# sea-with-sakura/ViT-of-Pytorch

Hardware: AMD Instinct MI355X
Metric: images/sec training step, ViT-B/16 224px bf16, 1/2/4/8 MI355X (higher is better)
Workload: dtype bf16; 1 GPU; ViT-B16 @224 train step (fwd+CE+bwd+SGD-momentum/OneCycleLR); model=ViT-B16, image_size=224, per_gpu_batch=256, global_batch=256, seq_len=197, num_classes=1000, parallelism=dp1, step_launch=eager

## Files before the change

### include/vit_hip.h

```cpp
#ifndef VIT_HIP_H_
#define VIT_HIP_H_

#include <stdint.h>

#ifdef __cplusplus
extern "C" {
#endif

typedef void* vit_stream_t;

enum vit_status {
  VIT_OK = 0,
  VIT_ERR_INVALID_ARG = 1,
  VIT_ERR_HIP = 2,
  VIT_ERR_UNSUPPORTED = 3,
};

const char* vit_last_error(void);
int vit_abi_version(void);
const char* vit_build_id(void);

enum vit_layout { VIT_K_CONTIG = 0, VIT_MN_CONTIG = 1 };

typedef struct vit_dropout {
  float p;
  uint32_t site;
  uint64_t seed;
  uint64_t offset;
  int64_t row_stride;
} vit_dropout;

int vit_dropout_mask(const vit_dropout* d, int64_t row0, int64_t rows, int64_t cols, float* mult,
                     int64_t ld, vit_stream_t stream);

enum vit_epilogue {
  VIT_EPI_F32 = 0,
  VIT_EPI_BF16 = 1,
  VIT_EPI_BIAS_BF16 = 2,
  VIT_EPI_BIAS_GELU = 3,
  VIT_EPI_BIAS_RESID_F32 = 4,
  VIT_EPI_GELU_BWD = 5,
  VIT_EPI_PATCH = 6,
  VIT_EPI_SPLITK = 7,
  VIT_EPI_BIAS_GELU_DGELU = 8,
  VIT_EPI_MUL_BF16 = 9,
};

typedef struct vit_gemm_args {
  int64_t M, N, K;
  const void* A;
  int64_t lda;
  int64_t a_batch_stride;
  int32_t a_layout;
  int32_t b_layout;
  const void* B;
  int64_t ldb;
  int64_t b_batch_stride;
  void* C;
  int64_t ldc;
  int64_t c_batch_stride;
  void* C2;
  int64_t ldc2;
  const float* bias;
  int64_t bias_batch_stride;
  const void* aux;
  int64_t ldaux;
  const float* aux2;
  int64_t batch;
  int64_t split_k;
  int64_t tokens;
  float* col_partial;
  int32_t epilogue;
  int32_t tile;
  const vit_dropout* dropout;
} vit_gemm_args;

int vit_gemm_bf16(const vit_gemm_args* args, vit_stream_t stream);
int64_t vit_gemm_tile_rows(const vit_gemm_args* args);
int64_t vit_gemm_partial_rows(const vit_gemm_args* args);
int64_t vit_gemm_split_rows(const vit_gemm_args* args);
int vit_gemm_bf16_part(const vit_gemm_args* args, int32_t part, vit_stream_t stream);
int vit_gemm_splitk_group(const vit_gemm_args* args, int32_t n, vit_stream_t stream);
#define VIT_GEMM_TABLE_MAX 128
int64_t vit_gemm_group_table_bytes(int32_t n);
int vit_gemm_group_prepare(const vit_gemm_args* args, const int32_t* direct, int32_t n, void* table,
                           int64_t table_bytes, int32_t* total, vit_stream_t stream);
int vit_gemm_group_launch(const void* table, int32_t n, int32_t total, vit_stream_t stream);

int vit_splitk_reduce(const float* ws, int64_t batch, int64_t split, int64_t M, int64_t N,
                      float* out, int64_t ldo, int64_t out_batch_stride, int32_t accumulate,
                      vit_stream_t stream);
#define VIT_SPLITK_GROUP_MAX 8
typedef struct vit_splitk_job {
  const float* ws;
  int64_t batch, split, M, N;
  float* out;
  int64_t ldo, out_batch_stride;
  int32_t accumulate;
  int32_t reserved;
} vit_splitk_job;
int vit_splitk_reduce_group(const vit_splitk_job* jobs, int32_t njobs, vit_stream_t stream);

int vit_layernorm_fwd(const float* x, int64_t ldx, const float* gamma, const float* beta,
                      void* y, int64_t ldy, int32_t y_f32, float* mean, float* rstd,
                      int64_t rows, int64_t D, float eps, vit_stream_t stream);
int64_t vit_layernorm_bwd_partial_rows(int64_t rows);
int64_t vit_layernorm_bwd_blocks(int64_t rows);
int vit_layernorm_bwd(const void* dy, int64_t lddy, int32_t dy_f32, const float* x, int64_t ldx,
                      const float* mean, const float* rstd, const float* gamma,
                      const float* dres, int64_t lddres, float* dx, int64_t lddx,
                      void* dx_bf16, int64_t lddxb, float* partial, float* dgamma_dbeta,
                      float* dx_colsum, int32_t accumulate_params, int64_t rows, int64_t D,
                      const vit_dropout* dx_dropout, vit_stream_t stream);

int vit_attention_fwd(const void* qkv, void* o, float* lse, int64_t B, int64_t N, int64_t H,
                      int64_t hd, float scale, vit_stream_t stream);
int vit_attention_bwd(const void* qkv, const void* o, const void* dout, const float* lse, void* dqkv,
                      float* bias_partial, int64_t B, int64_t N, int64_t H, int64_t hd, float scale,
                      vit_stream_t stream);
int vit_attention_fwd_rows(const void* qkv, void* o, float* lse, int64_t B, int64_t N, int64_t H, int64_t hd,
                           float scale, int64_t q_rows, vit_stream_t stream);
int vit_attention_bwd_rows(const void* qkv, const void* o, const void* dout, const float* lse, void* dqkv,
                           float* bias_partial, int64_t B, int64_t N, int64_t H, int64_t hd, float scale,
                           int64_t q_rows, vit_stream_t stream);
int64_t vit_attention_bias_rows(int64_t N, int64_t hd, int32_t path);
int64_t vit_attention_workspace_elems(int64_t B, int64_t N, int64_t H, int32_t path);
int vit_attention_fwd_ex(const void* qkv, void* o, float* lse, int64_t B, int64_t N, int64_t H, int64_t hd,
                         float scale, int64_t q_rows, int32_t path, vit_stream_t stream);
int vit_attention_bwd_ex(const void* qkv, const void* o, const void* dout, const float* lse, void* dqkv,
                         float* bias_partial, int64_t B, int64_t N, int64_t H, int64_t hd, float scale,
                         int64_t q_rows, int32_t path, float* workspace, vit_stream_t stream);

int vit_attention_fwd_varlen(const void* q, int64_t ldq, const void* k, int64_t ldk, const void* v, int64_t ldv,
                             void* o, int64_t ldo, const int32_t* cu_q, int64_t B, int64_t max_q, int64_t Nkv,
                             int64_t H, int64_t hd, float scale, vit_stream_t stream);

int vit_im2col(const float* x, void* out, int64_t B, int64_t img, int64_t P, int64_t Kpad,
               vit_stream_t stream);
int vit_im2col_hw(const float* x, void* out, int64_t B, int64_t H, int64_t W, int64_t Ph, int64_t Pw, int64_t Kpad,
                  vit_stream_t stream);

int vit_preprocess_u8(const uint8_t* images, int64_t B, int64_t H, int64_t W, int64_t image_stride,
                      const uint8_t* flips, int64_t out_h, int64_t out_w, const float* mean_std, float* out,
                      vit_stream_t stream);

enum vit_image_layout { VIT_IMAGES_HWC = 0, VIT_IMAGES_CHW = 1 };
int vit_preprocess_u8_gather(const uint8_t* images, int64_t n_images, int32_t layout, int64_t H, int64_t W,
                             int64_t image_stride, const int64_t* index, int64_t B, const uint8_t* flips,
                             int64_t out_h, int64_t out_w, const float* mean_std, float* out,
                             const int64_t* labels_in, int64_t* labels_out, vit_stream_t stream);

int vit_embed_grad(const float* dh0, int64_t B, int64_t N, int64_t D, float* dpos, float* dcls,
                   float* dconv_bias, const vit_dropout* dropout, vit_stream_t stream);

int64_t vit_colsum_partial_rows(int64_t rows);
int vit_colsum(const void* in, int32_t in_bf16, int64_t rows, int64_t cols, int64_t ld,
               float* partial, float* out, int32_t accumulate, vit_stream_t stream);
int vit_colsum3(const void* in, int32_t in_bf16, int64_t rows, int64_t seg, int64_t ld, float* partial,
                float* out0, float* out1, float* out2, int32_t accumulate, vit_stream_t stream);

#define VIT_COLSUM_BATCH_MAX 8
typedef struct vit_colsum_job {
  const float* in;
  int64_t rows, cols, ld, seg;
  float* out0;
  float* out1;
  float* out2;
  int32_t accumulate;
  int32_t reserved;
} vit_colsum_job;
int vit_colsum_batch(const vit_colsum_job* jobs, int32_t njobs, vit_stream_t stream);

int vit_gemm_f32(int64_t M, int64_t N, int64_t K, const float* A, int64_t lda, int32_t a_trans,
                 const float* B, int64_t ldb, int32_t b_trans, float* C, int64_t ldc,
                 const float* bias, int32_t accumulate, vit_stream_t stream);

int vit_cross_entropy(const float* logits, const int64_t* labels, int64_t B, int64_t C,
                      float* dlogits, float grad_scale, float* row_stats, vit_stream_t stream);

int vit_sgd_step(float* p, const float* g, float* buf, void* p_bf16, int64_t n, float lr,
                 float momentum, float weight_decay, int32_t first, vit_stream_t stream);
int vit_sgd_step_dev(float* p, const float* g, float* buf, void* p_bf16, int64_t n, const float* hyper,
                     float weight_decay, vit_stream_t stream);
int vit_cast_f32_bf16(const float* in, void* out, int64_t n, vit_stream_t stream);
int vit_cast_pad_rows(const float* in, int64_t rows, int64_t cols, void* out, int64_t ldo,
                      vit_stream_t stream);
#define VIT_CAST_BATCH_MAX 8
typedef struct vit_cast_job {
  const float* in;
  int64_t rows, cols, ldi;
  void* out;
  int64_t ldo, rows_pad, cols_pad;
} vit_cast_job;
int vit_cast_pad_batch(const vit_cast_job* jobs, int32_t njobs, vit_stream_t stream);
int vit_pack_cols(const float* in, int64_t zstride, int64_t ldi, int64_t rows, int64_t cols, int64_t Z,
                  void* out, int64_t ldo, int32_t out_bf16, vit_stream_t stream);
int vit_pack_cols_batched(const float* in, int64_t in_batch_stride, int64_t zstride, int64_t ldi, int64_t rows,
                          int64_t cols, int64_t Z, void* out, int64_t out_batch_stride, int64_t ldo,
                          int32_t out_bf16, int64_t batch, vit_stream_t stream);
int vit_transpose_f32_bf16(const float* in, int64_t rows, int64_t cols, int64_t ldi, void* out, int64_t ldo,
                           int64_t batch, int64_t in_batch_stride, int64_t out_batch_stride, vit_stream_t stream);
int vit_axpby(const float* x, float* y, int64_t n, float a, float b, vit_stream_t stream);

int vit_im2col_f32(const float* x, float* out, int64_t B, int64_t img, int64_t P, int64_t Kpad,
                   vit_stream_t stream);
int vit_im2col_hw_f32(const float* x, float* out, int64_t B, int64_t H, int64_t W, int64_t Ph, int64_t Pw,
                      int64_t Kpad, vit_stream_t stream);
int vit_embed_fwd_f32(float* h, int64_t B, int64_t N, int64_t D, const float* pos, const float* cls,
                      vit_stream_t stream);
int vit_gelu_f32(const float* in, float* out, int64_t n, vit_stream_t stream);
int vit_attention_fwd_f32(const float* qkv, float* o, int64_t B, int64_t N, int64_t H, int64_t hd,
                          float inv_sqrt_hd, vit_stream_t stream);

int vit_gelu_bwd_f32(const float* u, const float* dy, float* dx, int64_t n, vit_stream_t stream);
int vit_dropout_apply_f32(const vit_dropout* d, const float* in, float* out, int64_t rows, int64_t cols,
                          vit_stream_t stream);
int vit_add_bcast_f32(const float* x, const float* y, float* out, int64_t outer, int64_t inner, vit_stream_t stream);
int vit_segment_colsum(const void* in, int32_t in_bf16, int64_t ld, int64_t segs, int64_t seg_stride, int64_t row0,
                       int64_t seg_rows, int64_t cols, float scale, float* out, int64_t ldo, vit_stream_t stream);
int vit_segment_colsum_bcast(const void* in, int32_t in_bf16, int64_t ld, int64_t segs, int64_t seg_stride,
                             int64_t row0, int64_t seg_rows, int64_t cols, float scale, float* out, int64_t ldo,
                             void* bc, int64_t ldbc, int64_t bc_rows, vit_stream_t stream);
int64_t vit_router_dx_gate_partial_rows(int64_t rows_pad);
int vit_router_dx_gate(const float* dx, int64_t ldx, const float* g, int64_t ldg, float g_scale, const void* gp,
                       int64_t ldgp, int64_t T, int64_t N, int64_t reserve, int64_t cols, void* out, int64_t ldo,
                       int64_t rows_pad, int64_t cols_pad, float* col_partial, int64_t ldp, vit_stream_t stream);
int64_t vit_router_head_partials(int64_t T);
int vit_router_head_fwd(const float* logits, const float* noise, int32_t noise_mode, const float* yhard_in, int64_t T,
                        int64_t N, int32_t bs, int64_t reserve, int32_t training, float norm, float* soft, float* ysoft,
                        float* hard, float* indices, float* ent_part, float* entropy, vit_stream_t stream);
int vit_router_head_bwd(const float* soft, const float* ysoft, const float* dsoft, const float* dhard, const float* dind,
                        const float* dent, float norm, int64_t T, int64_t N, int32_t bs, int64_t reserve,
                        int32_t training, float* dlogits, vit_stream_t stream);
int vit_router_select(const float* indices, int64_t T, int32_t npos, const uint32_t* active_masks, int32_t nkeys,
                      void* active, void* sel, void* any, vit_stream_t stream);
int vit_cast_rows_masked(const float* in, int64_t ldi, int64_t rows, int64_t cols, const void* mask, void* out,
                         int64_t ldo, vit_stream_t stream);
int vit_cls_mse(const float* x, int64_t ldx, const float* t, int64_t ldt, int64_t B, int64_t D, float* e, float* part,
                float* loss, vit_stream_t stream);
int vit_cls_mse_bwd(float* dx, int64_t lddx, const float* e, int64_t B, int64_t D, const float* g,
// ... 24 lines not shown
```

### vit-of-pytorch_amd/csrc/capi.hip

```cpp
#include <stdarg.h>

#include "common.h"
#include "build_id.h"

namespace vit {
static thread_local char g_last_error[512] = "";

void set_error(const char* fmt, ...) {
  va_list ap;
  va_start(ap, fmt);
  vsnprintf(g_last_error, sizeof(g_last_error), fmt, ap);
  va_end(ap);
}

int check_hip(hipError_t e, const char* what) {
  if (e == hipSuccess) return VIT_OK;
  set_error("%s: %s", what, hipGetErrorString(e));
  return VIT_ERR_HIP;
}
}

extern "C" const char* vit_last_error(void) { return vit::g_last_error; }
extern "C" int vit_abi_version(void) { return 21; }
extern "C" const char* vit_build_id(void) { return VIT_BUILD_ID; }
```

### vit-of-pytorch_amd/csrc/elementwise.hip

```cpp
#include "common.h"

namespace {

template <typename OUT>
__global__ void im2col_kernel(const float* __restrict__ x, OUT* __restrict__ out, int B, int H, int W, int Ph, int Pw,
                              int Kpad) {
  const int gw = W / Pw;
  const int N = (H / Ph) * gw + 1;
  const long total = (long)B * N * Kpad;
  const int PP = Ph * Pw, K = 3 * PP;
  for (long i = (long)blockIdx.x * blockDim.x + threadIdx.x; i < total; i += (long)gridDim.x * blockDim.x) {
    const int col = (int)(i % Kpad);
    const long row = i / Kpad;
    const int t = (int)(row % N);
    const int b = (int)(row / N);
    float v = 0.f;
    if (t > 0 && col < K) {
      const int patch = t - 1, py = patch / gw, px = patch % gw;
      const int c = col / PP, rem = col % PP, ky = rem / Pw, kx = rem % Pw;
      v = x[(((long)b * 3 + c) * H + (py * Ph + ky)) * W + (px * Pw + kx)];
    }
    if constexpr (sizeof(OUT) == 2)
      out[i] = f2bf(v);
    else
      out[i] = v;
  }
}

__global__ void pos_grad_kernel(const float* __restrict__ dh0, int B, int N, int D, float* __restrict__ dpos,
                                DropDev drop) {
  const int n = blockIdx.y;
  const int d = blockIdx.x * blockDim.x + threadIdx.x;
  if (d >= D) return;
  float s = 0.f;
  if (drop.thr) {
    for (int b = 0; b < B; ++b) s += dh0[((long)b * N + n) * D + d] * drop_mult1(drop, (long)b * N + n, d);
  } else {
    for (int b = 0; b < B; ++b) s += dh0[((long)b * N + n) * D + d];
  }
  dpos[(long)n * D + d] = s;
}

__global__ void dropout_mask_kernel(DropDev drop, long row0, long rows, int cols, float* __restrict__ out, long ld) {
  const long r = blockIdx.y;
  const int c = blockIdx.x * blockDim.x + threadIdx.x;
  if (r >= rows || c >= cols) return;
  out[r * ld + c] = drop.thr ? drop_mult1(drop, row0 + r, c) : 1.0f;
}

template <typename OUT>
__global__ void im2col8_kernel(const float* __restrict__ x, OUT* __restrict__ out, int B, int H, int W, int Ph,
                               int Pw) {
  const int gw = W / Pw, N = (H / Ph) * gw + 1, PP = Ph * Pw, K8 = 3 * PP / 8;
  const long total = (long)B * N * K8;
  for (long i = (long)blockIdx.x * blockDim.x + threadIdx.x; i < total; i += (long)gridDim.x * blockDim.x) {
    const int c8 = (int)(i % K8);
    const long row = i / K8;
    const int t = (int)(row % N), b = (int)(row / N);
    float4 lo = make_float4(0.f, 0.f, 0.f, 0.f), hi = lo;
    if (t > 0) {
      const int patch = t - 1, py = patch / gw, px = patch % gw;
      const int col = c8 * 8, c = col / PP, rem = col % PP, ky = rem / Pw, kx = rem % Pw;
      const float4* src =
          reinterpret_cast<const float4*>(x + (((long)b * 3 + c) * H + (py * Ph + ky)) * W + (px * Pw + kx));
      lo = src[0];
      hi = src[1];
    }
    if constexpr (sizeof(OUT) == 2) {
      uint4 v;
      v.x = (uint32_t)f2bf(lo.x) | ((uint32_t)f2bf(lo.y) << 16);
      v.y = (uint32_t)f2bf(lo.z) | ((uint32_t)f2bf(lo.w) << 16);
      v.z = (uint32_t)f2bf(hi.x) | ((uint32_t)f2bf(hi.y) << 16);
      v.w = (uint32_t)f2bf(hi.z) | ((uint32_t)f2bf(hi.w) << 16);
      reinterpret_cast<uint4*>(out)[i] = v;
    } else {
      reinterpret_cast<float4*>(out)[2 * i] = lo;
      reinterpret_cast<float4*>(out)[2 * i + 1] = hi;
    }
  }
}

__global__ void __launch_bounds__(768) pos_grad4_kernel(const float* __restrict__ dh0, int B, int N, int D,
                                                        float* __restrict__ dpos, DropDev drop) {
  __shared__ float4 red[8][96];
  const int C4 = D / 4 / gridDim.y;
  const int n = blockIdx.x, c = threadIdx.x % C4, grp = threadIdx.x / C4;
  const int d = (blockIdx.y * C4 + c) * 4;
  float4 s = make_float4(0.f, 0.f, 0.f, 0.f);
  const float* base = dh0 + (long)n * D + d;
  const long bstride = (long)N * D;
#pragma unroll 4
  for (int b = grp; b < B; b += 8) {
    float4 v = *reinterpret_cast<const float4*>(base + b * bstride);
    if (drop.thr) {
      const long r = (long)b * N + n;
      v.x *= drop_mult1(drop, r, d);
      v.y *= drop_mult1(drop, r, d + 1);
      v.z *= drop_mult1(drop, r, d + 2);
      v.w *= drop_mult1(drop, r, d + 3);
    }
    s.x += v.x;
    s.y += v.y;
    s.z += v.z;
    s.w += v.w;
  }
  red[grp][c] = s;
  __syncthreads();
  if (grp == 0) {
#pragma unroll
    for (int k = 1; k < 8; ++k) {
      s.x += red[k][c].x;
      s.y += red[k][c].y;
      s.z += red[k][c].z;
      s.w += red[k][c].w;
    }
    *reinterpret_cast<float4*>(dpos + (long)n * D + d) = s;
  }
}

__global__ void __launch_bounds__(256) cls_bias_grad16_kernel(const float* __restrict__ dpos, int N, int D,
                                                              float* __restrict__ dcls, float* __restrict__ dbias) {
  __shared__ float red[16][17];
  const int c = threadIdx.x & 15, r = threadIdx.x >> 4;
  const int d = blockIdx.x * 16 + c;
  float s = 0.f;
  if (d < D)
    for (int n = 1 + r; n < N; n += 16) s += dpos[(long)n * D + d];
  red[r][c] = s;
  __syncthreads();
  if (r == 0 && d < D) {
    float t = 0.f;
#pragma unroll
    for (int k = 0; k < 16; ++k) t += red[k][c];
    dbias[d] = t;
    dcls[d] = dpos[d];
  }
}

constexpr int COLSUM_MAX_CHUNKS = 256;
constexpr int COLSUM_MIN_ROWS_PER_CHUNK = 64;

__device__ __forceinline__ float* seg_dst(float* out, float* out1, float* out2, long seg, long ch, int cols, int col) {
  if (seg <= 0) return out + ch * cols + col;
  const int k = (int)(col / seg);
  float* base = k == 0 ? out : (k == 1 ? out1 : out2);
  return base ? base + (col - k * seg) : nullptr;
}

template <bool BF16>
__global__ void __launch_bounds__(256) colsum8_kernel(const void* __restrict__ in, long rows, int cols, long ld,
                                                      int chunks, float* __restrict__ out, int accumulate,
                                                      long seg = 0, float* out1 = nullptr, float* out2 = nullptr) {
  __shared__ float red[8][32][9];
// ... 238 lines not shown
    buf[t] = d;
    p[t] -= lr * d;
    if (pb) pb[t] = f2bf(p[t]);
  }
}

__global__ void cast_kernel(const float* __restrict__ in, bf16_t* __restrict__ out, long n) {
  for (long i = (long)blockIdx.x * blockDim.x + threadIdx.x; i < n; i += (long)gridDim.x * blockDim.x) out[i] = f2bf(in[i]);
}
__global__ void cast_pad_kernel(const float* __restrict__ in, long rows, long cols, bf16_t* __restrict__ out, long ldo) {
  const long total = rows * ldo;
  for (long i = (long)blockIdx.x * blockDim.x + threadIdx.x; i < total; i += (long)gridDim.x * blockDim.x) {
    const long r = i / ldo, c = i % ldo;
    out[i] = c < cols ? f2bf(in[r * cols + c]) : (bf16_t)0;
  }
}
__global__ void axpby_kernel(const float* x, float* y, long n, float a, float b) {
  for (long i = (long)blockIdx.x * blockDim.x + threadIdx.x; i < n; i += (long)gridDim.x * blockDim.x)
    y[i] = a * x[i] + (b == 0.f ? 0.f : b * y[i]);
}

unsigned grid_for(long n, int per_thread = 1) {
  long b = (n / per_thread + 255) / 256;
  if (b < 1) b = 1;
  if (b > 8192) b = 8192;
  return (unsigned)b;
}

template <typename OUT>
void im2col_launch(const float* x, OUT* out, int64_t B, int64_t H, int64_t W, int64_t Ph, int64_t Pw, int64_t Kpad,
                   hipStream_t s) {
  const int64_t N = (H / Ph) * (W / Pw) + 1;
  if (Pw % 8 == 0 && W % 4 == 0 && Kpad == 3 * Ph * Pw && (uintptr_t)x % 16 == 0 && (uintptr_t)out % 16 == 0)
    hipLaunchKernelGGL(im2col8_kernel<OUT>, dim3(grid_for(B * N * Kpad / 8)), dim3(256), 0, s, x, out, (int)B, (int)H,
                       (int)W, (int)Ph, (int)Pw);
  else
    hipLaunchKernelGGL(im2col_kernel<OUT>, dim3(grid_for(B * N * Kpad)), dim3(256), 0, s, x, out, (int)B, (int)H,
                       (int)W, (int)Ph, (int)Pw, (int)Kpad);
}

}

extern "C" int vit_im2col_hw(const float* x, void* out, int64_t B, int64_t H, int64_t W, int64_t Ph, int64_t Pw,
                             int64_t Kpad, vit_stream_t stream) {
  VIT_CHECK_ARG(x && out && B > 0 && Ph > 0 && Pw > 0 && H >= Ph && W >= Pw && Kpad >= 3 * Ph * Pw &&
                    3 * H * W < (1L << 31) && Kpad < (1L << 31),
                "vit_im2col_hw: bad args");
  im2col_launch(x, (bf16_t*)out, B, H, W, Ph, Pw, Kpad, (hipStream_t)stream);
  VIT_LAUNCH_CHECK("vit_im2col_hw");
}

extern "C" int vit_im2col_hw_f32(const float* x, float* out, int64_t B, int64_t H, int64_t W, int64_t Ph, int64_t Pw,
                                 int64_t Kpad, vit_stream_t stream) {
  VIT_CHECK_ARG(x && out && B > 0 && Ph > 0 && Pw > 0 && H >= Ph && W >= Pw && Kpad >= 3 * Ph * Pw &&
                    3 * H * W < (1L << 31) && Kpad < (1L << 31),
                "vit_im2col_hw_f32: bad args");
  im2col_launch(x, out, B, H, W, Ph, Pw, Kpad, (hipStream_t)stream);
  VIT_LAUNCH_CHECK("vit_im2col_hw_f32");
}

extern "C" int vit_im2col(const float* x, void* out, int64_t B, int64_t img, int64_t P, int64_t Kpad,
                          vit_stream_t stream) {
  VIT_CHECK_ARG(x && out && B > 0 && P > 0 && img >= P && Kpad >= 3 * P * P, "vit_im2col: bad args");
  im2col_launch(x, (bf16_t*)out, B, img, img, P, P, Kpad, (hipStream_t)stream);
  VIT_LAUNCH_CHECK("vit_im2col");
}

extern "C" int vit_embed_grad(const float* dh0, int64_t B, int64_t N, int64_t D, float* dpos, float* dcls,
                              float* dconv_bias, const vit_dropout* dropout, vit_stream_t stream) {
  VIT_CHECK_ARG(dh0 && dpos && dcls && dconv_bias && B > 0 && N > 0 && D > 0, "vit_embed_grad: bad args");
  hipStream_t s = (hipStream_t)stream;
  int ys = 0;
  if (D % 4 == 0 && ((uintptr_t)dh0 % 16) == 0 && ((uintptr_t)dpos % 16) == 0) {
    const int d4 = (int)(D / 4);
    for (int y = (d4 + 95) / 96; y <= d4; ++y)
      if (d4 % y == 0) { ys = y; break; }
    if (ys == 1 && N < 256 && d4 % 2 == 0) ys = 2;
  }
  if (ys > 0)
    hipLaunchKernelGGL(pos_grad4_kernel, dim3((unsigned)N, (unsigned)ys), dim3((unsigned)(8 * (D / 4 / ys))), 0, s, dh0,
                       (int)B, (int)N, (int)D, dpos, make_drop(dropout));
  else
    hipLaunchKernelGGL(pos_grad_kernel, dim3((unsigned)((D + 255) / 256), (unsigned)N), dim3(256), 0, s, dh0, (int)B,
                       (int)N, (int)D, dpos, make_drop(dropout));
  hipLaunchKernelGGL(cls_bias_grad16_kernel, dim3((unsigned)((D + 15) / 16)), dim3(256), 0, s, dpos, (int)N, (int)D,
                     dcls, dconv_bias);
  VIT_LAUNCH_CHECK("vit_embed_grad");
}

extern "C" int64_t vit_colsum_partial_rows(int64_t rows) {
  int64_t c = rows / COLSUM_MIN_ROWS_PER_CHUNK;
  if (c > COLSUM_MAX_CHUNKS) c = COLSUM_MAX_CHUNKS;
  return c < 1 ? 1 : c;
}

extern "C" int vit_colsum3(const void* in, int32_t in_bf16, int64_t rows, int64_t seg, int64_t ld, float* partial,
                           float* out0, float* out1, float* out2, int32_t accumulate, vit_stream_t stream) {
  const int64_t cols = 3 * seg;
  VIT_CHECK_ARG(in && partial && seg > 0 && ld >= cols, "vit_colsum3: bad args");
  const int chunks = (int)vit_colsum_partial_rows(rows);
  const bool vec = cols % 8 == 0 && ld % 8 == 0 && ((uintptr_t)in % 32) == 0 && ((uintptr_t)partial % 16) == 0;
  VIT_CHECK_ARG(vec, "vit_colsum3: needs 8-column aligned rows");
  hipStream_t s = (hipStream_t)stream;
  const unsigned gx = (unsigned)((cols / 8 + 31) / 32);
  if (chunks == 1) {
    if (in_bf16)
      hipLaunchKernelGGL(colsum8_kernel<true>, dim3(gx, 1), dim3(256), 0, s, in, (long)rows, (int)cols, (long)ld, 1,
                         out0, (int)accumulate, (long)seg, out1, out2);
    else
      hipLaunchKernelGGL(colsum8_kernel<false>, dim3(gx, 1), dim3(256), 0, s, in, (long)rows, (int)cols, (long)ld, 1,
                         out0, (int)accumulate, (long)seg, out1, out2);
    VIT_LAUNCH_CHECK("vit_colsum3");
  }
  if (in_bf16)
    hipLaunchKernelGGL(colsum8_kernel<true>, dim3(gx, chunks), dim3(256), 0, s, in, (long)rows, (int)cols, (long)ld,
                       chunks, partial, 0, 0L, (float*)nullptr, (float*)nullptr);
  else
    hipLaunchKernelGGL(colsum8_kernel<false>, dim3(gx, chunks), dim3(256), 0, s, in, (long)rows, (int)cols, (long)ld,
                       chunks, partial, 0, 0L, (float*)nullptr, (float*)nullptr);
  hipLaunchKernelGGL(colsum8_kernel<false>, dim3(gx, 1), dim3(256), 0, s, (const void*)partial, (long)chunks,
                     (int)cols, (long)cols, 1, out0, (int)accumulate, (long)seg, out1, out2);
  VIT_LAUNCH_CHECK("vit_colsum3");
}

extern "C" int vit_colsum(const void* in, int32_t in_bf16, int64_t rows, int64_t cols, int64_t ld, float* partial,
                          float* out, int32_t accumulate, vit_stream_t stream) {
  VIT_CHECK_ARG(in && partial && out && cols > 0 && ld >= cols, "vit_colsum: bad args");
  hipStream_t s = (hipStream_t)stream;
  const int chunks = (int)vit_colsum_partial_rows(rows);
  const bool vec = cols % 8 == 0 && ld % 8 == 0 && ((uintptr_t)in % 32) == 0 && ((uintptr_t)partial % 16) == 0 &&
                   ((uintptr_t)out % 4) == 0;
  if (vec) {
    const unsigned gx = (unsigned)((cols / 8 + 31) / 32);
    float* dst1 = chunks == 1 ? out : partial;
    if (in_bf16)
      hipLaunchKernelGGL(colsum8_kernel<true>, dim3(gx, chunks), dim3(256), 0, s, in, (long)rows, (int)cols, (long)ld,
                         chunks, dst1, chunks == 1 ? (int)accumulate : 0);
    else
      hipLaunchKernelGGL(colsum8_kernel<false>, dim3(gx, chunks), dim3(256), 0, s, in, (long)rows, (int)cols,
                         (long)ld, chunks, dst1, chunks == 1 ? (int)accumulate : 0);
    if (chunks > 1)
      hipLaunchKernelGGL(colsum8_kernel<false>, dim3(gx, 1), dim3(256), 0, s, (const void*)partial, (long)chunks,
                         (int)cols, (long)cols, 1, out, (int)accumulate);
    VIT_LAUNCH_CHECK("vit_colsum");
  }
  const unsigned gx = (unsigned)((cols + 255) / 256);
  hipLaunchKernelGGL(colsum_partial_kernel, dim3(gx, chunks), dim3(256), 0, s, in, (int)in_bf16, (long)rows, (int)cols,
                     (long)ld, chunks, partial);
  hipLaunchKernelGGL(colsum_final_kernel, dim3(gx), dim3(256), 0, s, partial, chunks, (int)cols, out, (int)accumulate);
  VIT_LAUNCH_CHECK("vit_colsum");
}

namespace {
struct ColsumJobDev {
  const float* in;
  float* out[3];
  long ld;
  int rows, cols, seg, acc, blk0;
  int pad;
};
struct ColsumBatchDev {
  ColsumJobDev j[VIT_COLSUM_BATCH_MAX];
  int n;
};

__global__ void __launch_bounds__(256) colsum_batch_kernel(const ColsumBatchDev bt) {
  __shared__ float4 red[16][17];
  const int bid = blockIdx.x;
  int jx = 0;
#pragma unroll
  for (int k = 1; k < VIT_COLSUM_BATCH_MAX; ++k)
    if (k < bt.n && bid >= bt.j[k].blk0) jx = k;
  const ColsumJobDev& J = bt.j[jx];
  const int c0 = (bid - J.blk0) * 64;
  const int cg = threadIdx.x & 15, rl = threadIdx.x >> 4;
  const int c = c0 + cg * 4;
  float4 acc = {0.f, 0.f, 0.f, 0.f};
  if (J.pad && c < J.cols) {
    const float* p = J.in + c;
    const long ld = J.ld;
    int r = rl;
    for (; r + 112 < J.rows; r += 128) {
      float4 v[8];
#pragma unroll
      for (int u = 0; u < 8; ++u) v[u] = *reinterpret_cast<const float4*>(p + (long)(r + 16 * u) * ld);
#pragma unroll
      for (int u = 0; u < 8; ++u) {
        acc.x += v[u].x; acc.y += v[u].y; acc.z += v[u].z; acc.w += v[u].w;
      }
    }
    for (; r < J.rows; r += 16) {
      const float4 v = *reinterpret_cast<const float4*>(p + (long)r * ld);
      acc.x += v.x; acc.y += v.y; acc.z += v.z; acc.w += v.w;
    }
  } else if (c < J.cols) {
    const float* p = J.in + c;
    const int nc = J.cols - c < 4 ? J.cols - c : 4;
    for (int r = rl; r < J.rows; r += 16) {
      const float* q = p + (long)r * J.ld;
      acc.x += q[0];
      if (nc > 1) acc.y += q[1];
      if (nc > 2) acc.z += q[2];
      if (nc > 3) acc.w += q[3];
    }
  }
  red[rl][cg] = acc;
  __syncthreads();
  if (threadIdx.x < 64) {
    const int g = threadIdx.x >> 2, k = threadIdx.x & 3;
    const int col = c0 + threadIdx.x;
    if (col < J.cols) {
      float s = 0.f;
#pragma unroll
      for (int q = 0; q < 16; ++q) s += reinterpret_cast<const float*>(&red[q][g])[k];
      const int sg = J.seg > 0 ? col / J.seg : 0;
      float* base = J.out[sg];
      if (base) {
        float* dst = base + (col - sg * J.seg);
        *dst = J.acc ? *dst + s : s;
      }
    }
  }
}
}

extern "C" int vit_colsum_batch(const vit_colsum_job* jobs, int32_t njobs, vit_stream_t stream) {
  VIT_CHECK_ARG(jobs && njobs >= 1 && njobs <= VIT_COLSUM_BATCH_MAX, "vit_colsum_batch: njobs=%d outside [1, %d]",
                (int)njobs, VIT_COLSUM_BATCH_MAX);
  ColsumBatchDev bt{};
  int blk = 0;
  for (int k = 0; k < njobs; ++k) {
    const vit_colsum_job& s = jobs[k];
    VIT_CHECK_ARG(s.in && s.rows >= 1 && s.cols >= 1 && s.ld >= s.cols && s.rows <= 0x7fffffff &&
                      s.cols <= 0x7fffffff,
                  "vit_colsum_batch: job %d: bad shape (rows %lld, cols %lld, ld %lld)", k, (long long)s.rows,
                  (long long)s.cols, (long long)s.ld);
    VIT_CHECK_ARG(s.seg >= 0 && (s.seg == 0 || s.cols <= 3 * s.seg), "vit_colsum_batch: job %d: seg %lld", k,
                  (long long)s.seg);
    VIT_CHECK_ARG(s.out0 || s.out1 || s.out2, "vit_colsum_batch: job %d has no output", k);
    ColsumJobDev& d = bt.j[k];
    d.in = s.in;
    d.out[0] = s.out0;
    d.out[1] = s.out1;
    d.out[2] = s.out2;
    d.ld = (long)s.ld;
    d.rows = (int)s.rows;
    d.cols = (int)s.cols;
    d.seg = (int)s.seg;
    d.acc = s.accumulate ? 1 : 0;
    d.blk0 = blk;
    d.pad = (s.cols % 4 == 0 && s.ld % 4 == 0 && ((uintptr_t)s.in % 16) == 0) ? 1 : 0;
    blk += (int)((s.cols + 63) / 64);
  }
  bt.n = njobs;
  hipLaunchKernelGGL(colsum_batch_kernel, dim3(blk), dim3(256), 0, (hipStream_t)stream, bt);
  return vit::check_hip(hipGetLastError(), "vit_colsum_batch");
}

extern "C" int vit_gemm_f32(int64_t M, int64_t N, int64_t K, const float* A, int64_t lda, int32_t a_trans,
                            const float* B, int64_t ldb, int32_t b_trans, float* C, int64_t ldc, const float* bias,
                            int32_t accumulate, vit_stream_t stream) {
  VIT_CHECK_ARG(A && B && C && M >= 0 && N >= 0 && K >= 0, "vit_gemm_f32: bad args");
  if (M == 0 || N == 0) return VIT_OK;
  dim3 grid((unsigned)((N + 31) / 32), (unsigned)((M + 31) / 32)), block(256);
  hipLaunchKernelGGL(gemm_f32_kernel, grid, block, 0, (hipStream_t)stream, (int)M, (int)N, (int)K, A, (long)lda,
                     (int)a_trans, B, (long)ldb, (int)b_trans, C, (long)ldc, bias, (int)accumulate);
  VIT_LAUNCH_CHECK("vit_gemm_f32");
}

extern "C" int vit_cross_entropy(const float* logits, const int64_t* labels, int64_t B, int64_t C, float* dlogits,
                                 float grad_scale, float* row_stats, vit_stream_t stream) {
  VIT_CHECK_ARG(logits && labels && B > 0 && C > 0, "vit_cross_entropy: bad args");
  hipLaunchKernelGGL(ce_kernel, dim3((unsigned)B), dim3(256), 0, (hipStream_t)stream, logits, labels, (int)C, dlogits,
                     grad_scale, row_stats);
  VIT_LAUNCH_CHECK("vit_cross_entropy");
}

extern "C" int vit_sgd_step_dev(float* p, const float* g, float* buf, void* p_bf16, int64_t n, const float* hyper,
                                float weight_decay, vit_stream_t stream) {
  VIT_CHECK_ARG(p && g && buf && hyper && n >= 0, "vit_sgd_step_dev: bad args");
  VIT_CHECK_ARG(((uintptr_t)p | (uintptr_t)g | (uintptr_t)buf) % 16 == 0 && ((uintptr_t)p_bf16 % 8 == 0),
                "vit_sgd_step_dev: buffers must be 16-B aligned (bf16 mirror 8-B)");
  if (n == 0) return VIT_OK;
  hipLaunchKernelGGL(sgd_kernel<SgdDevScalars>, dim3(grid_for(n, 4)), dim3(256), 0, (hipStream_t)stream, p, g, buf,
                     (bf16_t*)p_bf16, (long)n, SgdDevScalars{hyper}, weight_decay);
  VIT_LAUNCH_CHECK("vit_sgd_step_dev");
}

extern "C" int vit_sgd_step(float* p, const float* g, float* buf, void* p_bf16, int64_t n, float lr, float momentum,
                            float weight_decay, int32_t first, vit_stream_t stream) {
  VIT_CHECK_ARG(p && g && buf && n >= 0, "vit_sgd_step: bad args");
  VIT_CHECK_ARG(((uintptr_t)p | (uintptr_t)g | (uintptr_t)buf) % 16 == 0 && ((uintptr_t)p_bf16 % 8 == 0),
                "vit_sgd_step: buffers must be 16-B aligned (bf16 mirror 8-B)");
  if (n == 0) return VIT_OK;
  hipLaunchKernelGGL(sgd_kernel<SgdHostScalars>, dim3(grid_for(n, 4)), dim3(256), 0, (hipStream_t)stream, p, g, buf,
                     (bf16_t*)p_bf16, (long)n, SgdHostScalars{lr, momentum, (int)first}, weight_decay);
  VIT_LAUNCH_CHECK("vit_sgd_step");
}

extern "C" int vit_cast_f32_bf16(const float* in, void* out, int64_t n, vit_stream_t stream) {
  VIT_CHECK_ARG(in && out && n >= 0, "vit_cast_f32_bf16: bad args");
  if (n == 0) return VIT_OK;
  hipLaunchKernelGGL(cast_kernel, dim3(grid_for(n)), dim3(256), 0, (hipStream_t)stream, in, (bf16_t*)out, (long)n);
  VIT_LAUNCH_CHECK("vit_cast_f32_bf16");
}

extern "C" int vit_cast_pad_rows(const float* in, int64_t rows, int64_t cols, void* out, int64_t ldo,
                                 vit_stream_t stream) {
  VIT_CHECK_ARG(in && out && ldo >= cols, "vit_cast_pad_rows: bad args");
  if (rows * ldo == 0) return VIT_OK;
  hipLaunchKernelGGL(cast_pad_kernel, dim3(grid_for(rows * ldo)), dim3(256), 0, (hipStream_t)stream, in, (long)rows,
                     (long)cols, (bf16_t*)out, (long)ldo);
  VIT_LAUNCH_CHECK("vit_cast_pad_rows");
}

namespace {
struct CastJobDev {
  const float* in;
  bf16_t* out;
  long rows, cols, ldi, ldo, rows_pad, cols_pad;
  int blk0, nb;
  int vec;
};
struct CastBatchDev {
  CastJobDev j[VIT_CAST_BATCH_MAX];
  int n;
};
__global__ void __launch_bounds__(256) cast_pad_batch_kernel(const CastBatchDev bt) {
  int jx = 0;
#pragma unroll
  for (int k = 1; k < VIT_CAST_BATCH_MAX; ++k)
    if (k < bt.n && (int)blockIdx.x >= bt.j[k].blk0) jx = k;
  const CastJobDev& J = bt.j[jx];
  if (J.vec) {
    const unsigned cq = (unsigned)(J.cols_pad >> 2), tq = (unsigned)(J.rows_pad * cq);
    for (unsigned q = (blockIdx.x - J.blk0) * 256u + threadIdx.x; q < tq; q += (unsigned)J.nb * 256u) {
      const unsigned r = q / cq, c = (q - r * cq) << 2;
      uint2 o = {0u, 0u};
      if (r < J.rows && c < J.cols) {
        const float4 v = *reinterpret_cast<const float4*>(J.in + r * J.ldi + c);
        o.x = pack2bf(v.x, v.y);
        o.y = pack2bf(v.z, v.w);
      }
      *reinterpret_cast<uint2*>(J.out + r * J.ldo + c) = o;
    }
    return;
  }
  const long total = J.rows_pad * J.cols_pad;
  for (long i = (long)(blockIdx.x - J.blk0) * 256 + threadIdx.x; i < total; i += (long)J.nb * 256) {
    const long r = i / J.cols_pad, c = i - r * J.cols_pad;
    J.out[r * J.ldo + c] = r < J.rows && c < J.cols ? f2bf(J.in[r * J.ldi + c]) : (bf16_t)0;
  }
}
}

extern "C" int vit_cast_pad_batch(const vit_cast_job* jobs, int32_t njobs, vit_stream_t stream) {
  VIT_CHECK_ARG(jobs && njobs >= 1 && njobs <= VIT_CAST_BATCH_MAX, "vit_cast_pad_batch: 1..%d jobs, got %d",
                VIT_CAST_BATCH_MAX, (int)njobs);
  CastBatchDev bt{};
  long blk = 0;
  for (int k = 0; k < njobs; ++k) {
    const vit_cast_job& j = jobs[k];
    VIT_CHECK_ARG(j.in && j.out && j.rows >= 0 && j.cols >= 0 && j.ldi >= j.cols && j.rows_pad >= j.rows &&
                      j.cols_pad >= j.cols && j.ldo >= j.cols_pad,
                  "vit_cast_pad_batch: job %d: bad shape", k);
    const int vec = (j.cols | j.cols_pad | j.ldi | j.ldo) % 4 == 0 && (uintptr_t)j.in % 16 == 0 &&
                    (uintptr_t)j.out % 8 == 0 && j.rows_pad * j.cols_pad / 4 < (1L << 31) ? 1 : 0;
    long nb = (j.rows_pad * j.cols_pad / (vec ? 4 : 1) + 255) / 256;
    if (nb > 2048) nb = 2048;
    if (nb < 1) nb = 1;
    CastJobDev& d = bt.j[k];
    d.in = j.in; d.out = (bf16_t*)j.out; d.rows = j.rows; d.cols = j.cols; d.ldi = j.ldi; d.ldo = j.ldo;
    d.rows_pad = j.rows_pad; d.cols_pad = j.cols_pad; d.blk0 = (int)blk; d.nb = (int)nb;
    d.vec = vec;
    blk += nb;
  }
  bt.n = njobs;
  hipLaunchKernelGGL(cast_pad_batch_kernel, dim3((unsigned)blk), dim3(256), 0, (hipStream_t)stream, bt);
  VIT_LAUNCH_CHECK("vit_cast_pad_batch");
}

extern "C" int vit_axpby(const float* x, float* y, int64_t n, float a, float b, vit_stream_t stream) {
  VIT_CHECK_ARG(x && y && n >= 0, "vit_axpby: bad args");
  if (n == 0) return VIT_OK;
  hipLaunchKernelGGL(axpby_kernel, dim3(grid_for(n)), dim3(256), 0, (hipStream_t)stream, x, y, (long)n, a, b);
  VIT_LAUNCH_CHECK("vit_axpby");
}

namespace {
template <bool BF16OUT>
__global__ void pack_cols_kernel(const float* __restrict__ in, long zstride, long ldi, int rows, int cols, int Z,
                                 void* __restrict__ out, long ldo, long in_bs = 0, long out_bs = 0) {
  in += (long)blockIdx.y * in_bs;
  out = (char*)out + (long)blockIdx.y * out_bs * (BF16OUT ? 2 : 4);
  const long total = (long)rows * Z * cols;
  for (long i = (long)blockIdx.x * blockDim.x + threadIdx.x; i < total; i += (long)gridDim.x * blockDim.x) {
    const long r = i / ((long)Z * cols);
    const int zc = (int)(i % ((long)Z * cols));
    const int z = zc / cols, c = zc % cols;
    const float v = in[z * zstride + r * ldi + c];
    if constexpr (BF16OUT)
      ((bf16_t*)out)[r * ldo + zc] = f2bf(v);
    else
      ((float*)out)[r * ldo + zc] = v;
  }
// ... 776 lines not shown
```

### vit-of-pytorch_amd/csrc/gemm.hip

```cpp
#include "gemm_decl.h"

#include <vector>

namespace {
using vitg::GemmDev;
using vitg::EPI_DROP;

int pick_tile(const vit_gemm_args* a) {
  if (a->tile > 0) return (int)a->tile;
  const bool ak = a->a_layout == VIT_K_CONTIG, bk = a->b_layout == VIT_K_CONTIG;
  if (a->epilogue == VIT_EPI_SPLITK && a->M >= 256 && a->N >= 256) {
    static const int env_sk = vit::knob("VIT_GEMM_SPLITK_CFG", 9);
    return env_sk == 5 || env_sk == 6 || env_sk == 7 || env_sk == 8 ? env_sk : 9;
  }
  if (a->M >= 1024 && a->N >= 256) {
    static const int env_rs = vit::knob("VIT_GEMM_RESID_PP2", 1);
    if (ak && (env_rs || !(a->epilogue == VIT_EPI_BIAS_RESID_F32 && a->K < 2048))) return 9;
    if (a->N >= 2048 && a->epilogue != VIT_EPI_GELU_BWD && a->epilogue != VIT_EPI_MUL_BF16) return 5;
    if (!bk && a->K >= 3072) return 5;
    return 3;
  }
  return 0;
}

// ... 101 lines not shown
  d.B = (const char*)a->B; d.ldb = a->ldb; d.b_bs = a->b_batch_stride; d.b_bytes = (uint32_t)b_bytes;
  d.C = a->C; d.ldc = a->ldc; d.c_bs = a->c_batch_stride;
  d.C2 = a->C2; d.ldc2 = a->ldc2;
  d.bias = a->bias; d.bias_bs = a->bias_batch_stride;
  d.aux = a->aux; d.ldaux = a->ldaux; d.aux2 = a->aux2;
  d.split_k = (int)a->split_k; d.tokens = (int)a->tokens;
  {
    auto al = [](const void* q) { return ((uintptr_t)q % 32) == 0; };
    bool v = al(a->C) && a->ldc % 8 == 0 && a->c_batch_stride % 8 == 0;
    if (a->C2) v = v && al(a->C2) && a->ldc2 % 8 == 0;
    if (a->bias) v = v && al(a->bias) && a->bias_batch_stride % 8 == 0;
    if (a->aux) v = v && al(a->aux) && a->ldaux % 8 == 0;
    if (a->aux2) v = v && al(a->aux2);
    if (a->epilogue == VIT_EPI_SPLITK) v = al(a->C) && a->N % 8 == 0;
    d.vec = v ? 1 : 0;
  }
  if (a->epilogue == VIT_EPI_SPLITK) {
    d.ldc = a->N;
    d.c_bs = a->M * a->N;
  }
  d.col_partial = a->col_partial;
  d.drop = make_drop(a->dropout);
  VIT_CHECK_ARG(!d.drop.thr || a->epilogue == VIT_EPI_PATCH || a->epilogue == VIT_EPI_BIAS_RESID_F32 ||
                    a->epilogue == VIT_EPI_BIAS_GELU_DGELU,
                "vit_gemm_bf16: dropout is supported on the PATCH, BIAS_RESID_F32 and BIAS_GELU_DGELU epilogues");
  VIT_CHECK_ARG(!d.drop.thr || (a->a_layout == VIT_K_CONTIG &&
                                  (a->b_layout == VIT_K_CONTIG || a->epilogue == VIT_EPI_BIAS_RESID_F32)),
                "vit_gemm_bf16: dropout epilogues need a K-contiguous A (and B, except BIAS_RESID_F32)");
  {
    static const int env_gm = vit::knob("VIT_GEMM_GROUP_M", 8);
    static const int env_nt = vit::knob("VIT_GEMM_NT", 0);
    d.group_m = env_gm;
    d.nt = env_nt;
    static const int env_diag = vit::knob("VIT_GEMM_DIAG", 0);
    d.diag = env_diag;
    static const int env_sx = vit::knob("VIT_GEMM_SPLIT_XCD", 1);
    d.split_xcd = env_sx;
    static const int env_prio = vit::knob("VIT_GEMM_PRIO", 1);
    d.prio = env_prio;
    static const int env_ilv = vit::knob("VIT_GEMM_ILV", -1);
    d.ilv = env_ilv;
#ifdef VIT_PP2_STAMPS
    d.stamps = g_pp2_stamp_buf;
#endif
  }
  return VIT_OK;
}

int gemm_bf16_impl(const vit_gemm_args* a, int part, vit_stream_t stream) {
  GemmDev d;
  bool empty = false;
  if (const int rc = make_dev(a, d, empty)) return rc;
  if (empty) return VIT_OK;
  const bool ak = a->a_layout == VIT_K_CONTIG, bk = a->b_layout == VIT_K_CONTIG;
  if (a->col_partial) {
    VIT_CHECK_ARG(a->batch == 1 && a->split_k == 1 && d.vec && a->N % 8 == 0 &&
                      (a->epilogue == VIT_EPI_F32 || a->epilogue == VIT_EPI_BF16 || a->epilogue == VIT_EPI_GELU_BWD ||
                       a->epilogue == VIT_EPI_MUL_BF16 ||
                       a->epilogue == VIT_EPI_BIAS_BF16 || a->epilogue == VIT_EPI_BIAS_RESID_F32),
                  "vit_gemm_bf16: col_partial needs batch 1, split_k 1, aligned N%%8==0 operands and a plain epilogue");
  }
  hipStream_t s = (hipStream_t)stream;
  const int batch = (int)a->batch, split = (int)a->split_k;
  const int cfg = pick_tile(a);
#ifdef VIT_DIAG_KNOBS
  VIT_CHECK_ARG(cfg >= 0 && cfg <= 11, "vit_gemm_bf16: bad tile config %d", cfg);
#else
  VIT_CHECK_ARG(cfg >= 0 && cfg <= 9, "vit_gemm_bf16: bad tile config %d", cfg);
#endif
  VIT_CHECK_ARG(cfg != 1 || a->K % 32 == 0, "vit_gemm_bf16: K");
  auto run = [&](int c, const GemmDev& g) -> hipError_t {
    switch (a->epilogue) {
      case VIT_EPI_F32: return vitg::launch_layout_x<VIT_EPI_F32>(c, g, ak, bk, batch, split, s);
      case VIT_EPI_BF16: return vitg::launch_layout_x<VIT_EPI_BF16>(c, g, ak, bk, batch, split, s);
      case VIT_EPI_BIAS_BF16: return vitg::launch_layout_x<VIT_EPI_BIAS_BF16>(c, g, ak, bk, batch, split, s);
      case VIT_EPI_BIAS_GELU: return vitg::launch_layout_x<VIT_EPI_BIAS_GELU>(c, g, ak, bk, batch, split, s);
      case VIT_EPI_BIAS_RESID_F32:
        if (g.drop.thr) return vitg::launch_kk_x<VIT_EPI_BIAS_RESID_F32 | EPI_DROP>(c, g, bk, batch, split, s);
        return vitg::launch_layout_x<VIT_EPI_BIAS_RESID_F32>(c, g, ak, bk, batch, split, s);
      case VIT_EPI_GELU_BWD: return vitg::launch_layout_x<VIT_EPI_GELU_BWD>(c, g, ak, bk, batch, split, s);
      case VIT_EPI_BIAS_GELU_DGELU:
        if (g.drop.thr) return vitg::launch_kk_x<VIT_EPI_BIAS_GELU_DGELU | EPI_DROP>(c, g, bk, batch, split, s);
        return vitg::launch_layout_x<VIT_EPI_BIAS_GELU_DGELU>(c, g, ak, bk, batch, split, s);
      case VIT_EPI_MUL_BF16: return vitg::launch_layout_x<VIT_EPI_MUL_BF16>(c, g, ak, bk, batch, split, s);
      case VIT_EPI_PATCH:
        if (g.drop.thr) return vitg::launch_kk_x<VIT_EPI_PATCH | EPI_DROP>(c, g, bk, batch, split, s);
        return vitg::launch_layout_x<VIT_EPI_PATCH>(c, g, ak, bk, batch, split, s);
      case VIT_EPI_SPLITK: return vitg::launch_layout_x<VIT_EPI_SPLITK>(c, g, ak, bk, batch, split, s);
      default: return hipErrorInvalidValue;
    }
  };
  if (a->epilogue < 0 || a->epilogue > VIT_EPI_MUL_BF16) {
    vit::set_error("vit_gemm_bf16: unknown epilogue %d", a->epilogue);
    return VIT_ERR_INVALID_ARG;
  }
  if (const long main_rows = wave_split_rows(a, cfg)) {
    GemmDev g1 = d, g2 = d;
    g1.M = (int)main_rows;
    g2.M = (int)(a->M - main_rows);
    const long r0 = main_rows;
    const long a_off = ak ? r0 * a->lda * 2 : r0 * 2;
    g2.A = d.A + a_off;
    g2.a_bytes = d.a_bytes > a_off ? (uint32_t)(d.a_bytes - a_off) : 0u;
    const int csz = (a->epilogue == VIT_EPI_F32 || a->epilogue == VIT_EPI_BIAS_RESID_F32) ? 4 : 2;
    g2.C = (char*)d.C + r0 * a->ldc * csz;
    if (d.C2) g2.C2 = (char*)d.C2 + r0 * a->ldc2 * 2;
    if (d.aux) g2.aux = (const char*)d.aux + r0 * a->ldaux * (a->epilogue == VIT_EPI_BIAS_RESID_F32 ? 4 : 2);
    if (d.col_partial) g2.col_partial = d.col_partial + (main_rows / 256) * a->N;
    g2.drop.row0 = (int)r0;
    hipError_t e = hipSuccess;
    if (part != 2) e = run(cfg, g1);
    if (e == hipSuccess && part != 1) e = run(rem_config(), g2);
    return vit::check_hip(e, "vit_gemm_bf16 launch");
  }
  if (part == 2) return VIT_OK;
  return vit::check_hip(run(cfg, d), "vit_gemm_bf16 launch");
}
}

extern "C" int vit_gemm_bf16(const vit_gemm_args* a, vit_stream_t stream) { return gemm_bf16_impl(a, 0, stream); }

extern "C" int vit_gemm_bf16_part(const vit_gemm_args* a, int32_t part, vit_stream_t stream) {
  VIT_CHECK_ARG(part == 1 || part == 2, "vit_gemm_bf16_part: part %d (1 = whole-wave rows, 2 = remainder)", part);
  return gemm_bf16_impl(a, part, stream);
}

extern "C" int vit_gemm_splitk_group(const vit_gemm_args* args, int32_t n, vit_stream_t stream) {
  VIT_CHECK_ARG(args != nullptr && n >= 1 && n <= vitg::GEMM_GROUP_MAX, "vit_gemm_splitk_group: 1..%d members, got %d",
                vitg::GEMM_GROUP_MAX, n);
  vitg::GemmGroup g{};
  long total = 0;
  for (int i = 0; i < n; ++i) {
    const vit_gemm_args* a = args + i;
    VIT_CHECK_ARG(a->epilogue == VIT_EPI_SPLITK && a->a_layout == VIT_MN_CONTIG && a->b_layout == VIT_MN_CONTIG &&
                      a->tile == 0 && !a->col_partial && !a->dropout,
                  "vit_gemm_splitk_group: member %d must be a split-K weight gradient (VIT_EPI_SPLITK, both operands "
                  "M/N-contiguous, no tile / col_partial / dropout)", i);
    bool empty = false;
    if (const int rc = make_dev(a, g.g[i], empty)) return rc;
    VIT_CHECK_ARG(!empty, "vit_gemm_splitk_group: member %d is empty", i);
    g.start[i] = (int)total;
    total += ((a->M + 255) / 256) * ((a->N + 255) / 256) * a->split_k * a->batch;
    VIT_CHECK_ARG(total < (1L << 30), "vit_gemm_splitk_group: grid too large");
  }
  g.start[n] = (int)total;
  g.n = n;
  return vit::check_hip(vitg::launch_splitk_group(g, (hipStream_t)stream), "vit_gemm_splitk_group launch");
}

extern "C" int64_t vit_gemm_group_table_bytes(int32_t n) {
  return n >= 1 && n <= vitg::GEMM_TABLE_MAX ? (int64_t)vitg::group_table_bytes(n) : 0;
}

extern "C" int vit_gemm_group_prepare(const vit_gemm_args* args, const int32_t* direct, int32_t n, void* table,
                                      int64_t table_bytes, int32_t* total_out, vit_stream_t stream) {
  VIT_CHECK_ARG(args != nullptr && n >= 1 && n <= vitg::GEMM_TABLE_MAX, "vit_gemm_group_prepare: 1..%d members, got %d",
                vitg::GEMM_TABLE_MAX, n);
  VIT_CHECK_ARG(table != nullptr && total_out != nullptr && table_bytes >= (int64_t)vitg::group_table_bytes(n) &&
                    ((uintptr_t)table % 16) == 0,
                "vit_gemm_group_prepare: needs a 16-byte aligned table of vit_gemm_group_table_bytes(n) bytes");
  const size_t soff = vitg::group_table_start_off(n);
  std::vector<char> host(vitg::group_table_bytes(n), 0);
  GemmDev* g = reinterpret_cast<GemmDev*>(host.data());
  int* start = reinterpret_cast<int*>(host.data() + soff);
  long total = 0;
  for (int i = 0; i < n; ++i) {
    const vit_gemm_args* a = args + i;
    VIT_CHECK_ARG(a->epilogue == VIT_EPI_SPLITK && a->a_layout == VIT_MN_CONTIG && a->b_layout == VIT_MN_CONTIG &&
                      a->tile == 0 && !a->col_partial && !a->dropout,
                  "vit_gemm_group_prepare: member %d must be a split-K weight gradient (VIT_EPI_SPLITK, both operands "
                  "M/N-contiguous, no tile / col_partial / dropout)", i);
    bool empty = false;
    if (const int rc = make_dev(a, g[i], empty)) return rc;
    VIT_CHECK_ARG(!empty, "vit_gemm_group_prepare: member %d is empty", i);
    if (direct && direct[i]) {
      VIT_CHECK_ARG(a->split_k == 1 && a->ldc >= a->N && (a->batch == 1 || a->c_batch_stride > 0),
                    "vit_gemm_group_prepare: direct member %d needs split_k 1, ldc >= N and an output batch stride", i);
      g[i].ldc = a->ldc;
      g[i].c_bs = a->c_batch_stride;
      g[i].vec = ((uintptr_t)a->C % 32) == 0 && a->ldc % 8 == 0 && a->c_batch_stride % 8 == 0;
    }
    start[i] = (int)total;
    total += ((a->M + 255) / 256) * ((a->N + 255) / 256) * a->split_k * a->batch;
    VIT_CHECK_ARG(total < (1L << 30), "vit_gemm_group_prepare: grid too large");
  }
  start[n] = (int)total;
  hipStream_t s = (hipStream_t)stream;
  if (const int rc = vit::check_hip(hipStreamSynchronize(s), "vit_gemm_group_prepare sync")) return rc;
  if (const int rc = vit::check_hip(hipMemcpy(table, host.data(), host.size(), hipMemcpyHostToDevice),
                                    "vit_gemm_group_prepare upload"))
    return rc;
  *total_out = (int32_t)total;
  return VIT_OK;
}

extern "C" int vit_gemm_group_launch(const void* table, int32_t n, int32_t total, vit_stream_t stream) {
  VIT_CHECK_ARG(table != nullptr && n >= 1 && n <= vitg::GEMM_TABLE_MAX && total >= 1,
                "vit_gemm_group_launch: a prepared table, its member count and its workgroup total");
  return vit::check_hip(vitg::launch_group_table(table, n, total, (hipStream_t)stream), "vit_gemm_group_launch");
}

namespace {
__global__ void splitk_reduce_kernel(const float* __restrict__ ws, int split, long M, long N, float* __restrict__ out,
                                     long ldo, long obs, int accumulate) {
  const int z = blockIdx.y;
  const long total = M * N;
  const float* w = ws + (long)z * split * total;
  float* o = out + z * obs;
  for (long i = (long)blockIdx.x * blockDim.x + threadIdx.x; i < total; i += (long)gridDim.x * blockDim.x) {
    float s = 0.f;
    for (int k = 0; k < split; ++k) s += w[k * total + i];
    const long m = i / N, n = i - m * N;
    float* dst = o + m * ldo + n;
    *dst = accumulate ? *dst + s : s;
  }
}
__global__ void splitk_reduce4_kernel(const float* __restrict__ ws, int split, long M, long N, float* __restrict__ out,
                                      long ldo, long obs, int accumulate) {
  const int z = blockIdx.y;
  const long total = M * N, total4 = total / 4;
  const float4* w = reinterpret_cast<const float4*>(ws + (long)z * split * total);
  float* o = out + z * obs;
  for (long i = (long)blockIdx.x * blockDim.x + threadIdx.x; i < total4; i += (long)gridDim.x * blockDim.x) {
    float4 s = make_float4(0.f, 0.f, 0.f, 0.f);
    int k = 0;
    for (; k + 4 <= split; k += 4) {
      const float4 a = w[(long)k * total4 + i], b = w[(long)(k + 1) * total4 + i];
      const float4 c = w[(long)(k + 2) * total4 + i], d = w[(long)(k + 3) * total4 + i];
      s.x += (a.x + b.x) + (c.x + d.x);
      s.y += (a.y + b.y) + (c.y + d.y);
      s.z += (a.z + b.z) + (c.z + d.z);
      s.w += (a.w + b.w) + (c.w + d.w);
    }
    for (; k < split; ++k) {
      const float4 a = w[(long)k * total4 + i];
      s.x += a.x; s.y += a.y; s.z += a.z; s.w += a.w;
    }
    const long e = i * 4, m = e / N, n = e - m * N;
    float4* dst = reinterpret_cast<float4*>(o + m * ldo + n);
    if (accumulate) {
      const float4 p = *dst;
      s.x += p.x; s.y += p.y; s.z += p.z; s.w += p.w;
    }
    *dst = s;
  }
}

struct SplitkJobDev {
  const float* ws;
  float* out;
  long M, N, ldo, obs;
  int split, batch, nb, blk0, acc;
};
struct SplitkGroupDev {
  SplitkJobDev j[VIT_SPLITK_GROUP_MAX];
  int n;
};
__global__ void splitk_reduce4_group_kernel(const SplitkGroupDev G) {
  int jx = 0;
#pragma unroll
  for (int k = 1; k < VIT_SPLITK_GROUP_MAX; ++k)
    if (k < G.n && (int)blockIdx.x >= G.j[k].blk0) jx = k;
  const SplitkJobDev& J = G.j[jx];
  const int local = blockIdx.x - J.blk0;
  const int z = local / J.nb, bx = local - z * J.nb;
  const long total = J.M * J.N, total4 = total / 4;
  const float4* w = reinterpret_cast<const float4*>(J.ws + (long)z * J.split * total);
  float* o = J.out + z * J.obs;
  for (long i = (long)bx * blockDim.x + threadIdx.x; i < total4; i += (long)J.nb * blockDim.x) {
    float4 s = make_float4(0.f, 0.f, 0.f, 0.f);
    int k = 0;
    for (; k + 4 <= J.split; k += 4) {
      const float4 a = w[(long)k * total4 + i], b = w[(long)(k + 1) * total4 + i];
      const float4 c = w[(long)(k + 2) * total4 + i], d = w[(long)(k + 3) * total4 + i];
      s.x += (a.x + b.x) + (c.x + d.x);
      s.y += (a.y + b.y) + (c.y + d.y);
      s.z += (a.z + b.z) + (c.z + d.z);
      s.w += (a.w + b.w) + (c.w + d.w);
    }
    for (; k < J.split; ++k) {
      const float4 a = w[(long)k * total4 + i];
      s.x += a.x; s.y += a.y; s.z += a.z; s.w += a.w;
    }
    const long e = i * 4, m = e / J.N, n = e - m * J.N;
    float4* dst = reinterpret_cast<float4*>(o + m * J.ldo + n);
    if (J.acc) {
      const float4 p = *dst;
      s.x += p.x; s.y += p.y; s.z += p.z; s.w += p.w;
    }
    *dst = s;
  }
}
}

extern "C" int vit_splitk_reduce_group(const vit_splitk_job* jobs, int32_t n, vit_stream_t stream) {
  VIT_CHECK_ARG(jobs && n >= 1 && n <= VIT_SPLITK_GROUP_MAX, "vit_splitk_reduce_group: 1..%d jobs, got %d",
                VIT_SPLITK_GROUP_MAX, (int)n);
  bool vec = true;
  for (int k = 0; k < n; ++k) {
    const vit_splitk_job& j = jobs[k];
    VIT_CHECK_ARG(j.ws && j.out && j.batch >= 1 && j.split >= 1 && j.M >= 1 && j.N >= 1 && j.ldo >= j.N,
                  "vit_splitk_reduce_group: job %d: bad args", k);
    vec = vec && j.N % 4 == 0 && j.ldo % 4 == 0 && j.out_batch_stride % 4 == 0 && ((uintptr_t)j.ws % 16) == 0 &&
          ((uintptr_t)j.out % 16) == 0;
  }
  if (!vec) {
    for (int k = 0; k < n; ++k) {
      const vit_splitk_job& j = jobs[k];
      if (const int rc = vit_splitk_reduce(j.ws, j.batch, j.split, j.M, j.N, j.out, j.ldo, j.out_batch_stride,
                                           j.accumulate, stream))
        return rc;
    }
    return VIT_OK;
  }
  SplitkGroupDev g{};
  long blk = 0;
  for (int k = 0; k < n; ++k) {
    const vit_splitk_job& j = jobs[k];
    long nb = (j.M * j.N / 4 + 255) / 256;
    if (nb > 4096) nb = 4096;
    SplitkJobDev& d = g.j[k];
    d.ws = j.ws; d.out = j.out; d.M = j.M; d.N = j.N; d.ldo = j.ldo; d.obs = j.out_batch_stride;
    d.split = (int)j.split; d.batch = (int)j.batch; d.nb = (int)nb; d.blk0 = (int)blk; d.acc = j.accumulate ? 1 : 0;
    blk += nb * j.batch;
  }
  g.n = n;
  VIT_CHECK_ARG(blk < (1L << 31), "vit_splitk_reduce_group: grid too large");
  hipLaunchKernelGGL(splitk_reduce4_group_kernel, dim3((unsigned)blk), dim3(256), 0, (hipStream_t)stream, g);
  VIT_LAUNCH_CHECK("vit_splitk_reduce_group");
}

extern "C" int vit_splitk_reduce(const float* ws, int64_t batch, int64_t split, int64_t M, int64_t N, float* out,
                                 int64_t ldo, int64_t out_batch_stride, int32_t accumulate, vit_stream_t stream) {
  VIT_CHECK_ARG(ws && out && batch >= 1 && split >= 1 && ldo >= N, "vit_splitk_reduce: bad args");
  if (M * N == 0) return VIT_OK;
  const bool vec = N % 4 == 0 && ldo % 4 == 0 && out_batch_stride % 4 == 0 && ((uintptr_t)ws % 16) == 0 &&
                   ((uintptr_t)out % 16) == 0;
  long blocks = (M * N / (vec ? 4 : 1) + 255) / 256;
  if (blocks > 4096) blocks = 4096;
  if (vec)
    hipLaunchKernelGGL(splitk_reduce4_kernel, dim3((unsigned)blocks, (unsigned)batch), dim3(256), 0,
                       (hipStream_t)stream, ws, (int)split, (long)M, (long)N, out, (long)ldo, (long)out_batch_stride,
                       (int)accumulate);
  else
    hipLaunchKernelGGL(splitk_reduce_kernel, dim3((unsigned)blocks, (unsigned)batch), dim3(256), 0, (hipStream_t)stream,
                       ws, (int)split, (long)M, (long)N, out, (long)ldo, (long)out_batch_stride, (int)accumulate);
  VIT_LAUNCH_CHECK("vit_splitk_reduce");
}
```

### vit-of-pytorch_amd/csrc/gemm_decl.h

```cpp
#pragma once
#include "common.h"
#include <stdlib.h>

namespace vitg {

struct GemmDev {
  int M, N, K;
  const char* A;
  long lda;
  long a_bs;
  uint32_t a_bytes;
  const char* B;
  long ldb;
  long b_bs;
  uint32_t b_bytes;
  void* C;
  long ldc;
  long c_bs;
  void* C2;
  long ldc2;
  const float* bias;
  long bias_bs;
  const void* aux;
  long ldaux;
  const float* aux2;
  int split_k;
  int tokens;
  int vec;
  float* col_partial;
  int group_m;
  int nt;
  DropDev drop;
  int diag;
  int split_xcd;
  int prio;
  int ilv;
#ifdef VIT_PP2_STAMPS
  unsigned long long* stamps;
#endif
};

constexpr int GEMM_GROUP_MAX = 4;
struct GemmGroup {
  GemmDev g[GEMM_GROUP_MAX];
  int start[GEMM_GROUP_MAX + 1];
  int n;
};
hipError_t launch_splitk_group(const GemmGroup& g, hipStream_t s);

constexpr int GEMM_TABLE_MAX = 128;
inline size_t group_table_start_off(int n) { return ((size_t)n * sizeof(GemmDev) + 15) & ~(size_t)15; }
inline size_t group_table_bytes(int n) { return group_table_start_off(n) + ((size_t)n + 1) * sizeof(int); }
hipError_t launch_group_table(const void* table, int n, int total, hipStream_t s);

constexpr int EPI_DROP = 16;

template <int EPI>
hipError_t launch_layout_x(int cfg, const GemmDev& d, bool ak, bool bk, int batch, int split, hipStream_t s);
template <int EPI>
hipError_t launch_kk_x(int cfg, const GemmDev& d, bool bk, int batch, int split, hipStream_t s);
template <> hipError_t launch_layout_x<0>(int, const GemmDev&, bool, bool, int, int, hipStream_t);
template <> hipError_t launch_layout_x<1>(int, const GemmDev&, bool, bool, int, int, hipStream_t);
template <> hipError_t launch_layout_x<2>(int, const GemmDev&, bool, bool, int, int, hipStream_t);
template <> hipError_t launch_layout_x<3>(int, const GemmDev&, bool, bool, int, int, hipStream_t);
template <> hipError_t launch_layout_x<4>(int, const GemmDev&, bool, bool, int, int, hipStream_t);
template <> hipError_t launch_layout_x<5>(int, const GemmDev&, bool, bool, int, int, hipStream_t);
template <> hipError_t launch_layout_x<6>(int, const GemmDev&, bool, bool, int, int, hipStream_t);
template <> hipError_t launch_layout_x<7>(int, const GemmDev&, bool, bool, int, int, hipStream_t);
template <> hipError_t launch_layout_x<8>(int, const GemmDev&, bool, bool, int, int, hipStream_t);
template <> hipError_t launch_layout_x<9>(int, const GemmDev&, bool, bool, int, int, hipStream_t);
template <> hipError_t launch_kk_x<20>(int, const GemmDev&, bool, int, int, hipStream_t);
template <> hipError_t launch_kk_x<22>(int, const GemmDev&, bool, int, int, hipStream_t);
template <> hipError_t launch_kk_x<24>(int, const GemmDev&, bool, int, int, hipStream_t);
}
```

### vit-of-pytorch_amd/csrc/gemm_e7.hip

```cpp
#include "gemm_kernels.h"

template <> hipError_t vitg::launch_layout_x<7>(int cfg, const GemmDev& d, bool ak, bool bk, int batch, int split, hipStream_t s) {
  return launch_layout<7>(cfg, d, ak, bk, batch, split, s);
}

hipError_t vitg::launch_splitk_group(const GemmGroup& g, hipStream_t s) { return launch_pp2_group(g, s); }

hipError_t vitg::launch_group_table(const void* table, int n, int total, hipStream_t s) {
  return launch_pp2_table(table, n, total, s);
}
```

### vit-of-pytorch_amd/csrc/gemm_pp2.inc

```
template <bool AK, bool BKC, int EPI, int BK = 64, int NA = 2>
__device__ __forceinline__ void pp2_tile(const GemmDev& p, const int tm, const int tn, const int z,
                                         const int split_idx, const int orig) {
  constexpr int BM = 256, BN = 256, KK = BK / 32;
  constexpr int NB = NA + 1;
  constexpr int TN = BN / 4, FM = 8, FN = TN / 16;
  constexpr int HALF = 128 * BK * 2;
  constexpr int A0_OFF = 0, A1_OFF = NA * HALF, B_OFF = 2 * NA * HALF;
  constexpr int LDS = (2 * NA + 2 * NB) * HALF;
  constexpr int I = BK / 16;
  constexpr int LDW = TN + 4;
  constexpr int PR = 32;
  constexpr int WST = PR * LDW * 4;
  static_assert(8 * WST <= LDS && LDS <= 160 * 1024, "LDS budget / epilogue staging");
  static_assert(2 * I * (NA - 1) <= 32 && (2 * NA - 1) * I <= 62 && 2 * (NB - 1) * I <= 62, "vmcnt range");
  __shared__ __attribute__((aligned(16))) char smem[LDS];

  const int lane = threadIdx.x & 63;
  const int wave = __builtin_amdgcn_readfirstlane(threadIdx.x >> 6);
  const int grp = wave >> 2, wn = wave & 3;
  const int m0 = tm * BM, n0 = tn * BN;
  if (p.diag >= 100 && ((orig >> 3) & 1) && (orig >> 3) < 32) {
    const unsigned long long t0 = __builtin_amdgcn_s_memrealtime();
    while (__builtin_amdgcn_s_memrealtime() - t0 < (unsigned long long)(p.diag - 100) * 100ull)
      __builtin_amdgcn_s_sleep(8);
  }

  const char* Ab = p.A + (long)z * p.a_bs * 2;
  const char* Bb = p.B + (long)z * p.b_bs * 2;
  const long a_shift = AK ? (long)m0 * p.lda * 2 : (long)m0 * 2;
  const long b_shift = BKC ? (long)n0 * p.ldb * 2 : (long)n0 * 2;
  const uint32_t a_rec = (long)p.a_bytes > a_shift ? (uint32_t)(p.a_bytes - a_shift) : 0u;
  const uint32_t b_rec = (long)p.b_bytes > b_shift ? (uint32_t)(p.b_bytes - b_shift) : 0u;
  const __amdgpu_buffer_rsrc_t rsA = make_rsrc(Ab + a_shift, a_rec);
  const __amdgpu_buffer_rsrc_t rsB = make_rsrc(Bb + b_shift, b_rec);
  const int a_h1 = AK ? (int)(128 * p.lda * 2) : 256;
  const int b_h1 = BKC ? (int)(128 * p.ldb * 2) : 256;

  const int nkt = p.K / BK;
  const int kt0 = (int)((long)nkt * split_idx / p.split_k);
  const int kt1 = (int)((long)nkt * (split_idx + 1) / p.split_k);
  const int nk = kt1 - kt0;

  v4f acc[FM][FN];
#pragma unroll
  for (int i = 0; i < FM; ++i)
#pragma unroll
    for (int j = 0; j < FN; ++j) acc[i][j] = v4f{0.f, 0.f, 0.f, 0.f};
  v8s af[KK][FM], bfr[KK][FN];
  const int w4 = wave & 3;
#ifdef VIT_PP2_STAMPS
  const bool stw = p.diag == 4 && p.stamps && orig == 0 && split_idx == 0 && z == 0 && w4 == 0;
  unsigned long long stv[8] = {0, 0, 0, 0, 0, 0, 0, 0};
#define PP2_ST(k)                                          \
  do {                                                     \
    if (stw && j == nk / 2) {                              \
      __builtin_amdgcn_sched_barrier(0);                   \
      stv[k] = __builtin_amdgcn_s_memtime();               \
      __builtin_amdgcn_sched_barrier(0);                   \
    }                                                      \
  } while (0)
#else
#define PP2_ST(k) \
  do {            \
  } while (0)
#endif

  auto ld_a = [&](int h, int t) {
    stage_tile<128, BK, AK, 4>(smem, (h ? A1_OFF : A0_OFF) + (t % NA) * HALF, rsA, p.lda, kt0 + t, w4, lane,
                               h ? a_h1 : 0);
  };
  auto ld_b = [&](int h, int t) {
    stage_tile<128, BK, BKC, 4>(smem, B_OFF + (t % NB) * 2 * HALF + h * HALF, rsB, p.ldb, kt0 + t, w4, lane,
                                h ? b_h1 : 0);
  };
  uint32_t a_lane[AK ? 1 : FM], b_lane[BKC ? 1 : FN];
  if constexpr (!AK) {
#pragma unroll
    for (int i = 0; i < FM; ++i) a_lane[i] = frag_tr_lane_off<128>(i * 16, lane);
  }
  if constexpr (!BKC) {
#pragma unroll
    for (int jn = 0; jn < FN; ++jn) b_lane[jn] = frag_tr_lane_off<128>((wn & 1) * 64 + jn * 16, lane);
  }
  const uint32_t s0 = (uint32_t)(uintptr_t)LDS_PTR(char, smem);
  auto mem = [&](int t) {
    const int aoff = (grp ? A1_OFF : A0_OFF) + (t % NA) * HALF;
    const int boff = B_OFF + (t % NB) * 2 * HALF + (wn >> 1) * HALF;
    const uint32_t ab = __builtin_amdgcn_readfirstlane(s0 + aoff), bb = __builtin_amdgcn_readfirstlane(s0 + boff);
#pragma unroll
    for (int kk = 0; kk < KK; ++kk) {
#pragma unroll
      for (int jn = 0; jn < FN; ++jn) {
        if constexpr (BKC)
          bfr[kk][jn] = read_frag<128, BK, BKC>(smem, boff, (wn & 1) * 64 + jn * 16, kk, lane);
        else
          bfr[kk][jn] = kk == 0 ? read_frag_tr_asm<128, 0>(b_lane[jn] + bb) : read_frag_tr_asm<128, 1>(b_lane[jn] + bb);
      }
#pragma unroll
      for (int i = 0; i < FM; ++i) {
        if constexpr (AK)
          af[kk][i] = read_frag<128, BK, AK>(smem, aoff, i * 16, kk, lane);
        else
          af[kk][i] = kk == 0 ? read_frag_tr_asm<128, 0>(a_lane[i] + ab) : read_frag_tr_asm<128, 1>(a_lane[i] + ab);
      }
    }
  };
#ifdef VIT_DIAG_KNOBS
  const bool ilv = p.ilv < 0 ? (!AK && !BKC) : p.ilv > 0;
#else
  constexpr bool ilv = !AK && !BKC;
#endif
  auto frag = [&](int t, int f) {
    constexpr int NF = FN + FM;
    const int kk = f / NF, r = f % NF;
    const int aoff = (grp ? A1_OFF : A0_OFF) + (t % NA) * HALF;
    const int boff = B_OFF + (t % NB) * 2 * HALF + (wn >> 1) * HALF;
    const uint32_t ab = __builtin_amdgcn_readfirstlane(s0 + aoff), bb = __builtin_amdgcn_readfirstlane(s0 + boff);
    if (r < FN) {
      if constexpr (BKC)
        bfr[kk][r] = read_frag<128, BK, BKC>(smem, boff, (wn & 1) * 64 + r * 16, kk, lane);
      else
        bfr[kk][r] = kk == 0 ? read_frag_tr_asm<128, 0>(b_lane[r] + bb) : read_frag_tr_asm<128, 1>(b_lane[r] + bb);
    } else {
      const int i = r - FN;
      if constexpr (AK)
        af[kk][i] = read_frag<128, BK, AK>(smem, aoff, i * 16, kk, lane);
      else
        af[kk][i] = kk == 0 ? read_frag_tr_asm<128, 0>(a_lane[i] + ab) : read_frag_tr_asm<128, 1>(a_lane[i] + ab);
    }
  };
  auto piece = [&](int q, int j, bool g1) {
    __builtin_amdgcn_sched_barrier(0);
    if (q < I) {
      const int t = g1 ? j + NA : j + NA - 1;
      if (t < nk)
        stage_piece<128, BK, AK, 4>(smem, (g1 ? A0_OFF : A1_OFF) + (t % NA) * HALF, rsA, p.lda, kt0 + t, w4, lane,
                                    g1 ? 0 : a_h1, q);
    } else {
      const int t = j + NB - 1;
      if (t < nk)
        stage_piece<128, BK, BKC, 4>(smem, B_OFF + (t % NB) * 2 * HALF + (g1 ? HALF : 0), rsB, p.ldb, kt0 + t, w4,
                                     lane, g1 ? b_h1 : 0, q - I);
    }
    __builtin_amdgcn_sched_barrier(0);
  };
  auto slot_ilv = [&](int j, bool g1) {
    constexpr int NFR = KK * (FN + FM), NP = 2 * I, PER = NFR / NP;
    static_assert(PER * NP == NFR, "whole fragments between pieces");
#pragma unroll
    for (int f = 0; f < NFR; ++f) {
      frag(j, f);
      if (f % PER == PER - 1) piece(f / PER, j, g1);
    }
  };
  auto reads_done = [&]() {
    asm volatile("s_waitcnt lgkmcnt(0)" ::: "memory");
    __builtin_amdgcn_sched_barrier(0);
  };
  auto compute = [&]() {
    if (p.prio == 1) __builtin_amdgcn_s_setprio(1);
#pragma unroll
    for (int kk = 0; kk < KK; ++kk)
#pragma unroll
      for (int i = 0; i < FM; ++i)
#pragma unroll
        for (int jn = 0; jn < FN; ++jn)
          acc[i][jn] = __builtin_amdgcn_mfma_f32_16x16x32_bf16(__builtin_bit_cast(v8bf, af[kk][i]),
                                                               __builtin_bit_cast(v8bf, bfr[kk][jn]), acc[i][jn], 0, 0, 0);
// ... 116 lines not shown
    }
  }
#ifdef VIT_PP2_STAMPS
  if (stw && lane == 0) {
#pragma unroll
    for (int k = 0; k < 8; ++k) p.stamps[grp * 8 + k] = stv[k];
  }
#endif
#undef PP2_ST

  if (p.diag == 2) {
    float t = 0.f;
#pragma unroll
    for (int i = 0; i < FM; ++i)
#pragma unroll
      for (int jn = 0; jn < FN; ++jn) t += acc[i][jn][0] + acc[i][jn][1] + acc[i][jn][2] + acc[i][jn][3];
    if (t == 1234.5f) ((float*)p.C)[threadIdx.x] = t;
    return;
  }
  const int wm0 = grp * 128, wn0 = wn * TN;
  const int g = lane >> 4, c = lane & 15;
  float* ws = reinterpret_cast<float*>(smem + wave * WST);
  constexpr int CPR = TN / 8;
  float csum[8] = {0.f, 0.f, 0.f, 0.f, 0.f, 0.f, 0.f, 0.f};
  constexpr int IT = PR * CPR / 64;
  static_assert(IT * 64 == PR * CPR, "whole chunks per pass");
  constexpr int AW = AuxPre<EPI>::W > 0 ? AuxPre<EPI>::W : 1;
  uint4 axc[IT][AW], axn[IT][AW];
  auto fetch_pass = [&](uint4 (*ax)[AW], int pass) {
    if constexpr (AuxPre<EPI>::W > 0) {
#pragma unroll
      for (int it = 0; it < IT; ++it) {
        const int e = lane + it * 64, row = e / CPR, ch = e % CPR;
        const int m = m0 + wm0 + pass * PR + row, n = n0 + wn0 + ch * 8;
        if (p.vec && m < p.M && n + 8 <= p.N) AuxPre<EPI>::fetch(p, m, n, ax[it]);
      }
    }
  };
  if (EpiOut<EPI>::FAST && p.vec && p.diag == 0 && m0 + BM <= p.M && n0 + BN <= p.N) {
    epilogue_fast<EPI, FN, LDW, CPR>(p, acc, ws, lane, m0 + wm0, n0 + wn0, z, split_idx, csum);
  } else {
  fetch_pass(axc, 0);
#pragma unroll
  for (int pass = 0; pass < 128 / PR; ++pass) {
    if (pass + 1 < 128 / PR) fetch_pass(axn, pass + 1);
#pragma unroll
    for (int i = 0; i < PR / 16; ++i)
#pragma unroll
      for (int jn = 0; jn < FN; ++jn)
#pragma unroll
        for (int r = 0; r < 4; ++r) ws[(i * 16 + 4 * g + r) * LDW + jn * 16 + c] = acc[pass * (PR / 16) + i][jn][r];
    asm volatile("s_waitcnt lgkmcnt(0)" ::: "memory");
    __builtin_amdgcn_wave_barrier();
#pragma unroll
    for (int it = 0; it < IT; ++it) {
      const int e = lane + it * 64, row = e / CPR, ch = e % CPR;
      const int m = m0 + wm0 + pass * PR + row, n = n0 + wn0 + ch * 8;
      float v[8];
      ld8f(ws + row * LDW + ch * 8, v);
      if (m >= p.M || n >= p.N || p.diag == 1 || (p.diag == 3 && (blockIdx.x & 1))) continue;
      if (p.vec && n + 8 <= p.N) {
        if constexpr (AuxPre<EPI>::W > 0) {
          float u[8];
          AuxPre<EPI>::unpack(axc[it], u);
          epi_store8<EPI>(p, z, split_idx, m, n, v, u);
        } else {
          epi_store8<EPI>(p, z, split_idx, m, n, v);
        }
        if (p.col_partial) {
#pragma unroll
          for (int k = 0; k < 8; ++k) csum[k] += v[k];
        }
      } else {
#pragma unroll
        for (int k = 0; k < 8; ++k) epi_store<EPI>(p, z, split_idx, m, n + k, v[k]);
      }
    }
    asm volatile("s_waitcnt lgkmcnt(0)" ::: "memory");
    __builtin_amdgcn_wave_barrier();
    if constexpr (AuxPre<EPI>::W > 0) {
#pragma unroll
      for (int it = 0; it < IT; ++it)
#pragma unroll
        for (int w = 0; w < AW; ++w) axc[it][w] = axn[it][w];
    }
  }
  }
  if (p.col_partial) {
#pragma unroll
    for (int k = 0; k < 8; ++k)
#pragma unroll
      for (int o = CPR; o < 64; o <<= 1) csum[k] += __shfl_xor(csum[k], o, 64);
    __syncthreads();
    float* red = reinterpret_cast<float*>(smem);
    if (lane < CPR) {
#pragma unroll
      for (int k = 0; k < 8; ++k) red[grp * BN + wn0 + lane * 8 + k] = csum[k];
    }
    __syncthreads();
    for (int col = threadIdx.x; col < BN; col += 512)
      if (n0 + col < p.N) p.col_partial[(long)tm * p.N + n0 + col] = red[col] + red[BN + col];
  }
}

__device__ __forceinline__ void splitk_coords(const GemmDev& p, int w, int nwg, int tiles_m, int tiles_n, int& tm, int& tn,
                                              int& z, int& split_idx) {
  const int zs = w / nwg;
  z = zs / p.split_k;
  split_idx = zs % p.split_k;
  tile_coords(w % nwg, tiles_m, tiles_n, p.group_m, tm, tn);
}

__device__ __forceinline__ int xcd_major(int lin, int total) {
  const int xcd = lin & 7, q8 = total >> 3, r8 = total & 7;
  return (xcd < r8 ? xcd * (q8 + 1) : r8 * (q8 + 1) + (xcd - r8) * q8) + (lin >> 3);
}

template <bool AK, bool BKC, int EPI, int BK = 64, int NA = 2>
__global__ void __launch_bounds__(512) gemm_pp2_kernel(const GemmDev p) {
  const int tiles_m = (p.M + 255) / 256, tiles_n = (p.N + 255) / 256;
  const int nwg = tiles_m * tiles_n;
  const int orig = blockIdx.x;
  int tm, tn, z, split_idx;
  if (p.split_k > 1 && p.split_xcd) {
    const int total = nwg * p.split_k * (int)gridDim.z;
    const int lin = blockIdx.x + nwg * (blockIdx.y + p.split_k * blockIdx.z);
    splitk_coords(p, xcd_major(lin, total), nwg, tiles_m, tiles_n, tm, tn, z, split_idx);
  } else {
    tile_coords(xcd_major(orig, nwg), tiles_m, tiles_n, p.group_m, tm, tn);
    z = blockIdx.z;
    split_idx = blockIdx.y;
  }
  pp2_tile<AK, BKC, EPI, BK, NA>(p, tm, tn, z, split_idx, orig);
}

template <bool AK, bool BKC>
__global__ void __launch_bounds__(512) gemm_pp2_group_kernel(const GemmGroup G) {
  const int orig = blockIdx.x;
  const int w = xcd_major(orig, G.start[G.n]);
  int gi = 0;
#pragma unroll
  for (int k = 1; k < GEMM_GROUP_MAX; ++k)
    if (k < G.n && w >= G.start[k]) gi = k;
  gi = __builtin_amdgcn_readfirstlane(gi);
  const GemmDev& p = G.g[gi];
  const int tiles_m = (p.M + 255) / 256, tiles_n = (p.N + 255) / 256;
  int tm, tn, z, split_idx;
  splitk_coords(p, w - G.start[gi], tiles_m * tiles_n, tiles_m, tiles_n, tm, tn, z, split_idx);
  pp2_tile<AK, BKC, VIT_EPI_SPLITK>(p, tm, tn, z, split_idx, orig);
}

template <bool AK, bool BKC>
__global__ void __launch_bounds__(512) gemm_pp2_table_kernel(const GemmDev* __restrict__ tab,
                                                             const int* __restrict__ start, const int n) {
  const int orig = blockIdx.x;
  const int w = xcd_major(orig, (int)gridDim.x);
  int lo = 0, hi = n;
  while (hi - lo > 1) {
    const int mid = (lo + hi) >> 1;
    if (w >= start[mid])
      lo = mid;
    else
      hi = mid;
  }
  const int gi = __builtin_amdgcn_readfirstlane(lo);
  const GemmDev p = tab[gi];
  const int tiles_m = (p.M + 255) / 256, tiles_n = (p.N + 255) / 256;
  int tm, tn, z, split_idx;
  splitk_coords(p, w - start[gi], tiles_m * tiles_n, tiles_m, tiles_n, tm, tn, z, split_idx);
  pp2_tile<AK, BKC, VIT_EPI_SPLITK>(p, tm, tn, z, split_idx, orig);
}

template <bool AK, bool BKC, int EPI, int BK = 64, int NA = 2>
hipError_t launch_pp2(const GemmDev& d, int batch, int split, hipStream_t s) {
  const int tiles = ((d.M + 255) / 256) * ((d.N + 255) / 256);
  dim3 grid(tiles, split, batch);
  hipLaunchKernelGGL((gemm_pp2_kernel<AK, BKC, EPI, BK, NA>), grid, dim3(512), 0, s, d);
  return hipGetLastError();
}

inline hipError_t launch_pp2_group(const GemmGroup& g, hipStream_t s) {
  hipLaunchKernelGGL((gemm_pp2_group_kernel<false, false>), dim3(g.start[g.n]), dim3(512), 0, s, g);
  return hipGetLastError();
}

inline hipError_t launch_pp2_table(const void* table, int n, int total, hipStream_t s) {
  const GemmDev* tab = (const GemmDev*)table;
  const int* start = (const int*)((const char*)table + vitg::group_table_start_off(n));
  hipLaunchKernelGGL((gemm_pp2_table_kernel<false, false>), dim3(total), dim3(512), 0, s, tab, start, n);
  return hipGetLastError();
}
```

### vit-of-pytorch_amd/vitmi/_lib.py

```python
from __future__ import annotations

import ctypes
import os

_HERE = os.path.dirname(os.path.abspath(__file__))
LIB_PATH = os.environ.get("VITMI_LIB") or os.path.join(_HERE, "libvit_hip.so")

c_i64 = ctypes.c_int64
c_i32 = ctypes.c_int32
c_f32 = ctypes.c_float
c_vp = ctypes.c_void_p

ABI_VERSION = 21

K_CONTIG, MN_CONTIG = 0, 1
(EPI_F32, EPI_BF16, EPI_BIAS_BF16, EPI_BIAS_GELU, EPI_BIAS_RESID_F32, EPI_GELU_BWD, EPI_PATCH, EPI_SPLITK,
 EPI_BIAS_GELU_DGELU, EPI_MUL_BF16) = range(10)


class Dropout(ctypes.Structure):
    _fields_ = [("p", c_f32), ("site", ctypes.c_uint32), ("seed", ctypes.c_uint64), ("offset", ctypes.c_uint64),
                ("row_stride", c_i64)]


class GemmArgs(ctypes.Structure):
    _fields_ = [
        ("M", c_i64), ("N", c_i64), ("K", c_i64),
        ("A", c_vp), ("lda", c_i64), ("a_batch_stride", c_i64),
        ("a_layout", c_i32), ("b_layout", c_i32),
        ("B", c_vp), ("ldb", c_i64), ("b_batch_stride", c_i64),
        ("C", c_vp), ("ldc", c_i64), ("c_batch_stride", c_i64),
        ("C2", c_vp), ("ldc2", c_i64),
        ("bias", c_vp), ("bias_batch_stride", c_i64),
        ("aux", c_vp), ("ldaux", c_i64), ("aux2", c_vp),
        ("batch", c_i64), ("split_k", c_i64), ("tokens", c_i64), ("col_partial", c_vp),
        ("epilogue", c_i32), ("tile", c_i32), ("dropout", ctypes.POINTER(Dropout)),
    ]


class ColsumJob(ctypes.Structure):
    _fields_ = [("inp", c_vp), ("rows", c_i64), ("cols", c_i64), ("ld", c_i64), ("seg", c_i64),
                ("out0", c_vp), ("out1", c_vp), ("out2", c_vp), ("accumulate", c_i32), ("reserved", c_i32)]


COLSUM_BATCH_MAX = 8


class SplitkJob(ctypes.Structure):
    _fields_ = [("ws", c_vp), ("batch", c_i64), ("split", c_i64), ("M", c_i64), ("N", c_i64), ("out", c_vp),
                ("ldo", c_i64), ("out_batch_stride", c_i64), ("accumulate", c_i32), ("reserved", c_i32)]


SPLITK_GROUP_MAX = 8


class CastJob(ctypes.Structure):
    _fields_ = [("inp", c_vp), ("rows", c_i64), ("cols", c_i64), ("ldi", c_i64), ("out", c_vp), ("ldo", c_i64),
                ("rows_pad", c_i64), ("cols_pad", c_i64)]


CAST_BATCH_MAX = 8

_SIGS = {
    "vit_last_error": (ctypes.c_char_p, []),
    "vit_abi_version": (c_i32, []),
    "vit_gemm_bf16": (c_i32, [ctypes.POINTER(GemmArgs), c_vp]),
    "vit_gemm_tile_rows": (c_i64, [ctypes.POINTER(GemmArgs)]),
    "vit_gemm_partial_rows": (c_i64, [ctypes.POINTER(GemmArgs)]),
    "vit_gemm_split_rows": (c_i64, [ctypes.POINTER(GemmArgs)]),
    "vit_gemm_bf16_part": (c_i32, [ctypes.POINTER(GemmArgs), c_i32, c_vp]),
    "vit_gemm_splitk_group": (c_i32, [ctypes.POINTER(GemmArgs), c_i32, c_vp]),
    "vit_gemm_group_table_bytes": (c_i64, [c_i32]),
    "vit_gemm_group_prepare": (c_i32, [ctypes.POINTER(GemmArgs), ctypes.POINTER(c_i32), c_i32, c_vp, c_i64,
                                       ctypes.POINTER(c_i32), c_vp]),
    "vit_gemm_group_launch": (c_i32, [c_vp, c_i32, c_i32, c_vp]),
    "vit_segment_colsum": (c_i32, [c_vp, c_i32, c_i64, c_i64, c_i64, c_i64, c_i64, c_i64, c_f32, c_vp, c_i64, c_vp]),
    "vit_segment_colsum_bcast": (c_i32, [c_vp, c_i32, c_i64, c_i64, c_i64, c_i64, c_i64, c_i64, c_f32, c_vp, c_i64,
                                         c_vp, c_i64, c_i64, c_vp]),
    "vit_router_dx_gate_partial_rows": (c_i64, [c_i64]),
    "vit_router_dx_gate": (c_i32, [c_vp, c_i64, c_vp, c_i64, c_f32, c_vp, c_i64, c_i64, c_i64, c_i64, c_i64, c_vp,
                                   c_i64, c_i64, c_i64, c_vp, c_i64, c_vp]),
    "vit_splitk_reduce_group": (c_i32, [ctypes.POINTER(SplitkJob), c_i32, c_vp]),
    "vit_cast_pad_batch": (c_i32, [ctypes.POINTER(CastJob), c_i32, c_vp]),
    "vit_router_head_partials": (c_i64, [c_i64]),
    "vit_cast_rows_masked": (c_i32, [c_vp, c_i64, c_i64, c_i64, c_vp, c_vp, c_i64, c_vp]),
    "vit_router_select": (c_i32, [c_vp, c_i64, c_i32, ctypes.POINTER(ctypes.c_uint32), c_i32, c_vp, c_vp, c_vp, c_vp]),
    "vit_cls_mse": (c_i32, [c_vp, c_i64, c_vp, c_i64, c_i64, c_i64, c_vp, c_vp, c_vp, c_vp]),
    "vit_cls_mse_bwd": (c_i32, [c_vp, c_i64, c_vp, c_i64, c_i64, c_vp, c_vp]),
    "vit_router_head_fwd": (c_i32, [c_vp, c_vp, c_i32, c_vp, c_i64, c_i64, c_i32, c_i64, c_i32, c_f32, c_vp, c_vp, c_vp,
                                    c_vp, c_vp, c_vp, c_vp]),
    "vit_router_head_bwd": (c_i32, [c_vp, c_vp, c_vp, c_vp, c_vp, c_vp, c_f32, c_i64, c_i64, c_i32, c_i64, c_i32, c_vp,
                                    c_vp]),
    "vit_splitk_reduce": (c_i32, [c_vp, c_i64, c_i64, c_i64, c_i64, c_vp, c_i64, c_i64, c_i32, c_vp]),
    "vit_layernorm_fwd": (c_i32, [c_vp, c_i64, c_vp, c_vp, c_vp, c_i64, c_i32, c_vp, c_vp, c_i64, c_i64, c_f32, c_vp]),
    "vit_layernorm_bwd_partial_rows": (c_i64, [c_i64]),
    "vit_layernorm_bwd_blocks": (c_i64, [c_i64]),
    "vit_layernorm_bwd": (c_i32, [c_vp, c_i64, c_i32, c_vp, c_i64, c_vp, c_vp, c_vp, c_vp, c_i64, c_vp, c_i64,
                                  c_vp, c_i64, c_vp, c_vp, c_vp, c_i32, c_i64, c_i64, ctypes.POINTER(Dropout),
                                  c_vp]),
    "vit_attention_fwd": (c_i32, [c_vp, c_vp, c_vp, c_i64, c_i64, c_i64, c_i64, c_f32, c_vp]),
    "vit_attention_bwd": (c_i32, [c_vp, c_vp, c_vp, c_vp, c_vp, c_vp, c_i64, c_i64, c_i64, c_i64, c_f32, c_vp]),
    "vit_attention_fwd_rows": (c_i32, [c_vp, c_vp, c_vp, c_i64, c_i64, c_i64, c_i64, c_f32, c_i64, c_vp]),
    "vit_attention_bwd_rows": (c_i32, [c_vp, c_vp, c_vp, c_vp, c_vp, c_vp, c_i64, c_i64, c_i64, c_i64, c_f32, c_i64,
                                       c_vp]),
    "vit_attention_bias_rows": (c_i64, [c_i64, c_i64, c_i32]),
    "vit_attention_workspace_elems": (c_i64, [c_i64, c_i64, c_i64, c_i32]),
    "vit_attention_fwd_ex": (c_i32, [c_vp, c_vp, c_vp, c_i64, c_i64, c_i64, c_i64, c_f32, c_i64, c_i32, c_vp]),
    "vit_attention_bwd_ex": (c_i32, [c_vp, c_vp, c_vp, c_vp, c_vp, c_vp, c_i64, c_i64, c_i64, c_i64, c_f32, c_i64,
                                     c_i32, c_vp, c_vp]),
    "vit_im2col": (c_i32, [c_vp, c_vp, c_i64, c_i64, c_i64, c_i64, c_vp]),
    "vit_im2col_hw": (c_i32, [c_vp, c_vp, c_i64, c_i64, c_i64, c_i64, c_i64, c_i64, c_vp]),
    "vit_preprocess_u8": (c_i32, [c_vp, c_i64, c_i64, c_i64, c_i64, c_vp, c_i64, c_i64, c_vp, c_vp, c_vp]),
    "vit_preprocess_u8_gather": (c_i32, [c_vp, c_i64, c_i32, c_i64, c_i64, c_i64, c_vp, c_i64, c_vp, c_i64, c_i64, c_vp,
                                         c_vp, c_vp, c_vp, c_vp]),
    "vit_embed_grad": (c_i32, [c_vp, c_i64, c_i64, c_i64, c_vp, c_vp, c_vp, ctypes.POINTER(Dropout), c_vp]),
    "vit_dropout_mask": (c_i32, [ctypes.POINTER(Dropout), c_i64, c_i64, c_i64, c_vp, c_i64, c_vp]),
    "vit_colsum_partial_rows": (c_i64, [c_i64]),
    "vit_colsum": (c_i32, [c_vp, c_i32, c_i64, c_i64, c_i64, c_vp, c_vp, c_i32, c_vp]),
    "vit_gemm_f32": (c_i32, [c_i64, c_i64, c_i64, c_vp, c_i64, c_i32, c_vp, c_i64, c_i32, c_vp, c_i64, c_vp, c_i32,
                             c_vp]),
    "vit_cross_entropy": (c_i32, [c_vp, c_vp, c_i64, c_i64, c_vp, c_f32, c_vp, c_vp]),
    "vit_sgd_step": (c_i32, [c_vp, c_vp, c_vp, c_vp, c_i64, c_f32, c_f32, c_f32, c_i32, c_vp]),
    "vit_cast_f32_bf16": (c_i32, [c_vp, c_vp, c_i64, c_vp]),
    "vit_cast_pad_rows": (c_i32, [c_vp, c_i64, c_i64, c_vp, c_i64, c_vp]),
    "vit_axpby": (c_i32, [c_vp, c_vp, c_i64, c_f32, c_f32, c_vp]),
    "vit_pack_cols": (c_i32, [c_vp, c_i64, c_i64, c_i64, c_i64, c_i64, c_vp, c_i64, c_i32, c_vp]),
    "vit_pack_cols_batched": (c_i32, [c_vp, c_i64, c_i64, c_i64, c_i64, c_i64, c_i64, c_vp, c_i64, c_i64, c_i32, c_i64,
                                      c_vp]),
    "vit_transpose_f32_bf16": (c_i32, [c_vp, c_i64, c_i64, c_i64, c_vp, c_i64, c_i64, c_i64, c_i64, c_vp]),
    "vit_colsum_batch": (c_i32, [ctypes.POINTER(ColsumJob), c_i32, c_vp]),
    "vit_colsum3": (c_i32, [c_vp, c_i32, c_i64, c_i64, c_i64, c_vp, c_vp, c_vp, c_vp, c_i32, c_vp]),
    "vit_im2col_f32": (c_i32, [c_vp, c_vp, c_i64, c_i64, c_i64, c_i64, c_vp]),
    "vit_im2col_hw_f32": (c_i32, [c_vp, c_vp, c_i64, c_i64, c_i64, c_i64, c_i64, c_i64, c_vp]),
    "vit_embed_fwd_f32": (c_i32, [c_vp, c_i64, c_i64, c_i64, c_vp, c_vp, c_vp]),
    "vit_gelu_f32": (c_i32, [c_vp, c_vp, c_i64, c_vp]),
    "vit_attention_fwd_f32": (c_i32, [c_vp, c_vp, c_i64, c_i64, c_i64, c_i64, c_f32, c_vp]),
    "vit_gelu_bwd_f32": (c_i32, [c_vp, c_vp, c_vp, c_i64, c_vp]),
    "vit_dropout_apply_f32": (c_i32, [ctypes.POINTER(Dropout), c_vp, c_vp, c_i64, c_i64, c_vp]),
    "vit_add_bcast_f32": (c_i32, [c_vp, c_vp, c_vp, c_i64, c_i64, c_vp]),
    "vit_unpack_bf16_f32": (c_i32, [c_vp, c_i64, c_i64, c_i64, c_vp, c_i64, c_vp]),
    "vit_attention_fwd_varlen": (c_i32, [c_vp, c_i64, c_vp, c_i64, c_vp, c_i64, c_vp, c_i64, c_vp, c_i64, c_i64, c_i64,
                                         c_i64, c_i64, c_f32, c_vp]),
    "vit_sqnorm_partial": (c_i32, [c_vp, c_i64, c_vp, c_i32, c_vp]),
    "vit_adamw_prep": (c_i32, [c_vp, c_i32, c_vp, c_vp, c_i32, c_f32, c_f32, c_f32, c_f32, c_vp, c_vp, c_vp]),
    "vit_adamw_update": (c_i32, [c_vp, c_vp, c_vp, c_vp, c_vp, c_vp, c_i32, c_vp, c_f32, c_f32, c_f32, c_f32, c_f32,
                                 c_f32, c_i32, c_vp]),
    "vit_adamw_chunk_elems": (c_i32, []),
    "vit_scale_by_coef": (c_i32, [c_vp, c_i64, c_vp, c_vp]),
    "vit_zero": (c_i32, [c_vp, c_i64, c_vp]),
    "vit_copy2d": (c_i32, [c_vp, c_i64, c_vp, c_i64, c_i64, c_i64, c_vp]),
    "vit_rows_select": (c_i32, [c_vp, c_i64, c_vp, c_i64, c_vp, c_i64, c_i64, c_vp]),
    "vit_sgd_step_dev": (c_i32, [c_vp, c_vp, c_vp, c_vp, c_i64, c_vp, c_f32, c_vp]),
    "vit_build_id": (ctypes.c_char_p, []),
}

EXPORTED = tuple(_SIGS)

_lib = None


class VitHipError(RuntimeError):
    pass


def load(path: str | None = None):
    global _lib
    if _lib is not None:
        return _lib
    p = path or LIB_PATH
    if not os.path.exists(p):
        raise VitHipError(f"libvit_hip.so not built ({p}); run `make -C vit-of-pytorch_amd` or __graft_entry__.build()")
    lib = ctypes.CDLL(p)
    for name, (res, args) in _SIGS.items():
        fn = getattr(lib, name)
        fn.restype = res
        fn.argtypes = args
    if lib.vit_abi_version() != ABI_VERSION:
        raise VitHipError(f"{p} has ABI {lib.vit_abi_version()}, the bindings expect {ABI_VERSION}: rebuild it "
                          "(make -C vit-of-pytorch_amd)")
    check_build_id(lib, p)
    _lib = lib
    return lib


def check_build_id(lib, path: str, expected: str | None = None):
    from . import buildid
    if expected is None:
        if not buildid.have_sources():
            return
        expected = buildid.tree_id()
    got = lib.vit_build_id().decode()
    if got != expected:
        raise VitHipError(f"{path} was built from other sources (build id {got}, this tree {expected}): rebuild it "
                          "(make -C vit-of-pytorch_amd)")


def check(status: int, what: str):
    if status != 0:
        msg = _lib.vit_last_error().decode(errors="replace") if _lib is not None else "?"
        raise VitHipError(f"{what} failed (status {status}): {msg}")
```

### vit-of-pytorch_amd/vitmi/engine.py

```python
from __future__ import annotations

import math
import os
from collections import OrderedDict
from dataclasses import dataclass

import torch

from . import ops
from ._lib import (EPI_BF16, EPI_BIAS_BF16, EPI_BIAS_GELU_DGELU, EPI_BIAS_RESID_F32, EPI_MUL_BF16, EPI_PATCH,
                   EPI_SPLITK, K_CONTIG, MN_CONTIG)

ALIGN = 64


def _rup(x, m):
    return (x + m - 1) // m * m


_NBUF = 2

_WGRAD_TARGET = int(os.environ.get("VIT_WGRAD_TARGET", "256"))


# ... 12 lines not shown
    mlp_dim: int = 3072
    num_heads: int = 12
    num_layers: int = 12
    num_classes: int = 1000

    def __post_init__(self):
        for f in ("image_size", "patch_size"):
            v = getattr(self, f)
            if not isinstance(v, int):
                object.__setattr__(self, f, _hw(v))

    @property
    def image_hw(self):
        return _hw(self.image_size)

    @property
    def patch_hw(self):
        return _hw(self.patch_size)

    @property
    def grid_hw(self):
        (h, w), (fh, fw) = self.image_hw, self.patch_hw
        return h // fh, w // fw

    @property
    def grid(self):
        gh, gw = self.grid_hw
        if gh != gw:
            raise ValueError(f"ArchConfig.grid is the side of a square patch grid; this one is {gh}x{gw} (use grid_hw)")
        return gh

    @property
    def tokens(self):
        gh, gw = self.grid_hw
        return gh * gw + 1

    @property
    def head_dim(self):
        return self.emb_dim // self.num_heads

    @property
    def patch_k(self):
        fh, fw = self.patch_hw
        return 3 * fh * fw


def layer_param_specs(cfg: ArchConfig, i: int):
    D, M, H = cfg.emb_dim, cfg.mlp_dim, cfg.num_heads
    hd = D // H
    p = f"transformer.encoder_layers.{i}."
    out = [(p + "norm1.weight", (D,)), (p + "norm1.bias", (D,))]
    for w in ("query", "key", "value"):
        out += [(p + f"attn.{w}.weight", (D, H, hd)), (p + f"attn.{w}.bias", (H, hd))]
    out += [(p + "attn.out.weight", (H, hd, D)), (p + "attn.out.bias", (D,))]
    out += [(p + "norm2.weight", (D,)), (p + "norm2.bias", (D,))]
    out += [(p + "mlp.fc1.weight", (M, D)), (p + "mlp.fc1.bias", (M,))]
    out += [(p + "mlp.fc2.weight", (D, M)), (p + "mlp.fc2.bias", (D,))]
    return out


def flat_param_specs(cfg: ArchConfig):
    D, C = cfg.emb_dim, cfg.num_classes
    specs = [("classifier.weight", (C, D)), ("classifier.bias", (C,)),
             ("transformer.norm.weight", (D,)), ("transformer.norm.bias", (D,))]
    for i in reversed(range(cfg.num_layers)):
        specs += layer_param_specs(cfg, i)
    specs += [("embedding.weight", (D, 3, *cfg.patch_hw)), ("embedding.bias", (D,)),
              ("transformer.pos_embedding.pos_embedding", (1, cfg.tokens, D)), ("cls_token", (1, 1, D))]
    return specs


class FlatLayout:
    def __init__(self, cfg: ArchConfig):
        self.cfg = cfg
        self.offsets = OrderedDict()
        self.shapes = OrderedDict()
        off = 0
        self.layer_ranges = {}
        for name, shape in flat_param_specs(cfg):
            n = math.prod(shape)
            self.offsets[name] = off
            self.shapes[name] = shape
            off = _rup(off + n, ALIGN)
        self.numel = off
        L = cfg.num_layers
        self.buckets = []
        self.buckets.append(("head", 0, self.offsets[self._lname(L - 1, "norm1.weight")]))
        for i in reversed(range(L)):
            start = self.offsets[self._lname(i, "norm1.weight")]
            end = self.offsets[self._lname(i - 1, "norm1.weight")] if i > 0 else self.offsets["embedding.weight"]
            self.buckets.append((f"layer{i}", start, end))
        self.buckets.append(("embed", self.offsets["embedding.weight"], self.numel))

    @staticmethod
    def _lname(i, s):
        return f"transformer.encoder_layers.{i}.{s}"

    def view(self, buf, name):
        o = self.offsets[name]
        shape = self.shapes[name]
        return buf[o:o + math.prod(shape)].view(shape)


class _Acts:

    def __init__(self, cfg: ArchConfig, b: int, dev):
        D, M, H, L, N = cfg.emb_dim, cfg.mlp_dim, cfg.num_heads, cfg.num_layers, cfg.tokens
        T = b * N
        Tp = _rup(T, 64)
        self.b, self.T, self.Tp = b, T, Tp
        z = lambda *s, dt=torch.bfloat16: torch.zeros(*s, device=dev, dtype=dt)
        f = torch.float32
        self.kpad = _rup(cfg.patch_k, 64)
        self.patches = z(Tp, self.kpad)
        self.h = [z(Tp, D, dt=f) for _ in range(L + 1)]
        self.hm = [z(Tp, D, dt=f) for _ in range(L)]
        self.ln1 = [z(Tp, D) for _ in range(L)]
        self.ln2 = [z(Tp, D) for _ in range(L)]
        self.mu1 = [z(T, dt=f) for _ in range(L)]
        self.rs1 = [z(T, dt=f) for _ in range(L)]
        self.mu2 = [z(T, dt=f) for _ in range(L)]
        self.rs2 = [z(T, dt=f) for _ in range(L)]
        self.qkv = [z(Tp, 3 * D) for _ in range(L)]
        self.o = [z(Tp, D) for _ in range(L)]
        self.lse = [z(b, H, N, dt=f) for _ in range(L)]
        self.gp = [z(Tp, M) for _ in range(L)]
        self.g = [z(Tp, M) for _ in range(L)]
        self.lncls = z(b, D, dt=f)
        self.muf = z(b, dt=f)
        self.rsf = z(b, dt=f)
        self.logits = z(b, cfg.num_classes, dt=f)
        self.dh = z(Tp, D, dt=f)
        self.dhb = [z(Tp, D), z(Tp, D)]
        self.dg = [z(Tp, M), z(Tp, M)]
        self.dyln = z(Tp, D)
        self.dO = z(Tp, D)
        self.dqkv = [z(Tp, 3 * D), z(Tp, 3 * D)]
        self.dlncls = z(b, D, dt=f)
        self.dlogits = z(b, cfg.num_classes, dt=f)
        self.row_stats = z(b, 3, dt=f)
        self.lnparts = [z(ops.layernorm_bwd_blocks(T), 3 * D, dt=f) for _ in range(_NBUF)]
        self.gelu_parts = [z(-(-T // 128), M, dt=f) for _ in range(_NBUF)]
        self.attn_bias_rows = ops.attention_bias_rows(N, D // H)
        self.qkv_bparts = [z(b * self.attn_bias_rows, 3 * D, dt=f) for _ in range(_NBUF)]
        nws = ops.attention_workspace_elems(b, N, H)
        self.attn_ws = z(nws, dt=f) if nws else None
        bp = _rup(b, 64)
        self.bp = bp
        self.c_o, self.c_ln2, self.c_dh, self.c_dh2, self.c_dyln = (z(bp, D) for _ in range(5))
        self.c_g, self.c_gp, self.c_dg = (z(bp, M) for _ in range(3))
        self.c_mu2, self.c_rs2 = z(b, dt=f), z(b, dt=f)
        self._cfg, self._dev = cfg, dev
        self.dhb_l = self.dg_l = self.dqkv_l = None

    def defer_bufs(self):
        if self.dhb_l is None:
            cfg = self._cfg
            D, M, L = cfg.emb_dim, cfg.mlp_dim, cfg.num_layers
            z = lambda *s: torch.zeros(*s, device=self._dev, dtype=torch.bfloat16)
            self.dhb_l = self.dhb + [z(self.Tp, D) for _ in range(2 * L - 1)]
            self.dg_l = self.dg + [z(self.Tp, M) for _ in range(max(L - 2, 0))]
            self.dqkv_l = self.dqkv + [z(self.Tp, 3 * D) for _ in range(max(L - 2, 0))]
        return self.dhb_l, self.dg_l, self.dqkv_l


class _BiasReducer:

    def __init__(self, eng, a):
        self.eng = eng
        self.a = a
        self.D = eng.cfg.emb_dim
        self.nxt = {}
        self.queued = {}
        self.jobs = []

    def buf(self, kind, bufs):
        n = self.queued.get(kind, 0)
        if n == len(bufs):
            self.flush()
            n = 0
        self.queued[kind] = n + 1
        i = self.nxt.get(kind, 0)
        self.nxt[kind] = (i + 1) % len(bufs)
        return bufs[i]

    def reduce(self, part, rows, cols, ld, outs, seg=0):
        self.jobs.append((part, rows, cols, ld, seg, outs, False))
        if len(self.jobs) == ops.COLSUM_BATCH_MAX:
            self.flush()

    def flush(self):
        if self.jobs:
            ops.colsum_batch(self.jobs)
            self.jobs = []
        self.queued.clear()

    def ln_bwd(self, dy, lddy, x, ldx, mean, rstd, gamma, dx, lddx, rows, dgamma_dbeta, dx_colsum, **kw):
        part = self.buf("ln", self.a.lnparts)
        D = self.D
        ops.layernorm_bwd(dy, lddy, x, ldx, mean, rstd, gamma, dx, lddx, part, rows, D, **kw)
        self.reduce(part, ops.layernorm_bwd_blocks(rows), 3 * D, 3 * D, (dgamma_dbeta, dgamma_dbeta[D:], dx_colsum),
                    seg=D)


class ViTEngine:

    def __init__(self, cfg: ArchConfig, device="cuda", flat: torch.Tensor | None = None):
        if cfg.emb_dim % cfg.num_heads:
            raise ValueError("emb_dim must be divisible by num_heads")
        if cfg.head_dim % 16 or cfg.head_dim > 96:
            raise NotImplementedError(f"head_dim {cfg.head_dim} not supported by the HIP attention kernel "
                                      "(multiples of 16 up to 96)")
        if cfg.emb_dim % 64 or cfg.mlp_dim % 64:
            raise NotImplementedError("emb_dim and mlp_dim must be multiples of 64")
        self.cfg = cfg
        self.dev = torch.device(device)
        self.attn_fwd_path = ops.ATTN_AUTO
        self.layout = FlatLayout(cfg)
        n = self.layout.numel
        self.flat = flat if flat is not None else torch.zeros(n, device=self.dev)
        self.grad = torch.zeros(n, device=self.dev)
        self.mirror = torch.zeros(n, device=self.dev, dtype=torch.bfloat16)
        D, L = cfg.emb_dim, cfg.num_layers
        M = cfg.mlp_dim
        bf = torch.bfloat16
        self.wqkv = torch.zeros(L, D, 3 * D, device=self.dev, dtype=bf)
        self.bqkv = torch.zeros(L, 3 * D, device=self.dev)
        kp = _rup(cfg.patch_k, 64)
        self.wconv = torch.zeros(D, kp, device=self.dev, dtype=torch.bfloat16) if kp != cfg.patch_k else None
        self._acts = {}
        self._mirror_sig = None
        o = [self.off(self.lname(i, "norm1.weight")) for i in range(L)]
        self.layer_stride = o[0] - o[1] if L > 1 else 0
        assert all(o[i] == o[0] - i * self.layer_stride for i in range(L))
        self._ws = None
        self.step_id = 0
        self.grad_ready_hook = None
        self.grad_ready_finish = None
        self.overlap_wgrad = os.environ.get("VITMI_OVERLAP", "0") == "1"
        self.group_wgrad = os.environ.get("VITMI_GROUP_WGRAD", "1") != "0"
        v = os.environ.get("VITMI_WGRAD_DEFER", "all")
        self.wgrad_defer = L if v == "all" else int(v)
        self._wgrad_tables = {}
        self.prune_last = os.environ.get("VITMI_PRUNE_LAST", "1") != "0"
        self._pruned = False
        self._side = None
        self._ev_pool, self._ev_next = [], 0
        self.probe = None
        self.probe_wgrad = None
        self.drop_seed = (torch.initial_seed() * 0x9E3779B97F4A7C15 + 0x632BE59BD9B4E019) & (2**64 - 1)
        self._drop_offset = 0
        self._drop = None

    def _event(self):
        if self._ev_next == len(self._ev_pool):
            self._ev_pool.append(torch.cuda.Event())
        ev = self._ev_pool[self._ev_next]
        self._ev_next += 1
        return ev

    def pv(self, name, buf=None):
        return self.layout.view(self.flat if buf is None else buf, name)

    def off(self, name):
        return self.layout.offsets[name]

    def lname(self, i, s):
        return f"transformer.encoder_layers.{i}.{s}"

    def load_params(self, params):
        for k, v in params.items():
            self.pv(k).copy_(v.to(self.dev, torch.float32).reshape(self.layout.shapes[k]))
        self.invalidate_mirror()

    def state(self):
        return OrderedDict((k, self.pv(k)) for k in self.layout.offsets)

    def invalidate_mirror(self):
        self._mirror_sig = None

    def refresh_mirror(self, full=True):
        cfg = self.cfg
        D = cfg.emb_dim
        if full:
            ops.cast_bf16(self.flat, self.mirror, self.layout.numel)
        M, L = cfg.mlp_dim, cfg.num_layers
        lst = self.layer_stride
        o0 = lambda s: self.off(self.lname(0, s))
        zs = self.off(self.lname(0, "attn.key.weight")) - o0("attn.query.weight")
        ops.pack_cols_batched(self.flat[o0("attn.query.weight"):], -lst, zs, D, D, D, 3, self.wqkv, D * 3 * D, 3 * D, L)
        ops.pack_cols_batched(self.flat[o0("attn.query.bias"):], -lst, zs, D, 1, D, 3, self.bqkv, 3 * D, 3 * D, L)
        if self.wconv is not None:
            w = self.off("embedding.weight")
            ops.cast_pad_rows(self.flat[w:], D, cfg.patch_k, self.wconv, self.wconv.shape[1])

    def mark_mirror_fresh(self, sig):
        self._mirror_sig = sig

    def acts(self, b):
        a = self._acts.get(b)
        if a is None:
            if len(self._acts) >= 2:
                self._acts.pop(next(iter(self._acts)))
            a = _Acts(self.cfg, b, self.dev)
            self._acts[b] = a
        return a

    def _splitk(self, M, N, K, z=1):
        return ops.splitk_factor(M, N, K, z, _WGRAD_TARGET)

    def _workspace(self, numel):
        if self._ws is None or self._ws.numel() < numel:
            self._ws = torch.empty(numel, device=self.dev)
        return self._ws

    def _wgrad(self, A, lda, B, ldb, M, N, K, out, ldo, batch=1, b_bs=0, out_bs=0):
        s = self._splitk(M, N, K, batch)
        ws = self._workspace(batch * s * M * N)
        if self.probe_wgrad is not None:
            ev0 = torch.cuda.Event(enable_timing=True)
            ev0.record()
        ops.gemm(A, B, ws, M, N, K, a_layout=MN_CONTIG, b_layout=MN_CONTIG, lda=lda, ldb=ldb, ldc=N,
                 epilogue=EPI_SPLITK, batch=batch, b_bs=b_bs, split_k=s)
        if self.probe_wgrad is not None:
            ev1 = torch.cuda.Event(enable_timing=True)
            ev1.record()
            self.probe_wgrad.append((ev0, ev1, 2.0 * M * N * K * batch, K, False))
        ops.splitk_reduce(ws, batch, s, M, N, out, ldo, out_bs)

    def _wgrad_group(self, specs):
        K = specs[0][6]
        assert all(sp[6] == K for sp in specs)
        s = ops.splitk_factor_group([(sp[4], sp[5], sp[9]) for sp in specs], K, _WGRAD_TARGET)
        sizes = [sp[9] * s * sp[4] * sp[5] for sp in specs]
        ws = self._workspace(sum(sizes))
        members, views, o = [], [], 0
        for sp, n in zip(specs, sizes):
            A, lda, B, ldb, M, N, _, _, _, batch, b_bs, _ = sp
            w = ws[o:o + n]
            o += n
            views.append(w)
            members.append((A, B, w, M, N, K, dict(a_layout=MN_CONTIG, b_layout=MN_CONTIG, lda=lda, ldb=ldb, ldc=N,
                                                    epilogue=EPI_SPLITK, batch=batch, b_bs=b_bs, split_k=s)))
        if self.probe_wgrad is not None:
            ev0 = torch.cuda.Event(enable_timing=True)
            ev0.record()
        ops.gemm_splitk_group(members)
        if self.probe_wgrad is not None:
            ev1 = torch.cuda.Event(enable_timing=True)
            ev1.record()
            self.probe_wgrad.append((ev0, ev1, sum(2.0 * sp[4] * sp[5] * K * sp[9] for sp in specs), K, True))
        ops.splitk_reduce_group([(w, sp[9], s, sp[4], sp[5], sp[7], sp[8], sp[11], False) for sp, w in zip(specs, views)])

    def _wgrad_batch(self, specs, slot):
        K = specs[0][6]
        assert all(sp[6] == K for sp in specs)
        s = ops.splitk_factor_group([(sp[4], sp[5], sp[9]) for sp in specs], K, _WGRAD_TARGET)
        views = None
        if s > 1:
            sizes = [sp[9] * s * sp[4] * sp[5] for sp in specs]
            ws = self._workspace(sum(sizes))
            views, o = [], 0
            for n in sizes:
                views.append(ws[o:o + n])
                o += n
        for c0 in range(0, len(specs), ops.GEMM_TABLE_MAX):
            part = specs[c0:c0 + ops.GEMM_TABLE_MAX]
            key = (s, self._ws.data_ptr() if s > 1 else 0) + tuple(
                (sp[0].data_ptr(), sp[1], sp[2].data_ptr(), sp[3], sp[4], sp[5], sp[7].data_ptr()) + tuple(sp[8:])
                for sp in part)
            ent = self._wgrad_tables.get((self._last_b, slot, c0))
            if ent is None or ent[0] != key:
                members = []
                for k, (A, lda, B, ldb, M, N, _, out, ldo, batch, b_bs, out_bs) in enumerate(part):
                    kw = dict(a_layout=MN_CONTIG, b_layout=MN_CONTIG, lda=lda, ldb=ldb, epilogue=EPI_SPLITK, batch=batch,
                              b_bs=b_bs, split_k=s)
                    if s == 1:
                        members.append((A, B, out, M, N, K, dict(kw, ldc=ldo, c_bs=out_bs), True))
                    else:
                        members.append((A, B, views[c0 + k], M, N, K, dict(kw, ldc=N), False))
                ent = (key, ops.GemmGroupTable(members))
                self._wgrad_tables[(self._last_b, slot, c0)] = ent
            if self.probe_wgrad is not None:
                ev0 = torch.cuda.Event(enable_timing=True)
                ev0.record()
            ent[1].launch()
            if self.probe_wgrad is not None:
                ev1 = torch.cuda.Event(enable_timing=True)
                ev1.record()
                self.probe_wgrad.append((ev0, ev1, sum(2.0 * sp[4] * sp[5] * K * sp[9] for sp in part), K, True))
        if s > 1:
            ops.splitk_reduce_group([(w, sp[9], s, sp[4], sp[5], sp[7], sp[8], sp[11], False)
                                     for sp, w in zip(specs, views)])

    def _dd(self, site, row_stride=1):
        if self._drop is None:
            return None
        p, seed, off = self._drop
        return ops.dropout_desc(p, site, seed, off, row_stride)

    def forward(self, x: torch.Tensor, dropout_p: float = 0.0):
        cfg = self.cfg
        if x.dim() != 4 or x.shape[1] != 3 or tuple(x.shape[2:]) != cfg.image_hw:
            raise ValueError(f"expected input [b, 3, {cfg.image_hw[0]}, {cfg.image_hw[1]}], got {tuple(x.shape)}")
        x = x.to(self.dev, torch.float32).contiguous()
        b = x.shape[0]
        a = self.acts(b)
        D, M, H, N, L = cfg.emb_dim, cfg.mlp_dim, cfg.num_heads, cfg.tokens, cfg.num_layers
        hd = D // H
        T = a.T
        mv = self.mirror
        f = self.flat
        if dropout_p and dropout_p > 0.0:
            if not dropout_p < 1.0:
                raise ValueError(f"dropout probability has to be in [0, 1), got {dropout_p}")
            self._drop_offset += 1
            self._drop = (float(dropout_p), self.drop_seed, self._drop_offset)
        else:
            self._drop = None
        dd = self._dd
        ops.im2col_hw(x, a.patches, b, *cfg.image_hw, *cfg.patch_hw, a.kpad)
        wconv = self.wconv if self.wconv is not None else mv[self.off("embedding.weight"):]
        ops.gemm(a.patches, wconv, a.h[0], T, D, a.kpad, a_layout=K_CONTIG, b_layout=K_CONTIG, lda=a.kpad,
                 ldb=a.kpad, ldc=D, epilogue=EPI_PATCH, bias=f[self.off("embedding.bias"):],
                 aux=f[self.off("transformer.pos_embedding.pos_embedding"):], ldaux=D,
                 aux2=f[self.off("cls_token"):], tokens=N, dropout=dd(0))
        scale = 1.0 / math.sqrt(hd)
        self._pruned = self.prune_last and self._drop is None
        for i in range(L):
            ln = lambda s: self.off(self.lname(i, s))
            ops.layernorm_fwd(a.h[i], D, f[ln("norm1.weight"):], f[ln("norm1.bias"):], a.ln1[i], D, a.mu1[i],
                              a.rs1[i], T, D)
            ops.gemm(a.ln1[i], self.wqkv[i], a.qkv[i], T, 3 * D, D, a_layout=K_CONTIG, b_layout=MN_CONTIG, lda=D,
                     ldb=3 * D, ldc=3 * D, epilogue=EPI_BIAS_BF16, bias=self.bqkv[i])
            last = self._pruned and i == L - 1
            ops.attention_fwd(a.qkv[i], a.o[i], a.lse[i], b, N, H, hd, scale, q_rows=1 if last else None,
                              path=self.attn_fwd_path)
            if last:
                self._forward_last_cls(a, i, b)
                break
            ops.gemm(a.o[i], mv[ln("attn.out.weight"):], a.hm[i], T, D, D, a_layout=K_CONTIG, b_layout=MN_CONTIG,
                     lda=D, ldb=D, ldc=D, epilogue=EPI_BIAS_RESID_F32, bias=f[ln("attn.out.bias"):], aux=a.h[i],
                     ldaux=D, dropout=dd(1 + 3 * i))
            ops.layernorm_fwd(a.hm[i], D, f[ln("norm2.weight"):], f[ln("norm2.bias"):], a.ln2[i], D, a.mu2[i],
                              a.rs2[i], T, D)
            if self.probe is not None:
                ev0 = torch.cuda.Event(enable_timing=True)
                ev0.record()
            ops.gemm(a.ln2[i], mv[ln("mlp.fc1.weight"):], a.gp[i], T, M, D, a_layout=K_CONTIG, b_layout=K_CONTIG,
                     lda=D, ldb=D, ldc=M, epilogue=EPI_BIAS_GELU_DGELU, bias=f[ln("mlp.fc1.bias"):], C2=a.g[i],
                     ldc2=M, dropout=dd(2 + 3 * i))
            if self.probe is not None:
                ev1 = torch.cuda.Event(enable_timing=True)
                ev1.record()
                self.probe.append((ev0, ev1))
            ops.gemm(a.g[i], mv[ln("mlp.fc2.weight"):], a.h[i + 1], T, D, M, a_layout=K_CONTIG, b_layout=K_CONTIG,
                     lda=M, ldb=M, ldc=D, epilogue=EPI_BIAS_RESID_F32, bias=f[ln("mlp.fc2.bias"):], aux=a.hm[i],
                     ldaux=D, dropout=dd(3 + 3 * i))
        ops.layernorm_fwd(a.h[L], N * D, f[self.off("transformer.norm.weight"):], f[self.off("transformer.norm.bias"):],
                          a.lncls, D, a.muf, a.rsf, b, D)
        C = cfg.num_classes
        ops.gemm_f32(b, C, D, a.lncls, D, False, f[self.off("classifier.weight"):], D, True, a.logits, C,
                     bias=f[self.off("classifier.bias"):])
        self.step_id += 1
        self._last_b = b
        return a.logits

    def _forward_last_cls(self, a, i, b):
        cfg = self.cfg
        D, M, N = cfg.emb_dim, cfg.mlp_dim, cfg.tokens
        f, mv = self.flat, self.mirror
        ln = lambda s: self.off(self.lname(i, s))
        S = N * D
        ops.gemm(a.o[i], mv[ln("attn.out.weight"):], a.hm[i], b, D, D, a_layout=K_CONTIG, b_layout=MN_CONTIG, lda=S,
                 ldb=D, ldc=S, epilogue=EPI_BIAS_RESID_F32, bias=f[ln("attn.out.bias"):], aux=a.h[i], ldaux=S)
        ops.copy2d(a.c_o, D * 2, a.o[i], S * 2, D * 2, b)
        ops.layernorm_fwd(a.hm[i], S, f[ln("norm2.weight"):], f[ln("norm2.bias"):], a.c_ln2, D, a.c_mu2, a.c_rs2,
                          b, D)
        ops.gemm(a.c_ln2, mv[ln("mlp.fc1.weight"):], a.c_gp, b, M, D, a_layout=K_CONTIG, b_layout=K_CONTIG, lda=D,
                 ldb=D, ldc=M, epilogue=EPI_BIAS_GELU_DGELU, bias=f[ln("mlp.fc1.bias"):], C2=a.c_g, ldc2=M)
        ops.gemm(a.c_g, mv[ln("mlp.fc2.weight"):], a.h[i + 1], b, D, M, a_layout=K_CONTIG, b_layout=K_CONTIG,
                 lda=M, ldb=M, ldc=S, epilogue=EPI_BIAS_RESID_F32, bias=f[ln("mlp.fc2.bias"):], aux=a.hm[i], ldaux=S)

    def _backward_last_cls(self, a, i, b, g, on_side, bias):
        cfg = self.cfg
        D, M, N = cfg.emb_dim, cfg.mlp_dim, cfg.tokens
        S = N * D
        f, mv = self.flat, self.mirror
        gv = lambda name: g[self.off(self.lname(i, name)):]
        bp = a.bp
        on_side(lambda: self._wgrad(a.c_dh, D, a.c_g, M, D, M, bp, gv("mlp.fc2.weight"), M))
        gpart = bias.buf("gelu", a.gelu_parts)
        w2 = mv[self.off(self.lname(i, "mlp.fc2.weight")):]
        kw = dict(a_layout=K_CONTIG, b_layout=MN_CONTIG, lda=D, ldb=M, ldc=M, epilogue=EPI_MUL_BF16, aux=a.c_gp,
                  ldaux=M, col_partial=gpart)
        ops.gemm(a.c_dh, w2, a.c_dg, b, M, D, **kw)
        tiles_m = ops.gemm_partial_rows(a.c_dh, w2, a.c_dg, b, M, D, **kw)
        bias.reduce(gpart, tiles_m, M, M, (gv("mlp.fc1.bias"),))
        on_side(lambda: self._wgrad(a.c_dg, M, a.c_ln2, D, M, D, bp, gv("mlp.fc1.weight"), D))
        ops.gemm(a.c_dg, mv[self.off(self.lname(i, "mlp.fc1.weight")):], a.c_dyln, b, D, M, a_layout=K_CONTIG,
                 b_layout=MN_CONTIG, lda=M, ldb=D, ldc=D, epilogue=EPI_BF16)
        bias.ln_bwd(a.c_dyln, D, a.hm[i], S, a.c_mu2, a.c_rs2, f[self.off(self.lname(i, "norm2.weight")):], a.dh, S, b,
                    gv("norm2.weight"), gv("attn.out.bias"), dres=a.dh, lddres=S, dx_bf16=a.c_dh2, lddxb=D)
        on_side(lambda: self._wgrad(a.c_o, D, a.c_dh2, D, D, D, bp, gv("attn.out.weight"), D))
        ops.zero_(a.dO)
        ops.gemm(a.c_dh2, mv[self.off(self.lname(i, "attn.out.weight")):], a.dO, b, D, D, a_layout=K_CONTIG,
                 b_layout=K_CONTIG, lda=D, ldb=D, ldc=S, epilogue=EPI_BF16)

    def forward_exact(self, x: torch.Tensor):
        cfg = self.cfg
        if x.dim() != 4 or x.shape[1] != 3 or tuple(x.shape[2:]) != cfg.image_hw:
            raise ValueError(f"expected input [b, 3, {cfg.image_hw[0]}, {cfg.image_hw[1]}], got {tuple(x.shape)}")
        x = x.to(self.dev, torch.float32).contiguous()
        b = x.shape[0]
        D, M, H, N, L, C = cfg.emb_dim, cfg.mlp_dim, cfg.num_heads, cfg.tokens, cfg.num_layers, cfg.num_classes
        hd = D // H
        T, kp = b * N, cfg.patch_k
        f = self.flat
        e = lambda *shape: torch.empty(*shape, device=self.dev)
        fv = lambda name: f[self.off(name):]
        patches = e(T, kp)
        ops.im2col_hw_f32(x, patches, b, *cfg.image_hw, *cfg.patch_hw, kp)
        h = e(T, D)
        ops.gemm_f32(T, D, kp, patches, kp, False, fv("embedding.weight"), kp, True, h, D, bias=fv("embedding.bias"))
        ops.embed_fwd_f32(h, b, N, D, fv("transformer.pos_embedding.pos_embedding"), fv("cls_token"))
        y, qkv, o, u = e(T, D), e(T, 3 * D), e(T, D), e(T, M)
        mu, rs = e(T), e(T)
        for i in range(L):
            ln = lambda s: fv(self.lname(i, s))
            ops.layernorm_fwd(h, D, ln("norm1.weight"), ln("norm1.bias"), y, D, mu, rs, T, D)
            for z, w in enumerate(("query", "key", "value")):
                ops.gemm_f32(T, D, D, y, D, False, ln(f"attn.{w}.weight"), D, False, qkv[:, z * D:], 3 * D,
                             bias=ln(f"attn.{w}.bias"))
            ops.attention_fwd_f32(qkv, o, b, N, H, hd, 1.0 / math.sqrt(hd))
            ops.gemm_f32(T, D, D, o, D, False, ln("attn.out.weight"), D, False, h, D, bias=ln("attn.out.bias"),
                         accumulate=True)
            ops.layernorm_fwd(h, D, ln("norm2.weight"), ln("norm2.bias"), y, D, mu, rs, T, D)
            ops.gemm_f32(T, M, D, y, D, False, ln("mlp.fc1.weight"), D, True, u, M, bias=ln("mlp.fc1.bias"))
            ops.gelu_f32(u, u, T * M)
            ops.gemm_f32(T, D, M, u, M, False, ln("mlp.fc2.weight"), M, True, h, D, bias=ln("mlp.fc2.bias"),
                         accumulate=True)
        lncls = e(b, D)
        ops.layernorm_fwd(h, N * D, fv("transformer.norm.weight"), fv("transformer.norm.bias"), lncls, D, mu, rs, b, D)
        logits = e(b, C)
        ops.gemm_f32(b, C, D, lncls, D, False, fv("classifier.weight"), D, True, logits, C, bias=fv("classifier.bias"))
        return logits

    def cross_entropy(self, labels: torch.Tensor, grad_scale: float | None = None):
        a = self.acts(self._last_b)
        gs = 1.0 / a.b if grad_scale is None else grad_scale
        ops.cross_entropy(a.logits, labels.to(self.dev, torch.int64).contiguous(), a.dlogits, gs, a.row_stats)
        return a.dlogits, a.row_stats

    def backward(self, dlogits: torch.Tensor, grad: torch.Tensor | None = None):
        cfg = self.cfg
        b = self._last_b
        a = self.acts(b)
        g = self.grad if grad is None else grad
        D, M, H, N, L, C = cfg.emb_dim, cfg.mlp_dim, cfg.num_heads, cfg.tokens, cfg.num_layers, cfg.num_classes
        hd = D // H
        T = a.T
        f = self.flat
        mv = self.mirror
        gv = lambda name: g[self.off(name):]
        dl = dlogits.to(self.dev, torch.float32).contiguous()
        hook = self.grad_ready_hook
        dd = self._dd
        main = torch.cuda.current_stream(self.dev)
        overlap = self.overlap_wgrad
        if overlap and self._side is None:
            self._side = torch.cuda.Stream(device=self.dev)
        side = self._side if overlap else main
        free_ev = {}

        def on_side(fn):
            if not overlap:
                fn()
                return
            ev = self._event()
            ev.record(main)
            side.wait_event(ev)
            with torch.cuda.stream(side):
                fn()

        def release(kind, idx):
            if overlap:
                ev = self._event()
                ev.record(side)
                free_ev[(kind, idx)] = ev

        def acquire(kind, idx):
            ev = free_ev.pop((kind, idx), None)
            if ev is not None:
                main.wait_event(ev)

        def fire(bucket):
            bias.flush()
            if not hook:
                return
            evs = []
            for st in ((main, side) if overlap else (main,)):
                ev = self._event()
                ev.record(st)
                evs.append(ev)
            hook(g, *bucket, evs)

        self._ev_next = 0
        group = self.group_wgrad and D >= 256
        defer = self.wgrad_defer if not hook and not overlap and D >= 256 and M >= 256 else 0
        pending, held, launches = [], 0, 0
        dhbs, dgs, dqkvs = a.defer_bufs() if defer else (a.dhb, a.dg, a.dqkv)
        nd = len(dhbs)

        def flush_wgrad():
            nonlocal pending, held, launches
            if pending:
                self._wgrad_batch(pending, launches)
                launches += 1
            pending, held = [], 0
        out_wb = None
        bias = _BiasReducer(self, a)
        ops.gemm_f32(C, D, b, dl, C, True, a.lncls, D, False, gv("classifier.weight"), D)
        bias.reduce(dl, b, C, C, (gv("classifier.bias"),))
        ops.gemm_f32(b, D, C, dl, C, False, f[self.off("classifier.weight"):], D, False, a.dlncls, D)
        wb = 0
        pruned = self._pruned
        ops.zero_(a.dh)
        if not pruned:
            ops.zero_(dhbs[wb])
        bias.ln_bwd(a.dlncls, D, a.h[L], N * D, a.muf, a.rsf, f[self.off("transformer.norm.weight"):], a.dh, N * D, b,
                    gv("transformer.norm.weight"), gv(self.lname(L - 1, "mlp.fc2.bias")),
                    dx_bf16=a.c_dh if pruned else dhbs[wb], lddxb=D if pruned else N * D,
                    dx_dropout=dd(3 + 3 * (L - 1), N))
        fire(self.layout.buckets[0])
        scale = 1.0 / math.sqrt(hd)
        for i in reversed(range(L)):
            ln = lambda s: self.off(self.lname(i, s))
            li = i % len(dgs)
            if pruned and i == L - 1:
                self._backward_last_cls(a, i, b, g, on_side, bias)
                wb = (wb + 1) % nd
            else:
                dhb = dhbs[wb]
                if defer:
                    pending.append((dhb, D, a.g[i], M, D, M, a.Tp, gv(self.lname(i, "mlp.fc2.weight")), M, 1, 0, 0))
                else:
                    on_side(lambda: self._wgrad(dhb, D, a.g[i], M, D, M, a.Tp, gv(self.lname(i, "mlp.fc2.weight")), M))
                release("dhb", wb)
                dg = dgs[li]
                acquire("dg", li)
                gpart = bias.buf("gelu", a.gelu_parts)
                w2 = mv[ln("mlp.fc2.weight"):]
                kw = dict(a_layout=K_CONTIG, b_layout=MN_CONTIG, lda=D, ldb=M, ldc=M, epilogue=EPI_MUL_BF16, aux=a.gp[i],
                          ldaux=M, col_partial=gpart)
                ops.gemm(dhb, w2, dg, T, M, D, **kw)
                tiles_m = ops.gemm_partial_rows(dhb, w2, dg, T, M, D, **kw)
                bias.reduce(gpart, tiles_m, M, M, (gv(self.lname(i, "mlp.fc1.bias")),))
                if defer:
                    pending.append((dg, M, a.ln2[i], D, M, D, a.Tp, gv(self.lname(i, "mlp.fc1.weight")), D, 1, 0, 0))
                else:
                    on_side(lambda: self._wgrad(dg, M, a.ln2[i], D, M, D, a.Tp, gv(self.lname(i, "mlp.fc1.weight")), D))
                release("dg", li)
                ops.gemm(dg, mv[ln("mlp.fc1.weight"):], a.dyln, T, D, M, a_layout=K_CONTIG, b_layout=MN_CONTIG, lda=M,
                         ldb=D, ldc=D, epilogue=EPI_BF16)
                wb = (wb + 1) % nd
                acquire("dhb", wb)
                dhb = dhbs[wb]
                bias.ln_bwd(a.dyln, D, a.hm[i], D, a.mu2[i], a.rs2[i], f[ln("norm2.weight"):], a.dh, D, T,
                            gv(self.lname(i, "norm2.weight")), gv(self.lname(i, "attn.out.bias")),
                            dres=a.dh, lddres=D, dx_bf16=dhb, lddxb=D, dx_dropout=dd(1 + 3 * i))
                out_spec = (a.o[i], D, dhb, D, D, D, a.Tp, gv(self.lname(i, "attn.out.weight")), D, 1, 0, 0)
                if defer:
                    pending.append(out_spec)
                elif group:
                    out_wb = wb
                else:
                    on_side(lambda: self._wgrad(*out_spec[:9]))
                    release("dhb", wb)
                ops.gemm(dhb, mv[ln("attn.out.weight"):], a.dO, T, D, D, a_layout=K_CONTIG, b_layout=K_CONTIG, lda=D,
                         ldb=D, ldc=D, epilogue=EPI_BF16)
            dqkv = dqkvs[li]
            acquire("dqkv", li)
            qpart = bias.buf("qkv", a.qkv_bparts)
            ops.attention_bwd(a.qkv[i], a.o[i], a.dO, a.lse[i], dqkv, b, N, H, hd, scale, bias_partial=qpart,
                              q_rows=1 if pruned and i == L - 1 else None, workspace=a.attn_ws)
            qo = ln("attn.query.weight")
            zs = ln("attn.key.weight") - qo
            qb = ln("attn.query.bias")
            bias.reduce(qpart, b * a.attn_bias_rows, 3 * D, 3 * D, (g[qb:], g[qb + zs:], g[qb + 2 * zs:]), seg=D)
            qkv_spec = (a.ln1[i], D, dqkv, 3 * D, D, D, a.Tp, g[qo:], D, 3, D, zs)
            if defer:
                pending.append(qkv_spec)
                held += 1
                if held == defer and i > 0:
                    flush_wgrad()
            elif out_wb is not None:
                on_side(lambda: self._wgrad_group([out_spec, qkv_spec]))
                release("dqkv", li)
                release("dhb", out_wb)
                out_wb = None
            else:
                on_side(lambda: self._wgrad(*qkv_spec[:9], batch=3, b_bs=D, out_bs=zs))
                release("dqkv", li)
            ops.gemm(dqkv, self.wqkv[i], a.dyln, T, D, 3 * D, a_layout=K_CONTIG, b_layout=K_CONTIG, lda=3 * D,
                     ldb=3 * D, ldc=D, epilogue=EPI_BF16)
            wb = (wb + 1) % nd
            acquire("dhb", wb)
            bias.ln_bwd(a.dyln, D, a.h[i], D, a.mu1[i], a.rs1[i], f[ln("norm1.weight"):], a.dh, D, T,
                        gv(self.lname(i, "norm1.weight")), gv(self.lname(i - 1, "mlp.fc2.bias")) if i > 0 else None,
                        dres=a.dh, lddres=D, dx_bf16=dhbs[wb], lddxb=D,
                        dx_dropout=dd(3 + 3 * (i - 1)) if i > 0 else dd(0))
            fire(self.layout.buckets[L - i])
        dhb = dhbs[wb]
        if defer and cfg.patch_k >= 256:
            pending.append((dhb, D, a.patches, a.kpad, D, cfg.patch_k, a.Tp, gv("embedding.weight"), cfg.patch_k, 1, 0, 0))
        else:
            on_side(lambda: self._wgrad(dhb, D, a.patches, a.kpad, D, cfg.patch_k, a.Tp, gv("embedding.weight"),
                                        cfg.patch_k))
        flush_wgrad()
        ops.embed_grad(a.dh, b, N, D, gv("transformer.pos_embedding.pos_embedding"), gv("cls_token"),
                       gv("embedding.bias"), dropout=dd(0))
        fire(self.layout.buckets[-1])
        bias.flush()
        if overlap:
            main.wait_stream(side)
        return g
```

### vit-of-pytorch_amd/vitmi/ops.py

```python
from __future__ import annotations

import ctypes

import torch

from . import _lib
from ._lib import COLSUM_BATCH_MAX, Dropout, GemmArgs, check

BF16 = torch.bfloat16
F32 = torch.float32


def lib():
    return _lib.load()


def _stream():
    return ctypes.c_void_p(torch.cuda.current_stream().cuda_stream)


def _p(t):
    return ctypes.c_void_p(0 if t is None else t.data_ptr())


# ... 74 lines not shown
    return int(lib().vit_gemm_partial_rows(ctypes.byref(_gemm_args(A, B, C, M, N, K, **kw))))


def splitk_reduce(ws, batch, split, M, N, out, ldo, out_bs=0, accumulate=False):
    _chk(ws, F32, "ws")
    _chk(out, F32, "out")
    check(lib().vit_splitk_reduce(_p(ws), batch, split, M, N, _p(out), ldo, out_bs, int(accumulate), _stream()),
          "vit_splitk_reduce")


def splitk_reduce_group(jobs):
    for k in range(0, len(jobs), _lib.SPLITK_GROUP_MAX):
        part = jobs[k:k + _lib.SPLITK_GROUP_MAX]
        arr = (_lib.SplitkJob * len(part))()
        for i, (ws, batch, split, M, N, out, ldo, out_bs, acc) in enumerate(part):
            _chk(ws, F32, "ws")
            _chk(out, F32, "out")
            arr[i] = _lib.SplitkJob(_p(ws), batch, split, M, N, _p(out), ldo, out_bs, int(acc), 0)
        check(lib().vit_splitk_reduce_group(arr, len(part), _stream()), "vit_splitk_reduce_group")


def layernorm_fwd(x, ldx, gamma, beta, y, ldy, mean, rstd, rows, D, eps=1e-5):
    _chk(x, F32, "x")
    check(lib().vit_layernorm_fwd(_p(x), ldx, _p(gamma), _p(beta), _p(y), ldy, int(y.dtype == F32), _p(mean),
                                  _p(rstd), rows, D, eps, _stream()), "vit_layernorm_fwd")


def layernorm_bwd_partial_rows(rows):
    return int(lib().vit_layernorm_bwd_partial_rows(rows))


def layernorm_bwd_blocks(rows):
    return int(lib().vit_layernorm_bwd_blocks(rows))


def layernorm_bwd(dy, lddy, x, ldx, mean, rstd, gamma, dx, lddx, partial, rows, D, *, dres=None, lddres=0,
                  dx_bf16=None, lddxb=0, dgamma_dbeta=None, dx_colsum=None, accumulate=False, dx_dropout=None):
    check(lib().vit_layernorm_bwd(_p(dy), lddy, int(dy.dtype == F32), _p(x), ldx, _p(mean), _p(rstd), _p(gamma),
                                  _p(dres), lddres, _p(dx), lddx, _p(dx_bf16), lddxb, _p(partial), _p(dgamma_dbeta),
                                  _p(dx_colsum), int(accumulate), rows, D, _dp(dx_dropout), _stream()),
          "vit_layernorm_bwd")


ATTN_AUTO, ATTN_RESIDENT, ATTN_TILED, ATTN_ONESHOT = 0, 1, 2, 3


def attention_bias_rows(N, hd, path=ATTN_AUTO):
    return int(lib().vit_attention_bias_rows(N, hd, path))


def attention_workspace_elems(B, N, H, path=ATTN_AUTO):
    return int(lib().vit_attention_workspace_elems(B, N, H, path))


def attention_fwd(qkv, o, lse, B, N, H, hd, scale, q_rows=None, path=ATTN_AUTO):
    _chk(qkv, BF16, "qkv")
    _chk(o, BF16, "o")
    _chk(lse, F32, "lse")
    check(lib().vit_attention_fwd_ex(_p(qkv), _p(o), _p(lse), B, N, H, hd, scale, N if q_rows is None else q_rows,
                                     path, _stream()), "vit_attention_fwd")


def attention_bwd(qkv, o, dout, lse, dqkv, B, N, H, hd, scale, bias_partial=None, q_rows=None, path=ATTN_AUTO,
                  workspace=None):
    _chk(workspace, F32, "workspace")
    need = attention_workspace_elems(B, N, H, path)
    if need and (workspace is None or workspace.numel() < need):
        if workspace is not None:
            raise ValueError(f"attention workspace has {workspace.numel()} floats, needs {need}")
        workspace = torch.empty(need, device=qkv.device, dtype=F32)
    check(lib().vit_attention_bwd_ex(_p(qkv), _p(o), _p(dout), _p(lse), _p(dqkv), _p(bias_partial), B, N, H, hd,
                                     scale, N if q_rows is None else q_rows, path, _p(workspace if need else None),
                                     _stream()), "vit_attention_bwd")


def im2col(x, out, B, img, P, Kpad):
    _chk(x, F32, "x")
    _chk(out, BF16, "out")
    check(lib().vit_im2col(_p(x), _p(out), B, img, P, Kpad, _stream()), "vit_im2col")


def im2col_hw(x, out, B, H, W, Ph, Pw, Kpad):
    _chk(x, F32, "x")
    _chk(out, BF16, "out")
    check(lib().vit_im2col_hw(_p(x), _p(out), B, H, W, Ph, Pw, Kpad, _stream()), "vit_im2col_hw")


def preprocess_u8(images, out, flips=None, mean=(0.5, 0.5, 0.5), std=(0.5, 0.5, 0.5)):
    _chk(images, torch.uint8, "images")
    _chk(out, F32, "out")
    _chk(flips, torch.uint8, "flips")
    if images.dim() != 4 or images.shape[3] != 3 or out.dim() != 4 or out.shape[1] != 3:
        raise ValueError(f"preprocess_u8: images [B,H,W,3] -> out [B,3,h,w], got {tuple(images.shape)} -> "
                         f"{tuple(out.shape)}")
    B, H, W, _ = images.shape
    if out.shape[0] != B or (flips is not None and flips.numel() != B):
        raise ValueError("preprocess_u8: batch mismatch")
    if images[0].stride() != (W * 3, 3, 1) or not out.is_contiguous():
        raise ValueError("preprocess_u8: images must have contiguous [H, W, 3] rows and out must be contiguous")
    ms = (ctypes.c_float * 6)(*[float(v) for v in mean], *[float(v) for v in std])
    check(lib().vit_preprocess_u8(_p(images), B, H, W, images.stride(0) if B > 1 else H * W * 3, _p(flips),
                                  out.shape[2], out.shape[3], ms, _p(out), _stream()), "vit_preprocess_u8")


IMAGES_HWC, IMAGES_CHW = 0, 1


def preprocess_u8_gather(images, index, out, flips=None, mean=(0.5, 0.5, 0.5), std=(0.5, 0.5, 0.5), layout=IMAGES_HWC,
                         labels_in=None, labels_out=None, image_stride=None):
    _chk(images, torch.uint8, "images")
    _chk(index, torch.int64, "index")
    _chk(out, F32, "out")
    _chk(flips, torch.uint8, "flips")
    _chk(labels_in, torch.int64, "labels_in")
    _chk(labels_out, torch.int64, "labels_out")
    chw = layout == IMAGES_CHW
    if images.dim() != 4 or images.shape[1 if chw else 3] != 3 or out.dim() != 4 or out.shape[1] != 3:
        raise ValueError(f"preprocess_u8_gather: images {'[n,3,H,W]' if chw else '[n,H,W,3]'} -> out [B,3,h,w], got "
                         f"{tuple(images.shape)} -> {tuple(out.shape)}")
    n = images.shape[0]
    H, W = (images.shape[2], images.shape[3]) if chw else (images.shape[1], images.shape[2])
    B = out.shape[0]
    if index.dim() != 1 or index.numel() != B or (flips is not None and flips.numel() != B) or \
            (labels_out is not None and labels_out.numel() != B) or (labels_in is not None and labels_in.numel() != n):
        raise ValueError("preprocess_u8_gather: batch mismatch")
    if n and images[0].stride() != ((H * W, W, 1) if chw else (W * 3, 3, 1)) or not out.is_contiguous():
        raise ValueError("preprocess_u8_gather: every image must be contiguous and out must be contiguous")
    for name, t in (("index", index), ("flips", flips), ("labels_in", labels_in), ("labels_out", labels_out)):
        if t is not None and not t.is_contiguous():
            raise ValueError(f"preprocess_u8_gather: {name} must be contiguous")
    if image_stride is None:
        image_stride = images.stride(0) if n > 1 else H * W * 3
    ms = (ctypes.c_float * 6)(*[float(v) for v in mean], *[float(v) for v in std])
    check(lib().vit_preprocess_u8_gather(_p(images), n, int(layout), H, W, int(image_stride), _p(index), B, _p(flips),
                                         out.shape[2], out.shape[3], ms, _p(out), _p(labels_in), _p(labels_out),
                                         _stream()), "vit_preprocess_u8_gather")


def embed_grad(dh0, B, N, D, dpos, dcls, dconv_bias, dropout=None):
    check(lib().vit_embed_grad(_p(dh0), B, N, D, _p(dpos), _p(dcls), _p(dconv_bias), _dp(dropout), _stream()),
          "vit_embed_grad")


def colsum_partial_rows(rows):
    return int(lib().vit_colsum_partial_rows(rows))


def colsum(inp, rows, cols, ld, partial, out, accumulate=False):
    check(lib().vit_colsum(_p(inp), int(inp.dtype == BF16), rows, cols, ld, _p(partial), _p(out), int(accumulate),
                           _stream()), "vit_colsum")


def colsum_batch(jobs):
    arr = (_lib.ColsumJob * len(jobs))()
    for k, (inp, rows, cols, ld, seg, outs, acc) in enumerate(jobs):
        if inp.dtype != F32:
            raise ValueError("colsum_batch: f32 inputs only")
        o = list(outs) + [None] * (3 - len(outs))
        arr[k] = _lib.ColsumJob(_p(inp), rows, cols, ld, seg, _p(o[0]), _p(o[1]), _p(o[2]), int(acc), 0)
    check(lib().vit_colsum_batch(arr, len(jobs), _stream()), "vit_colsum_batch")


def gemm_f32(M, N, K, A, lda, a_trans, B, ldb, b_trans, C, ldc, bias=None, accumulate=False):
    check(lib().vit_gemm_f32(M, N, K, _p(A), lda, int(a_trans), _p(B), ldb, int(b_trans), _p(C), ldc, _p(bias),
                             int(accumulate), _stream()), "vit_gemm_f32")


def cross_entropy(logits, labels, dlogits, grad_scale, row_stats):
    _chk(logits, F32, "logits")
    _chk(labels, torch.int64, "labels")
    B, C = logits.shape
    check(lib().vit_cross_entropy(_p(logits), _p(labels), B, C, _p(dlogits), grad_scale, _p(row_stats), _stream()),
          "vit_cross_entropy")


def sgd_step(p, g, buf, p_bf16, n, lr, momentum, wd, first):
    check(lib().vit_sgd_step(_p(p), _p(g), _p(buf), _p(p_bf16), n, lr, momentum, wd, int(first), _stream()),
          "vit_sgd_step")


def cast_bf16(inp, out, n):
    check(lib().vit_cast_f32_bf16(_p(inp), _p(out), n, _stream()), "vit_cast_f32_bf16")


def cast_pad_rows(inp, rows, cols, out, ldo):
    check(lib().vit_cast_pad_rows(_p(inp), rows, cols, _p(out), ldo, _stream()), "vit_cast_pad_rows")


def cast_pad_batch(jobs):
    for k in range(0, len(jobs), _lib.CAST_BATCH_MAX):
        part = jobs[k:k + _lib.CAST_BATCH_MAX]
        arr = (_lib.CastJob * len(part))()
        for i, (inp, rows, cols, ldi, out, ldo, rows_pad, cols_pad) in enumerate(part):
            _chk(inp, F32, "inp")
            _chk(out, BF16, "out")
            arr[i] = _lib.CastJob(_p(inp), rows, cols, ldi, _p(out), ldo, rows_pad, cols_pad)
        check(lib().vit_cast_pad_batch(arr, len(part), _stream()), "vit_cast_pad_batch")


def axpby(x, y, n, a, b):
    check(lib().vit_axpby(_p(x), _p(y), n, a, b, _stream()), "vit_axpby")


def pack_cols(inp, zstride, ldi, rows, cols, Z, out, ldo):
    check(lib().vit_pack_cols(_p(inp), zstride, ldi, rows, cols, Z, _p(out), ldo, int(out.dtype == BF16), _stream()),
          "vit_pack_cols")


def pack_cols_batched(inp, in_bs, zstride, ldi, rows, cols, Z, out, out_bs, ldo, batch):
    check(lib().vit_pack_cols_batched(_p(inp), in_bs, zstride, ldi, rows, cols, Z, _p(out), out_bs, ldo,
                                      int(out.dtype == BF16), batch, _stream()), "vit_pack_cols_batched")


def transpose_bf16(inp, rows, cols, ldi, out, ldo, batch=1, in_bs=0, out_bs=0):
    _chk(out, BF16, "out")
    check(lib().vit_transpose_f32_bf16(_p(inp), rows, cols, ldi, _p(out), ldo, batch, in_bs, out_bs, _stream()),
          "vit_transpose_f32_bf16")


def colsum3(inp, rows, seg, ld, partial, out0, out1, out2, accumulate=False):
    check(lib().vit_colsum3(_p(inp), int(inp.dtype == BF16), rows, seg, ld, _p(partial), _p(out0), _p(out1), _p(out2),
                            int(accumulate), _stream()), "vit_colsum3")


def im2col_f32(x, out, B, img, P, Kpad):
    _chk(x, F32, "x")
    _chk(out, F32, "out")
    check(lib().vit_im2col_f32(_p(x), _p(out), B, img, P, Kpad, _stream()), "vit_im2col_f32")


def im2col_hw_f32(x, out, B, H, W, Ph, Pw, Kpad):
    _chk(x, F32, "x")
    _chk(out, F32, "out")
    check(lib().vit_im2col_hw_f32(_p(x), _p(out), B, H, W, Ph, Pw, Kpad, _stream()), "vit_im2col_hw_f32")


def embed_fwd_f32(h, B, N, D, pos, cls):
    check(lib().vit_embed_fwd_f32(_p(h), B, N, D, _p(pos), _p(cls), _stream()), "vit_embed_fwd_f32")


def gelu_f32(inp, out, n):
    check(lib().vit_gelu_f32(_p(inp), _p(out), n, _stream()), "vit_gelu_f32")


def attention_fwd_f32(qkv, o, B, N, H, hd, inv_sqrt_hd):
    _chk(qkv, F32, "qkv")
    _chk(o, F32, "o")
    check(lib().vit_attention_fwd_f32(_p(qkv), _p(o), B, N, H, hd, inv_sqrt_hd, _stream()), "vit_attention_fwd_f32")


def gelu_bwd_f32(u, dy, dx, n):
    check(lib().vit_gelu_bwd_f32(_p(u), _p(dy), _p(dx), n, _stream()), "vit_gelu_bwd_f32")


def dropout_apply_f32(d, inp, out, rows, cols):
    check(lib().vit_dropout_apply_f32(_dp(d), _p(inp), _p(out), rows, cols, _stream()), "vit_dropout_apply_f32")


def add_bcast_f32(x, y, out, outer, inner):
    check(lib().vit_add_bcast_f32(_p(x), _p(y), _p(out), outer, inner, _stream()), "vit_add_bcast_f32")


def segment_colsum(inp, ld, segs, seg_rows, cols, out, ldo, seg_stride=None, row0=0, scale=1.0):
    _chk(out, F32, "out")
    st = seg_rows if seg_stride is None else seg_stride
    check(lib().vit_segment_colsum(_p(inp), int(inp.dtype == BF16), ld, segs, st, row0, seg_rows, cols, float(scale),
                                   _p(out), ldo, _stream()), "vit_segment_colsum")


def segment_colsum_bcast(inp, ld, segs, seg_rows, cols, out, ldo, bc, ldbc, bc_rows, seg_stride=None, row0=0,
                         scale=1.0):
    _chk(out, F32, "out")
    _chk(bc, BF16, "bc")
    st = seg_rows if seg_stride is None else seg_stride
    check(lib().vit_segment_colsum_bcast(_p(inp), int(inp.dtype == BF16), ld, segs, st, row0, seg_rows, cols,
                                         float(scale), _p(out), ldo, _p(bc), ldbc, bc_rows, _stream()),
          "vit_segment_colsum_bcast")


def router_dx_gate_partial_rows(rows_pad):
    return int(lib().vit_router_dx_gate_partial_rows(rows_pad))


def router_dx_gate(dx, ldx, g, ldg, g_scale, gp, ldgp, T, N, reserve, cols, out, ldo, col_partial=None, ldp=0):
    _chk(dx, F32, "dx")
    _chk(g, F32, "g")
    _chk(gp, BF16, "gp")
    _chk(out, BF16, "out")
    check(lib().vit_router_dx_gate(_p(dx), ldx, _p(g), ldg, float(g_scale), _p(gp), ldgp, T, N, reserve, cols, _p(out),
                                   ldo, out.shape[0], out.shape[1], _p(col_partial), ldp, _stream()),
          "vit_router_dx_gate")


def router_head_fwd(logits, noise, noise_mode, yhard, N, reserve, training, norm):
    _chk(logits, F32, "logits")
    T, bs = logits.shape[0], logits.shape[1]
    for t, n in ((noise, "noise"), (yhard, "yhard")):
        if t is not None:
            _chk(t, F32, n)
            if tuple(t.shape) != tuple(logits.shape):
                raise ValueError(f"router_head_fwd: {n} shape {tuple(t.shape)} != logits {tuple(logits.shape)}")
    dev = logits.device
    soft, hard = torch.empty_like(logits), torch.empty_like(logits)
    ysoft = torch.empty_like(logits) if training else None
    idx = torch.empty(T, device=dev, dtype=F32)
    part = torch.empty(max(int(lib().vit_router_head_partials(T)), 1), device=dev, dtype=F32)
    ent = torch.empty((), device=dev, dtype=F32)
    check(lib().vit_router_head_fwd(_p(logits), _p(noise), int(noise_mode), _p(yhard), T, N, bs, reserve, int(training),
                                    float(norm), _p(soft), _p(ysoft), _p(hard), _p(idx), _p(part), _p(ent), _stream()),
          "vit_router_head_fwd")
    return soft, ysoft, hard, idx, ent


def router_head_bwd(soft, ysoft, dsoft, dhard, dind, dent, N, reserve, training, norm):
    _chk(soft, F32, "soft")
    for t, n in ((ysoft, "ysoft"), (dsoft, "dsoft"), (dhard, "dhard"), (dind, "dind"), (dent, "dent")):
        if t is not None:
            _chk(t, F32, n)
    T, bs = soft.shape[0], soft.shape[1]
    dl = torch.empty_like(soft)
    check(lib().vit_router_head_bwd(_p(soft), _p(ysoft), _p(dsoft), _p(dhard), _p(dind), _p(dent), float(norm), T, N,
                                    bs, reserve, int(training), _p(dl), _stream()), "vit_router_head_bwd")
    return dl


def cls_mse(x, ldx, t, ldt, B, D, return_part=False):
    _chk(x, F32, "x")
    _chk(t, F32, "t")
    e = torch.empty(B, D, device=x.device, dtype=F32)
    part = torch.empty(B, device=x.device, dtype=F32)
    loss = torch.empty((), device=x.device, dtype=F32)
    check(lib().vit_cls_mse(_p(x), ldx, _p(t), ldt, B, D, _p(e), _p(part), _p(loss), _stream()), "vit_cls_mse")
    return (loss, e, part) if return_part else (loss, e)


def cls_mse_bwd(dx, lddx, e, g):
    _chk(dx, F32, "dx")
    _chk(e, F32, "e")
    _chk(g, F32, "g")
    check(lib().vit_cls_mse_bwd(_p(dx), lddx, _p(e), e.shape[0], e.shape[1], _p(g), _stream()), "vit_cls_mse_bwd")


def router_select(indices, active_sets, nkeys):
    _chk(indices, F32, "indices")
    if not indices.is_contiguous():
        raise ValueError("router_select: indices must be contiguous")
    T, dev = indices.numel(), indices.device
    masks = []
    for st in active_sets:
        m = 0
        for v in st:
            if not 0 <= int(v) < 32:
                raise ValueError(f"router_select: index value {v} outside [0, 32)")
            m |= 1 << int(v)
        masks.append(m)
    active = torch.empty(len(masks), T, device=dev, dtype=torch.bool)
    sel = torch.empty(nkeys, T, device=dev, dtype=torch.bool)
    anyf = torch.empty(nkeys, device=dev, dtype=torch.bool)
    arr = (ctypes.c_uint32 * max(len(masks), 1))(*masks)
    check(lib().vit_router_select(_p(indices), T, len(masks), arr, nkeys, _p(active), _p(sel), _p(anyf), _stream()),
          "vit_router_select")
    return active, sel, anyf


def cast_rows_masked(inp, ldi, rows, cols, mask, out, ldo):
    _chk(inp, F32, "inp")
    _chk(out, BF16, "out")
    if mask is not None and (mask.dtype != torch.bool or not mask.is_contiguous() or mask.numel() != rows):
        raise ValueError("cast_rows_masked: mask must be a contiguous bool tensor of `rows` elements")
    check(lib().vit_cast_rows_masked(_p(inp), ldi, rows, cols, _p(mask), _p(out), ldo, _stream()),
          "vit_cast_rows_masked")


def unpack_bf16_f32(inp, ldi, rows, cols, out, ldo):
    _chk(inp, BF16, "inp")
    _chk(out, F32, "out")
    check(lib().vit_unpack_bf16_f32(_p(inp), ldi, rows, cols, _p(out), ldo, _stream()), "vit_unpack_bf16_f32")


def attention_fwd_varlen(q, ldq, k, ldk, v, ldv, o, ldo, cu_q, B, max_q, Nkv, H, hd, scale):
    for t, n in ((q, "q"), (k, "k"), (v, "v"), (o, "o")):
        _chk(t, BF16, n)
    _chk(cu_q, torch.int32, "cu_q")
    check(lib().vit_attention_fwd_varlen(_p(q), ldq, _p(k), ldk, _p(v), ldv, _p(o), ldo, _p(cu_q), B, max_q, Nkv, H,
                                         hd, scale, _stream()), "vit_attention_fwd_varlen")


def sqnorm_partial(g, n, partial):
    _chk(g, F32, "g")
    _chk(partial, torch.float64, "partial")
    check(lib().vit_sqnorm_partial(_p(g), n, _p(partial), partial.numel(), _stream()), "vit_sqnorm_partial")


def adamw_prep(partial, used, steps, lr, beta1, beta2, max_norm, table, norm_out):
    nseg = 0 if steps is None else steps.numel()
    check(lib().vit_adamw_prep(_p(partial), 0 if partial is None else partial.numel(), _p(used), _p(steps), nseg,
                               lr, beta1, beta2, max_norm, _p(table), _p(norm_out), _stream()), "vit_adamw_prep")


def adamw_update(p, g, m, v, p_bf16, chunks, table, lr, beta1, beta2, eps, wd, write_grad):
    check(lib().vit_adamw_update(_p(p), _p(g), _p(m), _p(v), _p(p_bf16), _p(chunks), chunks.numel() // 3, _p(table),
                                 1.0 - lr * wd, beta1, beta2, 1.0 - beta1, 1.0 - beta2, eps, int(write_grad),
                                 _stream()), "vit_adamw_update")


def adamw_chunk_elems():
    return lib().vit_adamw_chunk_elems()


def scale_by_coef(g, n, coef):
    check(lib().vit_scale_by_coef(_p(g), n, _p(coef), _stream()), "vit_scale_by_coef")


def zero_(t):
    if not t.is_contiguous():
        raise ValueError("zero_: contiguous tensor expected")
    check(lib().vit_zero(_p(t), t.numel() * t.element_size(), _stream()), "vit_zero")


def splitk_factor_group(shapes, K, cus=256):
    tiles = sum(-(-M // 256) * -(-N // 256) * b for M, N, b in shapes)
    smax = max(1, min((K // 64) // 8, 32))
    t_tile = 2.0 * 256 * 256 * K / 4.0e12
    slab = sum(2.0 * M * N * 4 * b for M, N, b in shapes) / 5.0e12
    best, best_t = 1, None
    for s in range(1, smax + 1):
        t = -(-tiles * s // cus) * t_tile / s + s * slab
        if best_t is None or t < best_t * (1 - 1e-9):
            best, best_t = s, t
    return best


def gemm_splitk_group(members):
    if not 1 <= len(members) <= 4:
        raise ValueError("gemm_splitk_group: 1 to 4 members")
    arr = (GemmArgs * len(members))()
    for i, (A, B, C, M, N, K, kw) in enumerate(members):
        _chk(A, BF16, "A")
        _chk(B, BF16, "B")
        arr[i] = _gemm_args(A, B, C, M, N, K, **kw)
    check(lib().vit_gemm_splitk_group(arr, len(members), _stream()), "vit_gemm_splitk_group")


GEMM_TABLE_MAX = 128


class GemmGroupTable:

    def __init__(self, members):
        n = len(members)
        if not 1 <= n <= GEMM_TABLE_MAX:
            raise ValueError(f"GemmGroupTable: 1 to {GEMM_TABLE_MAX} members")
        arr = (GemmArgs * n)()
        direct = (ctypes.c_int32 * n)()
        for i, (A, B, C, M, N, K, kw, d) in enumerate(members):
            _chk(A, BF16, "A")
            _chk(B, BF16, "B")
            _chk(C, F32, "C")
            arr[i] = _gemm_args(A, B, C, M, N, K, **kw)
            direct[i] = int(bool(d))
        nbytes = int(lib().vit_gemm_group_table_bytes(n))
        self.table = torch.empty(nbytes, device=members[0][0].device, dtype=torch.uint8)
        total = ctypes.c_int32(0)
        check(lib().vit_gemm_group_prepare(arr, direct, n, _p(self.table), nbytes, ctypes.byref(total), _stream()),
              "vit_gemm_group_prepare")
        self.n, self.total = n, int(total.value)

    def launch(self):
        check(lib().vit_gemm_group_launch(_p(self.table), self.n, self.total, _stream()), "vit_gemm_group_launch")


def splitk_factor(M, N, K, batch=1, cus=256):
    tile = 256 if M >= 256 and N >= 256 else 128
    slots = cus if tile == 256 else 2 * cus
    tiles = -(-M // tile) * -(-N // tile) * batch
    smax = max(1, min((K // 64) // 8, 32))
    t_tile = 2.0 * tile * tile * K / 4.0e12
    slab = 2.0 * M * N * 4 * batch / 5.0e12
    best, best_t = 1, None
    for s in range(1, smax + 1):
        t = -(-tiles * s // slots) * t_tile / s + s * slab
        if best_t is None or t < best_t * (1 - 1e-9):
            best, best_t = s, t
    return best


def wgrad(A, lda, B, ldb, M, N, K, out, ldo, accumulate=False, batch=1, a_bs=0, b_bs=0, out_bs=0, target=256):
    from ._lib import EPI_SPLITK, MN_CONTIG
    s = splitk_factor(M, N, K, batch, target)
    ws = torch.empty(batch * s * M * N, device=out.device, dtype=F32)
    gemm(A, B, ws, M, N, K, a_layout=MN_CONTIG, b_layout=MN_CONTIG, lda=lda, ldb=ldb, ldc=N, epilogue=EPI_SPLITK,
         batch=batch, a_bs=a_bs, b_bs=b_bs, split_k=s)
    splitk_reduce(ws, batch, s, M, N, out, ldo, out_bs, accumulate)


def rows_select(dst, mask, src=None):
    if mask.dtype != torch.bool or not mask.is_contiguous() or mask.numel() != dst.shape[0]:
        raise ValueError("rows_select: mask must be a contiguous bool tensor of dst.shape[0] elements")
    rb = dst.shape[1] * dst.element_size()
    if src is not None and (src.dtype != dst.dtype or src.shape[1] != dst.shape[1]):
        raise ValueError("rows_select: src must match dst's dtype and row width")
    check(lib().vit_rows_select(_p(dst), dst.stride(0) * dst.element_size(), _p(src),
                                0 if src is None else src.stride(0) * src.element_size(), _p(mask), dst.shape[0], rb,
                                _stream()), "vit_rows_select")


def copy2d(dst, dpitch, src, spitch, width, height):
    check(lib().vit_copy2d(_p(dst), dpitch, _p(src), spitch, width, height, _stream()), "vit_copy2d")


def sgd_step_dev(p, g, buf, p_bf16, n, hyper, wd):
    _chk(hyper, F32, "hyper")
    check(lib().vit_sgd_step_dev(_p(p), _p(g), _p(buf), _p(p_bf16), n, _p(hyper), wd, _stream()), "vit_sgd_step_dev")
```

Baseline: 7674 images/sec.

## Fuse deferred bias column-sum jobs into grouped wgrad GEMM launch as filler work

Bias-gradient column-sum jobs in the backward pass are now deferred and packed into the grouped weight-gradient GEMM table as extra filler workgroups, instead of going out as separate colsum_batch launches. A new fill-table prepare/launch API builds unit descriptors that pair colsum jobs with the GEMM workgroups, and the colsum body is shared through a device header. The aim is to cut kernel launches and use idle CUs in the tail of the grouped GEMM. In exchange the table build is more complex, the table cache key now includes the filler jobs, and overlapping output ranges must be checked.

```diff
diff --git a/include/vit_hip.h b/include/vit_hip.h
--- a/include/vit_hip.h
+++ b/include/vit_hip.h
@@ -86,6 +86,15 @@
 int vit_gemm_group_prepare(const vit_gemm_args* args, const int32_t* direct, int32_t n, void* table,
                            int64_t table_bytes, int32_t* total, vit_stream_t stream);
 int vit_gemm_group_launch(const void* table, int32_t n, int32_t total, vit_stream_t stream);
+#define VIT_GEMM_FILL_JOBS_MAX 1024
+struct vit_colsum_job;
+int64_t vit_gemm_group_fill_table_bytes(int32_t n, const struct vit_colsum_job* jobs, const int32_t* chain,
+                                        int32_t njobs);
+int vit_gemm_group_fill_prepare(const vit_gemm_args* args, const int32_t* direct, int32_t n,
+                                const struct vit_colsum_job* jobs, const int32_t* chain, int32_t njobs, void* table,
+                                int64_t table_bytes, int32_t* total, int32_t* n_units, vit_stream_t stream);
+int vit_gemm_group_fill_launch(const void* table, int32_t n, int32_t total, int32_t njobs, int32_t n_units,
+                               vit_stream_t stream);
 
 int vit_splitk_reduce(const float* ws, int64_t batch, int64_t split, int64_t M, int64_t N,
                       float* out, int64_t ldo, int64_t out_batch_stride, int32_t accumulate,
diff --git a/vit-of-pytorch_amd/csrc/capi.hip b/vit-of-pytorch_amd/csrc/capi.hip
--- a/vit-of-pytorch_amd/csrc/capi.hip
+++ b/vit-of-pytorch_amd/csrc/capi.hip
@@ -21,5 +21,5 @@
 }
 
 extern "C" const char* vit_last_error(void) { return vit::g_last_error; }
-extern "C" int vit_abi_version(void) { return 21; }
+extern "C" int vit_abi_version(void) { return 22; }
 extern "C" const char* vit_build_id(void) { return VIT_BUILD_ID; }
diff --git a/vit-of-pytorch_amd/csrc/colsum_dev.h b/vit-of-pytorch_amd/csrc/colsum_dev.h
--- /dev/null
+++ b/vit-of-pytorch_amd/csrc/colsum_dev.h
@@ -0,0 +1,110 @@
+#pragma once
+#include "common.h"
+
+namespace vitc {
+
+struct ColsumJobDev {
+  const float* in;
+  float* out[3];
+  long ld;
+  int rows, cols, seg, acc, blk0;
+  int pad;
+};
+
+inline int make_colsum_dev(const vit_colsum_job& s, int k, const char* who, ColsumJobDev& d) {
+  VIT_CHECK_ARG(s.in && s.rows >= 1 && s.cols >= 1 && s.ld >= s.cols && s.rows <= 0x7fffffff && s.cols <= 0x7fffffff,
+                "%s: job %d: bad shape (rows %lld, cols %lld, ld %lld)", who, k, (long long)s.rows, (long long)s.cols,
+                (long long)s.ld);
+  VIT_CHECK_ARG(s.seg >= 0 && (s.seg == 0 || s.cols <= 3 * s.seg), "%s: job %d: seg %lld", who, k, (long long)s.seg);
+  VIT_CHECK_ARG(s.out0 || s.out1 || s.out2, "%s: job %d has no output", who, k);
+  d.in = s.in;
+  d.out[0] = s.out0;
+  d.out[1] = s.out1;
+  d.out[2] = s.out2;
+  d.ld = (long)s.ld;
+  d.rows = (int)s.rows;
+  d.cols = (int)s.cols;
+  d.seg = (int)s.seg;
+  d.acc = s.accumulate ? 1 : 0;
+  d.blk0 = 0;
+  d.pad = (s.cols % 4 == 0 && s.ld % 4 == 0 && ((uintptr_t)s.in % 16) == 0) ? 1 : 0;
+  return VIT_OK;
+}
+
+constexpr int COLSUM_RED_BYTES = 16 * 17 * (int)sizeof(float4);
+
+__device__ __forceinline__ void colsum_block(const ColsumJobDev& J, const int c0, const int t, float4 (*red)[17],
+                                             const bool active) {
+  const int cg = t & 15, rl = t >> 4;
+  const int c = c0 + cg * 4;
+  float4 acc = {0.f, 0.f, 0.f, 0.f};
+  if (active && J.pad && c < J.cols) {
+    const float* p = J.in + c;
+    const long ld = J.ld;
+    int r = rl;
+    for (; r + 112 < J.rows; r += 128) {
+      float4 v[8];
+#pragma unroll
+      for (int u = 0; u < 8; ++u) v[u] = *reinterpret_cast<const float4*>(p + (long)(r + 16 * u) * ld);
+#pragma unroll
+      for (int u = 0; u < 8; ++u) {
+        acc.x += v[u].x; acc.y += v[u].y; acc.z += v[u].z; acc.w += v[u].w;
+      }
+    }
+    for (; r < J.rows; r += 16) {
+      const float4 v = *reinterpret_cast<const float4*>(p + (long)r * ld);
+      acc.x += v.x; acc.y += v.y; acc.z += v.z; acc.w += v.w;
+    }
+  } else if (active && c < J.cols) {
+    const float* p = J.in + c;
+    const int nc = J.cols - c < 4 ? J.cols - c : 4;
+    for (int r = rl; r < J.rows; r += 16) {
+      const float* q = p + (long)r * J.ld;
+      acc.x += q[0];
+      if (nc > 1) acc.y += q[1];
+      if (nc > 2) acc.z += q[2];
+      if (nc > 3) acc.w += q[3];
+    }
+  }
+  red[rl][cg] = acc;
+  __syncthreads();
+  if (active && t < 64) {
+    const int g = t >> 2, k = t & 3;
+    const int col = c0 + t;
+    if (col < J.cols) {
+      float s = 0.f;
+#pragma unroll
+      for (int q = 0; q < 16; ++q) s += reinterpret_cast<const float*>(&red[q][g])[k];
+      const int sg = J.seg > 0 ? col / J.seg : 0;
+      float* base = J.out[sg];
+      if (base) {
+        float* dst = base + (col - sg * J.seg);
+        *dst = J.acc ? *dst + s : s;
+      }
+    }
+  }
+}
+
+struct FillUnitDev {
+  int job, blk, len, pad;
+};
+
+__device__ __forceinline__ void colsum_fill_workgroup(const ColsumJobDev* __restrict__ jobs,
+                                                      const FillUnitDev* __restrict__ units, const int n_units,
+                                                      const int fw, char* lds) {
+  const int half = __builtin_amdgcn_readfirstlane((int)threadIdx.x >> 8), t = threadIdx.x & 255;
+  const int u0 = 2 * fw, u = u0 + half;
+  const bool have = u < n_units;
+  const FillUnitDev mine = have ? units[u] : FillUnitDev{0, 0, 0, 0};
+  const int len0 = u0 < n_units ? units[u0].len : 0, len1 = u0 + 1 < n_units ? units[u0 + 1].len : 0;
+  const int steps = len0 > len1 ? len0 : len1;
+  float4(*red)[17] = reinterpret_cast<float4(*)[17]>(lds + half * COLSUM_RED_BYTES);
+  for (int s = 0; s < steps; ++s) {
+    const bool active = have && s < mine.len;
+    const int jx = __builtin_amdgcn_readfirstlane(active ? mine.job + s : 0);
+    if (s > 0) __syncthreads();
+    colsum_block(jobs[jx], mine.blk * 64, t, red, active);
+  }
+}
+
+}
diff --git a/vit-of-pytorch_amd/csrc/elementwise.hip b/vit-of-pytorch_amd/csrc/elementwise.hip
--- a/vit-of-pytorch_amd/csrc/elementwise.hip
+++ b/vit-of-pytorch_amd/csrc/elementwise.hip
@@ -1,4 +1,5 @@
 #include "common.h"
+#include "colsum_dev.h"
 
 namespace {
 
@@ -543,13 +544,7 @@
 }
 
 namespace {
-struct ColsumJobDev {
-  const float* in;
-  float* out[3];
-  long ld;
-  int rows, cols, seg, acc, blk0;
-  int pad;
-};
+using vitc::ColsumJobDev;
 struct ColsumBatchDev {
   ColsumJobDev j[VIT_COLSUM_BATCH_MAX];
   int n;
@@ -563,55 +558,7 @@
   for (int k = 1; k < VIT_COLSUM_BATCH_MAX; ++k)
     if (k < bt.n && bid >= bt.j[k].blk0) jx = k;
   const ColsumJobDev& J = bt.j[jx];
-  const int c0 = (bid - J.blk0) * 64;
-  const int cg = threadIdx.x & 15, rl = threadIdx.x >> 4;
-  const int c = c0 + cg * 4;
-  float4 acc = {0.f, 0.f, 0.f, 0.f};
-  if (J.pad && c < J.cols) {
-    const float* p = J.in + c;
-    const long ld = J.ld;
-    int r = rl;
-    for (; r + 112 < J.rows; r += 128) {
-      float4 v[8];
-#pragma unroll
-      for (int u = 0; u < 8; ++u) v[u] = *reinterpret_cast<const float4*>(p + (long)(r + 16 * u) * ld);
-#pragma unroll
-      for (int u = 0; u < 8; ++u) {
-        acc.x += v[u].x; acc.y += v[u].y; acc.z += v[u].z; acc.w += v[u].w;
-      }
-    }
-    for (; r < J.rows; r += 16) {
-      const float4 v = *reinterpret_cast<const float4*>(p + (long)r * ld);
-      acc.x += v.x; acc.y += v.y; acc.z += v.z; acc.w += v.w;
-    }
-  } else if (c < J.cols) {
-    const float* p = J.in + c;
-    const int nc = J.cols - c < 4 ? J.cols - c : 4;
-    for (int r = rl; r < J.rows; r += 16) {
-      const float* q = p + (long)r * J.ld;
-      acc.x += q[0];
-      if (nc > 1) acc.y += q[1];
-      if (nc > 2) acc.z += q[2];
-      if (nc > 3) acc.w += q[3];
-    }
-  }
-  red[rl][cg] = acc;
-  __syncthreads();
-  if (threadIdx.x < 64) {
-    const int g = threadIdx.x >> 2, k = threadIdx.x & 3;
-    const int col = c0 + threadIdx.x;
-    if (col < J.cols) {
-      float s = 0.f;
-#pragma unroll
-      for (int q = 0; q < 16; ++q) s += reinterpret_cast<const float*>(&red[q][g])[k];
-      const int sg = J.seg > 0 ? col / J.seg : 0;
-      float* base = J.out[sg];
-      if (base) {
-        float* dst = base + (col - sg * J.seg);
-        *dst = J.acc ? *dst + s : s;
-      }
-    }
-  }
+  vitc::colsum_block(J, (bid - J.blk0) * 64, threadIdx.x, red, true);
 }
 }
 
@@ -621,27 +568,9 @@
   ColsumBatchDev bt{};
   int blk = 0;
   for (int k = 0; k < njobs; ++k) {
-    const vit_colsum_job& s = jobs[k];
-    VIT_CHECK_ARG(s.in && s.rows >= 1 && s.cols >= 1 && s.ld >= s.cols && s.rows <= 0x7fffffff &&
-                      s.cols <= 0x7fffffff,
-                  "vit_colsum_batch: job %d: bad shape (rows %lld, cols %lld, ld %lld)", k, (long long)s.rows,
-                  (long long)s.cols, (long long)s.ld);
-    VIT_CHECK_ARG(s.seg >= 0 && (s.seg == 0 || s.cols <= 3 * s.seg), "vit_colsum_batch: job %d: seg %lld", k,
-                  (long long)s.seg);
-    VIT_CHECK_ARG(s.out0 || s.out1 || s.out2, "vit_colsum_batch: job %d has no output", k);
-    ColsumJobDev& d = bt.j[k];
-    d.in = s.in;
-    d.out[0] = s.out0;
-    d.out[1] = s.out1;
-    d.out[2] = s.out2;
-    d.ld = (long)s.ld;
-    d.rows = (int)s.rows;
-    d.cols = (int)s.cols;
-    d.seg = (int)s.seg;
-    d.acc = s.accumulate ? 1 : 0;
-    d.blk0 = blk;
-    d.pad = (s.cols % 4 == 0 && s.ld % 4 == 0 && ((uintptr_t)s.in % 16) == 0) ? 1 : 0;
-    blk += (int)((s.cols + 63) / 64);
+    if (const int rc = vitc::make_colsum_dev(jobs[k], k, "vit_colsum_batch", bt.j[k])) return rc;
+    bt.j[k].blk0 = blk;
+    blk += (int)((jobs[k].cols + 63) / 64);
   }
   bt.n = njobs;
   hipLaunchKernelGGL(colsum_batch_kernel, dim3(blk), dim3(256), 0, (hipStream_t)stream, bt);
diff --git a/vit-of-pytorch_amd/csrc/gemm.hip b/vit-of-pytorch_amd/csrc/gemm.hip
--- a/vit-of-pytorch_amd/csrc/gemm.hip
+++ b/vit-of-pytorch_amd/csrc/gemm.hip
@@ -277,17 +277,11 @@
   return n >= 1 && n <= vitg::GEMM_TABLE_MAX ? (int64_t)vitg::group_table_bytes(n) : 0;
 }
 
-extern "C" int vit_gemm_group_prepare(const vit_gemm_args* args, const int32_t* direct, int32_t n, void* table,
-                                      int64_t table_bytes, int32_t* total_out, vit_stream_t stream) {
-  VIT_CHECK_ARG(args != nullptr && n >= 1 && n <= vitg::GEMM_TABLE_MAX, "vit_gemm_group_prepare: 1..%d members, got %d",
-                vitg::GEMM_TABLE_MAX, n);
-  VIT_CHECK_ARG(table != nullptr && total_out != nullptr && table_bytes >= (int64_t)vitg::group_table_bytes(n) &&
-                    ((uintptr_t)table % 16) == 0,
-                "vit_gemm_group_prepare: needs a 16-byte aligned table of vit_gemm_group_table_bytes(n) bytes");
+namespace {
+int build_group_members(const vit_gemm_args* args, const int32_t* direct, int32_t n, char* host, int32_t* total_out) {
   const size_t soff = vitg::group_table_start_off(n);
-  std::vector<char> host(vitg::group_table_bytes(n), 0);
-  GemmDev* g = reinterpret_cast<GemmDev*>(host.data());
-  int* start = reinterpret_cast<int*>(host.data() + soff);
+  GemmDev* g = reinterpret_cast<GemmDev*>(host);
+  int* start = reinterpret_cast<int*>(host + soff);
   long total = 0;
   for (int i = 0; i < n; ++i) {
     const vit_gemm_args* a = args + i;
@@ -310,19 +304,128 @@
     VIT_CHECK_ARG(total < (1L << 30), "vit_gemm_group_prepare: grid too large");
   }
   start[n] = (int)total;
-  hipStream_t s = (hipStream_t)stream;
-  if (const int rc = vit::check_hip(hipStreamSynchronize(s), "vit_gemm_group_prepare sync")) return rc;
-  if (const int rc = vit::check_hip(hipMemcpy(table, host.data(), host.size(), hipMemcpyHostToDevice),
-                                    "vit_gemm_group_prepare upload"))
-    return rc;
   *total_out = (int32_t)total;
+  return VIT_OK;
+}
+
+int upload_table(void* table, const std::vector<char>& host, vit_stream_t stream, const char* who) {
+  if (const int rc = vit::check_hip(hipStreamSynchronize((hipStream_t)stream), who)) return rc;
+  return vit::check_hip(hipMemcpy(table, host.data(), host.size(), hipMemcpyHostToDevice), who);
+}
+
+void fill_out_range(const vit_colsum_job& j, int k, uintptr_t& lo, uintptr_t& hi) {
+  const float* o = k == 0 ? j.out0 : k == 1 ? j.out1 : j.out2;
+  long w = 0;
+  if (j.seg == 0)
+    w = k == 0 ? (long)j.cols : 0;
+  else
+    w = j.cols - k * j.seg < 0 ? 0 : (j.cols - k * j.seg < j.seg ? j.cols - k * j.seg : j.seg);
+  lo = (uintptr_t)o;
+  hi = o ? lo + (uintptr_t)w * sizeof(float) : lo;
+}
+
+long fill_unit_count(const vit_colsum_job* jobs, const int32_t* chain, int32_t njobs) {
+  if (njobs < 0 || njobs > VIT_GEMM_FILL_JOBS_MAX || (njobs > 0 && !jobs)) return -1;
+  long units = 0;
+  for (int k = 0; k < njobs; ++k)
+    if (!(k > 0 && chain && chain[k]) && jobs[k].cols > 0) units += (jobs[k].cols + 63) / 64;
+  return units;
+}
+}
+
+extern "C" int vit_gemm_group_prepare(const vit_gemm_args* args, const int32_t* direct, int32_t n, void* table,
+                                      int64_t table_bytes, int32_t* total_out, vit_stream_t stream) {
+  VIT_CHECK_ARG(args != nullptr && n >= 1 && n <= vitg::GEMM_TABLE_MAX, "vit_gemm_group_prepare: 1..%d members, got %d",
+                vitg::GEMM_TABLE_MAX, n);
+  VIT_CHECK_ARG(table != nullptr && total_out != nullptr && table_bytes >= (int64_t)vitg::group_table_bytes(n) &&
+                    ((uintptr_t)table % 16) == 0,
+                "vit_gemm_group_prepare: needs a 16-byte aligned table of vit_gemm_group_table_bytes(n) bytes");
+  std::vector<char> host(vitg::group_table_bytes(n), 0);
+  int32_t total = 0;
+  if (const int rc = build_group_members(args, direct, n, host.data(), &total)) return rc;
+  if (const int rc = upload_table(table, host, stream, "vit_gemm_group_prepare upload")) return rc;
+  *total_out = total;
   return VIT_OK;
 }
 
 extern "C" int vit_gemm_group_launch(const void* table, int32_t n, int32_t total, vit_stream_t stream) {
   VIT_CHECK_ARG(table != nullptr && n >= 1 && n <= vitg::GEMM_TABLE_MAX && total >= 1,
                 "vit_gemm_group_launch: a prepared table, its member count and its workgroup total");
-  return vit::check_hip(vitg::launch_group_table(table, n, total, (hipStream_t)stream), "vit_gemm_group_launch");
+  return vit::check_hip(vitg::launch_group_table(table, n, total, 0, 0, (hipStream_t)stream), "vit_gemm_group_launch");
+}
+
+extern "C" int64_t vit_gemm_group_fill_table_bytes(int32_t n, const vit_colsum_job* jobs, const int32_t* chain,
+                                                   int32_t njobs) {
+  const long units = fill_unit_count(jobs, chain, njobs);
+  if (n < 1 || n > vitg::GEMM_TABLE_MAX || units < 0) return 0;
+  return (int64_t)vitg::fill_table_bytes(n, njobs, units);
+}
+
+extern "C" int vit_gemm_group_fill_prepare(const vit_gemm_args* args, const int32_t* direct, int32_t n,
+                                           const vit_colsum_job* jobs, const int32_t* chain, int32_t njobs, void* table,
+                                           int64_t table_bytes, int32_t* total_out, int32_t* units_out,
+                                           vit_stream_t stream) {
+  const char* who = "vit_gemm_group_fill_prepare";
+  VIT_CHECK_ARG(args != nullptr && n >= 1 && n <= vitg::GEMM_TABLE_MAX, "%s: 1..%d members, got %d", who,
+                vitg::GEMM_TABLE_MAX, n);
+  VIT_CHECK_ARG(njobs >= 0 && njobs <= VIT_GEMM_FILL_JOBS_MAX && (njobs == 0 || jobs != nullptr),
+                "%s: 0..%d filler jobs, got %d", who, VIT_GEMM_FILL_JOBS_MAX, njobs);
+  VIT_CHECK_ARG(!(chain && njobs > 0 && chain[0]), "%s: job 0 has no job to chain to", who);
+  for (int k = 0; k < njobs; ++k) {
+    vitc::ColsumJobDev d;
+    if (const int rc = vitc::make_colsum_dev(jobs[k], k, who, d)) return rc;
+  }
+  const long units = fill_unit_count(jobs, chain, njobs);
+  const size_t bytes = vitg::fill_table_bytes(n, njobs, units);
+  VIT_CHECK_ARG(table != nullptr && total_out != nullptr && units_out != nullptr && table_bytes >= (int64_t)bytes &&
+                    ((uintptr_t)table % 16) == 0 && units < (1L << 24),
+                "%s: needs a 16-byte aligned table of vit_gemm_group_fill_table_bytes(...) bytes", who);
+  std::vector<char> host(bytes, 0);
+  int32_t total = 0;
+  if (const int rc = build_group_members(args, direct, n, host.data(), &total)) return rc;
+  vitc::ColsumJobDev* jd = reinterpret_cast<vitc::ColsumJobDev*>(host.data() + vitg::fill_jobs_off(n));
+  vitc::FillUnitDev* ud = reinterpret_cast<vitc::FillUnitDev*>(host.data() + vitg::fill_units_off(n, njobs));
+  std::vector<int> head(njobs > 0 ? njobs : 0);
+  long u = 0;
+  for (int k = 0; k < njobs; ++k) {
+    if (const int rc = vitc::make_colsum_dev(jobs[k], k, who, jd[k])) return rc;
+    const bool linked = k > 0 && chain && chain[k];
+    head[k] = linked ? head[k - 1] : k;
+    if (linked)
+      VIT_CHECK_ARG(jobs[k].cols == jobs[k - 1].cols && jobs[k].seg == jobs[k - 1].seg,
+                    "%s: job %d is chained to job %d but differs in cols / seg", who, k, k - 1);
+    for (int i = 0; i < k; ++i)
+      for (int a = 0; a < 3; ++a)
+        for (int b = 0; b < 3; ++b) {
+          uintptr_t lo0, hi0, lo1, hi1;
+          fill_out_range(jobs[i], a, lo0, hi0);
+          fill_out_range(jobs[k], b, lo1, hi1);
+          if (lo0 < hi0 && lo1 < hi1 && lo0 < hi1 && lo1 < hi0)
+            VIT_CHECK_ARG(head[i] == head[k] && a == b && lo0 == lo1,
+                          "%s: jobs %d and %d share an output: chain them (same output slot and address)", who, i, k);
+        }
+    if (!linked) {
+      const int nb = (int)((jobs[k].cols + 63) / 64);
+      for (int b = 0; b < nb; ++b) ud[u + b] = vitc::FillUnitDev{k, b, 1, 0};
+      u += nb;
+    } else {
+      const int nb = (int)((jobs[k].cols + 63) / 64);
+      for (int b = 0; b < nb; ++b) ud[u - nb + b].len += 1;
+    }
+  }
+  if (const int rc = upload_table(table, host, stream, "vit_gemm_group_fill_prepare upload")) return rc;
+  *total_out = total;
+  *units_out = (int32_t)units;
+  return VIT_OK;
+}
+
+extern "C" int vit_gemm_group_fill_launch(const void* table, int32_t n, int32_t total, int32_t njobs, int32_t n_units,
+                                          vit_stream_t stream) {
+  VIT_CHECK_ARG(table != nullptr && n >= 1 && n <= vitg::GEMM_TABLE_MAX && total >= 1 && njobs >= 0 &&
+                    njobs <= VIT_GEMM_FILL_JOBS_MAX && n_units >= 0 && (njobs > 0 || n_units == 0),
+                "vit_gemm_group_fill_launch: a prepared table, its member count, workgroup total, job and unit counts");
+  return vit::check_hip(vitg::launch_group_table(table, n, total, njobs, n_units, (hipStream_t)stream),
+                        "vit_gemm_group_fill_launch");
 }
 
 namespace {
diff --git a/vit-of-pytorch_amd/csrc/gemm_decl.h b/vit-of-pytorch_amd/csrc/gemm_decl.h
--- a/vit-of-pytorch_amd/csrc/gemm_decl.h
+++ b/vit-of-pytorch_amd/csrc/gemm_decl.h
@@ -1,5 +1,6 @@
 #pragma once
 #include "common.h"
+#include "colsum_dev.h"
 #include <stdlib.h>
 
 namespace vitg {
@@ -51,7 +52,14 @@
 constexpr int GEMM_TABLE_MAX = 128;
 inline size_t group_table_start_off(int n) { return ((size_t)n * sizeof(GemmDev) + 15) & ~(size_t)15; }
 inline size_t group_table_bytes(int n) { return group_table_start_off(n) + ((size_t)n + 1) * sizeof(int); }
-hipError_t launch_group_table(const void* table, int n, int total, hipStream_t s);
+inline size_t fill_jobs_off(int n) { return (group_table_bytes(n) + 15) & ~(size_t)15; }
+inline size_t fill_units_off(int n, int njobs) {
+  return (fill_jobs_off(n) + (size_t)njobs * sizeof(vitc::ColsumJobDev) + 15) & ~(size_t)15;
+}
+inline size_t fill_table_bytes(int n, int njobs, long n_units) {
+  return fill_units_off(n, njobs) + (size_t)n_units * sizeof(vitc::FillUnitDev);
+}
+hipError_t launch_group_table(const void* table, int n, int total, int njobs, int n_units, hipStream_t s);
 
 constexpr int EPI_DROP = 16;
 
diff --git a/vit-of-pytorch_amd/csrc/gemm_e7.hip b/vit-of-pytorch_amd/csrc/gemm_e7.hip
--- a/vit-of-pytorch_amd/csrc/gemm_e7.hip
+++ b/vit-of-pytorch_amd/csrc/gemm_e7.hip
@@ -6,6 +6,6 @@
 
 hipError_t vitg::launch_splitk_group(const GemmGroup& g, hipStream_t s) { return launch_pp2_group(g, s); }
 
-hipError_t vitg::launch_group_table(const void* table, int n, int total, hipStream_t s) {
-  return launch_pp2_table(table, n, total, s);
+hipError_t vitg::launch_group_table(const void* table, int n, int total, int njobs, int n_units, hipStream_t s) {
+  return launch_pp2_table(table, n, total, njobs, n_units, s);
 }
diff --git a/vit-of-pytorch_amd/csrc/gemm_pp2.inc b/vit-of-pytorch_amd/csrc/gemm_pp2.inc
--- a/vit-of-pytorch_amd/csrc/gemm_pp2.inc
+++ b/vit-of-pytorch_amd/csrc/gemm_pp2.inc
@@ -1,3 +1,10 @@
+template <int BK = 64, int NA = 2>
+constexpr int pp2_lds_bytes() {
+  return (4 * NA + 2) * 128 * BK * 2;
+}
+template <int BK, int NA>
+__shared__ __attribute__((aligned(16))) char pp2_smem[pp2_lds_bytes<BK, NA>()];
+
 template <bool AK, bool BKC, int EPI, int BK = 64, int NA = 2>
 __device__ __forceinline__ void pp2_tile(const GemmDev& p, const int tm, const int tn, const int z,
                                          const int split_idx, const int orig) {
@@ -12,8 +19,9 @@
   constexpr int PR = 32;
   constexpr int WST = PR * LDW * 4;
   static_assert(8 * WST <= LDS && LDS <= 160 * 1024, "LDS budget / epilogue staging");
+  static_assert(LDS == pp2_lds_bytes<BK, NA>(), "pp2_smem is this tile's LDS");
   static_assert(2 * I * (NA - 1) <= 32 && (2 * NA - 1) * I <= 62 && 2 * (NB - 1) * I <= 62, "vmcnt range");
-  __shared__ __attribute__((aligned(16))) char smem[LDS];
+  char(&smem)[LDS] = pp2_smem<BK, NA>;
 
   const int lane = threadIdx.x & 63;
   const int wave = __builtin_amdgcn_readfirstlane(threadIdx.x >> 6);
@@ -436,9 +444,17 @@
 
 template <bool AK, bool BKC>
 __global__ void __launch_bounds__(512) gemm_pp2_table_kernel(const GemmDev* __restrict__ tab,
-                                                             const int* __restrict__ start, const int n) {
+                                                             const int* __restrict__ start, const int n,
+                                                             const int total,
+                                                             const vitc::ColsumJobDev* __restrict__ fill_jobs,
+                                                             const vitc::FillUnitDev* __restrict__ fill_units,
+                                                             const int n_units) {
   const int orig = blockIdx.x;
-  const int w = xcd_major(orig, (int)gridDim.x);
+  if (orig >= total) {
+    vitc::colsum_fill_workgroup(fill_jobs, fill_units, n_units, orig - total, pp2_smem<64, 2>);
+    return;
+  }
+  const int w = xcd_major(orig, total);
   int lo = 0, hi = n;
   while (hi - lo > 1) {
     const int mid = (lo + hi) >> 1;
@@ -468,9 +484,15 @@
   return hipGetLastError();
 }
 
-inline hipError_t launch_pp2_table(const void* table, int n, int total, hipStream_t s) {
+inline hipError_t launch_pp2_table(const void* table, int n, int total, int njobs, int n_units, hipStream_t s) {
   const GemmDev* tab = (const GemmDev*)table;
-  const int* start = (const int*)((const char*)table + vitg::group_table_start_off(n));
-  hipLaunchKernelGGL((gemm_pp2_table_kernel<false, false>), dim3(total), dim3(512), 0, s, tab, start, n);
+  const char* base = (const char*)table;
+  const int* start = (const int*)(base + vitg::group_table_start_off(n));
+  const vitc::ColsumJobDev* jobs = njobs > 0 ? (const vitc::ColsumJobDev*)(base + vitg::fill_jobs_off(n)) : nullptr;
+  const vitc::FillUnitDev* units =
+      njobs > 0 ? (const vitc::FillUnitDev*)(base + vitg::fill_units_off(n, njobs)) : nullptr;
+  if (njobs <= 0) n_units = 0;
+  hipLaunchKernelGGL((gemm_pp2_table_kernel<false, false>), dim3(total + (n_units + 1) / 2), dim3(512), 0, s, tab,
+                     start, n, total, jobs, units, n_units);
   return hipGetLastError();
 }
diff --git a/vit-of-pytorch_amd/vitmi/_lib.py b/vit-of-pytorch_amd/vitmi/_lib.py
--- a/vit-of-pytorch_amd/vitmi/_lib.py
+++ b/vit-of-pytorch_amd/vitmi/_lib.py
@@ -11,7 +11,7 @@
 c_f32 = ctypes.c_float
 c_vp = ctypes.c_void_p
 
-ABI_VERSION = 21
+ABI_VERSION = 22
 
 K_CONTIG, MN_CONTIG = 0, 1
 (EPI_F32, EPI_BF16, EPI_BIAS_BF16, EPI_BIAS_GELU, EPI_BIAS_RESID_F32, EPI_GELU_BWD, EPI_PATCH, EPI_SPLITK,
@@ -74,6 +74,11 @@
     "vit_gemm_group_prepare": (c_i32, [ctypes.POINTER(GemmArgs), ctypes.POINTER(c_i32), c_i32, c_vp, c_i64,
                                        ctypes.POINTER(c_i32), c_vp]),
     "vit_gemm_group_launch": (c_i32, [c_vp, c_i32, c_i32, c_vp]),
+    "vit_gemm_group_fill_table_bytes": (c_i64, [c_i32, ctypes.POINTER(ColsumJob), ctypes.POINTER(c_i32), c_i32]),
+    "vit_gemm_group_fill_prepare": (c_i32, [ctypes.POINTER(GemmArgs), ctypes.POINTER(c_i32), c_i32,
+                                            ctypes.POINTER(ColsumJob), ctypes.POINTER(c_i32), c_i32, c_vp, c_i64,
+                                            ctypes.POINTER(c_i32), ctypes.POINTER(c_i32), c_vp]),
+    "vit_gemm_group_fill_launch": (c_i32, [c_vp, c_i32, c_i32, c_i32, c_i32, c_vp]),
     "vit_segment_colsum": (c_i32, [c_vp, c_i32, c_i64, c_i64, c_i64, c_i64, c_i64, c_i64, c_f32, c_vp, c_i64, c_vp]),
     "vit_segment_colsum_bcast": (c_i32, [c_vp, c_i32, c_i64, c_i64, c_i64, c_i64, c_i64, c_i64, c_f32, c_vp, c_i64,
                                          c_vp, c_i64, c_i64, c_vp]),
diff --git a/vit-of-pytorch_amd/vitmi/engine.py b/vit-of-pytorch_amd/vitmi/engine.py
--- a/vit-of-pytorch_amd/vitmi/engine.py
+++ b/vit-of-pytorch_amd/vitmi/engine.py
@@ -188,6 +188,15 @@
         self.c_mu2, self.c_rs2 = z(b, dt=f), z(b, dt=f)
         self._cfg, self._dev = cfg, dev
         self.dhb_l = self.dg_l = self.dqkv_l = None
+        self.bias_l = None
+
+    def bias_bufs(self):
+        if self.bias_l is None:
+            L = self._cfg.num_layers
+            grow = lambda bufs, n: bufs + [torch.zeros_like(bufs[0]) for _ in range(max(n - len(bufs), 0))]
+            self.bias_l = {"ln": grow(self.lnparts, 2 * L + 1), "gelu": grow(self.gelu_parts, L),
+                           "qkv": grow(self.qkv_bparts, L)}
+        return self.bias_l
 
     def defer_bufs(self):
         if self.dhb_l is None:
@@ -202,15 +211,21 @@
 
 class _BiasReducer:
 
-    def __init__(self, eng, a):
+    def __init__(self, eng, a, deferred=False):
         self.eng = eng
         self.a = a
         self.D = eng.cfg.emb_dim
         self.nxt = {}
         self.queued = {}
         self.jobs = []
+        self.deferred = deferred
+        self.own = a.bias_bufs() if deferred else None
 
     def buf(self, kind, bufs):
+        if self.deferred:
+            i = self.nxt.get(kind, 0)
+            self.nxt[kind] = i + 1
+            return self.own[kind][i]
         n = self.queued.get(kind, 0)
         if n == len(bufs):
             self.flush()
@@ -222,13 +237,22 @@
 
     def reduce(self, part, rows, cols, ld, outs, seg=0):
         self.jobs.append((part, rows, cols, ld, seg, outs, False))
-        if len(self.jobs) == ops.COLSUM_BATCH_MAX:
+        if len(self.jobs) == ops.COLSUM_BATCH_MAX and not self.deferred:
             self.flush()
 
     def flush(self):
-        if self.jobs:
-            ops.colsum_batch(self.jobs)
-            self.jobs = []
+        if self.deferred:
+            return
+        self.finish()
+
+    def take(self):
+        jobs, self.jobs = self.jobs, []
+        return jobs
+
+    def finish(self):
+        for k in range(0, len(self.jobs), ops.COLSUM_BATCH_MAX):
+            ops.colsum_batch(self.jobs[k:k + ops.COLSUM_BATCH_MAX])
+        self.jobs = []
         self.queued.clear()
 
     def ln_bwd(self, dy, lddy, x, ldx, mean, rstd, gamma, dx, lddx, rows, dgamma_dbeta, dx_colsum, **kw):
@@ -278,6 +302,7 @@
         v = os.environ.get("VITMI_WGRAD_DEFER", "all")
         self.wgrad_defer = L if v == "all" else int(v)
         self._wgrad_tables = {}
+        self.bias_defer = os.environ.get("VITMI_BIAS_DEFER", "1") != "0"
         self.prune_last = os.environ.get("VITMI_PRUNE_LAST", "1") != "0"
         self._pruned = False
         self._side = None
@@ -388,7 +413,7 @@
             self.probe_wgrad.append((ev0, ev1, sum(2.0 * sp[4] * sp[5] * K * sp[9] for sp in specs), K, True))
         ops.splitk_reduce_group([(w, sp[9], s, sp[4], sp[5], sp[7], sp[8], sp[11], False) for sp, w in zip(specs, views)])
 
-    def _wgrad_batch(self, specs, slot):
+    def _wgrad_batch(self, specs, slot, fill=None):
         K = specs[0][6]
         assert all(sp[6] == K for sp in specs)
         s = ops.splitk_factor_group([(sp[4], sp[5], sp[9]) for sp in specs], K, _WGRAD_TARGET)
@@ -402,9 +427,13 @@
                 o += n
         for c0 in range(0, len(specs), ops.GEMM_TABLE_MAX):
             part = specs[c0:c0 + ops.GEMM_TABLE_MAX]
+            jobs = fill if c0 + ops.GEMM_TABLE_MAX >= len(specs) else None
             key = (s, self._ws.data_ptr() if s > 1 else 0) + tuple(
                 (sp[0].data_ptr(), sp[1], sp[2].data_ptr(), sp[3], sp[4], sp[5], sp[7].data_ptr()) + tuple(sp[8:])
                 for sp in part)
+            if jobs is not None:
+                key += tuple((j[0].data_ptr(),) + tuple(j[1:5]) + tuple(o.data_ptr() if o is not None else 0 for o in j[5])
+                             for j in jobs)
             ent = self._wgrad_tables.get((self._last_b, slot, c0))
             if ent is None or ent[0] != key:
                 members = []
@@ -415,7 +444,7 @@
                         members.append((A, B, out, M, N, K, dict(kw, ldc=ldo, c_bs=out_bs), True))
                     else:
                         members.append((A, B, views[c0 + k], M, N, K, dict(kw, ldc=N), False))
-                ent = (key, ops.GemmGroupTable(members))
+                ent = (key, ops.GemmGroupTable(members, fill=jobs))
                 self._wgrad_tables[(self._last_b, slot, c0)] = ent
             if self.probe_wgrad is not None:
                 ev0 = torch.cuda.Event(enable_timing=True)
@@ -651,13 +680,16 @@
         def flush_wgrad():
             nonlocal pending, held, launches
             if pending:
-                self._wgrad_batch(pending, launches)
+                self._wgrad_batch(pending, launches, fill=bias.take() if bias.deferred else None)
                 launches += 1
             pending, held = [], 0
         out_wb = None
-        bias = _BiasReducer(self, a)
+        bias = _BiasReducer(self, a, deferred=bool(defer) and self.bias_defer)
         ops.gemm_f32(C, D, b, dl, C, True, a.lncls, D, False, gv("classifier.weight"), D)
-        bias.reduce(dl, b, C, C, (gv("classifier.bias"),))
+        if bias.deferred and dl.data_ptr() != a.dlogits.data_ptr():
+            ops.colsum_batch([(dl, b, C, C, 0, (gv("classifier.bias"),), False)])
+        else:
+            bias.reduce(dl, b, C, C, (gv("classifier.bias"),))
         ops.gemm_f32(b, D, C, dl, C, False, f[self.off("classifier.weight"):], D, False, a.dlncls, D)
         wb = 0
         pruned = self._pruned
@@ -757,7 +789,7 @@
         ops.embed_grad(a.dh, b, N, D, gv("transformer.pos_embedding.pos_embedding"), gv("cls_token"),
                        gv("embedding.bias"), dropout=dd(0))
         fire(self.layout.buckets[-1])
-        bias.flush()
+        bias.finish()
         if overlap:
             main.wait_stream(side)
         return g
diff --git a/vit-of-pytorch_amd/vitmi/ops.py b/vit-of-pytorch_amd/vitmi/ops.py
--- a/vit-of-pytorch_amd/vitmi/ops.py
+++ b/vit-of-pytorch_amd/vitmi/ops.py
@@ -250,13 +250,17 @@
 
 
 def colsum_batch(jobs):
+    check(lib().vit_colsum_batch(_colsum_jobs(jobs), len(jobs), _stream()), "vit_colsum_batch")
+
+
+def _colsum_jobs(jobs):
     arr = (_lib.ColsumJob * len(jobs))()
     for k, (inp, rows, cols, ld, seg, outs, acc) in enumerate(jobs):
         if inp.dtype != F32:
             raise ValueError("colsum_batch: f32 inputs only")
         o = list(outs) + [None] * (3 - len(outs))
         arr[k] = _lib.ColsumJob(_p(inp), rows, cols, ld, seg, _p(o[0]), _p(o[1]), _p(o[2]), int(acc), 0)
-    check(lib().vit_colsum_batch(arr, len(jobs), _stream()), "vit_colsum_batch")
+    return arr
 
 
 def gemm_f32(M, N, K, A, lda, a_trans, B, ldb, b_trans, C, ldc, bias=None, accumulate=False):
@@ -541,14 +545,17 @@
 
 
 GEMM_TABLE_MAX = 128
+GEMM_FILL_JOBS_MAX = 1024
 
 
 class GemmGroupTable:
 
-    def __init__(self, members):
+    def __init__(self, members, fill=None, chain=None):
         n = len(members)
         if not 1 <= n <= GEMM_TABLE_MAX:
             raise ValueError(f"GemmGroupTable: 1 to {GEMM_TABLE_MAX} members")
+        if fill is not None and len(fill) > GEMM_FILL_JOBS_MAX:
+            raise ValueError(f"GemmGroupTable: at most {GEMM_FILL_JOBS_MAX} filler jobs")
         arr = (GemmArgs * n)()
         direct = (ctypes.c_int32 * n)()
         for i, (A, B, C, M, N, K, kw, d) in enumerate(members):
@@ -557,15 +564,34 @@
             _chk(C, F32, "C")
             arr[i] = _gemm_args(A, B, C, M, N, K, **kw)
             direct[i] = int(bool(d))
-        nbytes = int(lib().vit_gemm_group_table_bytes(n))
-        self.table = torch.empty(nbytes, device=members[0][0].device, dtype=torch.uint8)
         total = ctypes.c_int32(0)
-        check(lib().vit_gemm_group_prepare(arr, direct, n, _p(self.table), nbytes, ctypes.byref(total), _stream()),
-              "vit_gemm_group_prepare")
+        self.njobs = self.units = None
+        if fill is None:
+            nbytes = int(lib().vit_gemm_group_table_bytes(n))
+            self.table = torch.empty(nbytes, device=members[0][0].device, dtype=torch.uint8)
+            check(lib().vit_gemm_group_prepare(arr, direct, n, _p(self.table), nbytes, ctypes.byref(total), _stream()),
+                  "vit_gemm_group_prepare")
+        else:
+            nj = len(fill)
+            jobs = _colsum_jobs(fill) if nj else None
+            ch = (ctypes.c_int32 * nj)(*[int(bool(c)) for c in chain]) if chain is not None and nj else None
+            nbytes = int(lib().vit_gemm_group_fill_table_bytes(n, jobs, ch, nj))
+            if nbytes <= 0:
+                raise ValueError("GemmGroupTable: bad member or filler job count")
+            self.table = torch.empty(nbytes, device=members[0][0].device, dtype=torch.uint8)
+            units = ctypes.c_int32(0)
+            check(lib().vit_gemm_group_fill_prepare(arr, direct, n, jobs, ch, nj, _p(self.table), nbytes,
+                                                    ctypes.byref(total), ctypes.byref(units), _stream()),
+                  "vit_gemm_group_fill_prepare")
+            self.njobs, self.units = nj, int(units.value)
         self.n, self.total = n, int(total.value)
 
     def launch(self):
-        check(lib().vit_gemm_group_launch(_p(self.table), self.n, self.total, _stream()), "vit_gemm_group_launch")
+        if self.njobs is None:
+            check(lib().vit_gemm_group_launch(_p(self.table), self.n, self.total, _stream()), "vit_gemm_group_launch")
+        else:
+            check(lib().vit_gemm_group_fill_launch(_p(self.table), self.n, self.total, self.njobs, self.units,
+                                                   _stream()), "vit_gemm_group_fill_launch")
 
 
 def splitk_factor(M, N, K, batch=1, cus=256):
```

Result: no change. 7716 images/sec, median of 6 (+0.6%).
